# microsoft/XPretrain

Measured on AMD Instinct MI355X. Metric: video-text pairs/sec, higher is better.
Workload: dtype bf16; 1 GPU; CLIP-ViP ViT-B/16 video-text contrastive train step (fwd+loss+bwd+grad-sync+clip+AdamW), 12 frames 224^2, 32 text tokens, local batch 8, BASELINE configs[1]; global_batch=8, parallelism=dp1, gemm_cu_budget=256, grad_wire=fp32, forced_one_rank_collectives=False, video_forward_chains=2, optimizer_overlaps_next_forward_from_layer=3, launch=eager

## Files before the change

include/xpretrain_hip.h:

```cpp
#ifndef XPRETRAIN_HIP_H
#define XPRETRAIN_HIP_H

#include <stddef.h>
#include <stdint.h>

#ifdef __cplusplus
extern "C" {
#endif

#define XP_ABI_VERSION 1

enum { XP_BF16 = 0, XP_F32 = 1 };
enum { XP_OK = 0, XP_ERR_ARG = -1, XP_ERR_LAUNCH = -2, XP_ERR_UNSUPPORTED = -3 };

int xp_abi_version(void);
const char* xp_last_error(void);

enum {
  XP_EPI_NONE = 0,
  XP_EPI_BIAS = 1,
  XP_EPI_BIAS_QSCALE = 2,
  XP_EPI_BIAS_GELU = 3,
  XP_EPI_BIAS_RESID = 4,
  XP_EPI_GELU_BWD = 5,
  XP_EPI_PATCH = 6,
  XP_EPI_SCALE = 7,
  XP_EPI_BIAS_GELU_ERF = 8,
  XP_EPI_GELU_ERF_BWD = 9
};

typedef struct XpGemmDesc {
  const void* A; const void* B; void* C;
  int64_t M, N, K;
  int64_t lda, ldb, ldc;
  int32_t a_kstrided, b_kstrided;
  int32_t in_dtype, out_dtype;
  int32_t epilogue;
  int32_t split_k;
  int64_t a_grp, a_grp_stride, a_off;
  int64_t c_grp, c_grp_stride, c_off;
  const float* bias;
  float scale; int64_t scale_cols;
  const void* resid; int64_t ldr;
  void* aux; int64_t ldaux;
  const float* tab1; const float* tab2; int64_t tab_L;
  float* colsum_partials;
  int32_t reserved0;
  int32_t side_M;
  const float* resid_side; float* out_side; int64_t side_S;
  const void* a_frames; int32_t a_frames_u8; int32_t fr_H, fr_W, fr_P; float fr_mean[3], fr_std[3];
} XpGemmDesc;

int xp_gemm(const XpGemmDesc* desc, void* stream);

int32_t xp_gemm_auto_split(const XpGemmDesc* desc);
int32_t xp_gemm_auto_split_slack(const XpGemmDesc* desc);
int xp_set_cu_budget(int32_t cus);
int32_t xp_get_cu_budget(void);
int64_t xp_gemm_colsum_rows(const XpGemmDesc* desc);
int32_t xp_gemm_tile_rows(const XpGemmDesc* desc);

int xp_splitk_reduce(const float* slabs, float* out, int64_t n, int32_t splits, int32_t accumulate, void* stream);

size_t xp_colsum_workspace_bytes(int64_t rows, int64_t cols);
int xp_colsum(const void* X, int64_t rows, int64_t cols, int64_t ldx, int32_t dtype, float* out,
              int32_t accumulate, void* workspace, size_t workspace_bytes, void* stream);

int64_t xp_colsum_partial_rows(int64_t rows, int64_t cols);
int xp_colsum_partials(const void* X, int64_t rows, int64_t cols, int64_t ldx, int32_t dtype, float* partials,
                       size_t partials_bytes, void* stream);

#define XP_REDUCE_MAX_SEGS 16
typedef struct {
  const float* in; float* out;
  int64_t stride;
  int32_t nrows, width;
  int32_t accumulate, reserved;
} XpReduceSeg;
size_t xp_reduce_rows_batch_workspace_bytes(const XpReduceSeg* segs_host, int32_t n);
int xp_reduce_rows_batch(const XpReduceSeg* segs_host, int32_t n, void* workspace, size_t workspace_bytes, void* stream);

int xp_layernorm_fwd(const void* x, int64_t ldx, const float* gamma, const float* beta, void* y, int64_t ldy,
                     float* mean, float* rstd, int64_t rows, int64_t cols, float eps, int32_t dtype, void* stream);
int xp_layernorm_fwd_side(const void* x, int64_t ldx, const float* gamma, const float* beta, void* y, int64_t ldy,
                          float* mean, float* rstd, int64_t rows, int64_t cols, float eps, int32_t dtype,
                          const float* x_side, float* y_side, int64_t side_S, int32_t side_M, int32_t side_stride, void* stream);
size_t xp_layernorm_bwd_workspace_bytes(int64_t rows, int64_t cols);
int64_t xp_layernorm_bwd_partial_rows(int64_t rows);
int xp_layernorm_bwd_partials(const void* dy, int64_t lddy, const void* x, int64_t ldx, const float* gamma,
                              const float* mean, const float* rstd, const void* dres, int64_t lddres,
                              void* dx, int64_t lddx, int32_t with_dx_colsum, int64_t rows, int64_t cols,
                              int32_t dtype, void* workspace, size_t workspace_bytes, void* stream);
int xp_layernorm_bwd(const void* dy, int64_t lddy, const void* x, int64_t ldx, const float* gamma,
                     const float* mean, const float* rstd, const void* dres, int64_t lddres,
                     void* dx, int64_t lddx, float* dgamma, float* dbeta, int32_t accumulate,
                     int64_t rows, int64_t cols, int32_t dtype,
                     void* workspace, size_t workspace_bytes, void* stream);
int xp_layernorm_bwd_partials_side(const void* dy, int64_t lddy, const void* x, int64_t ldx, const float* gamma,
                                   const float* mean, const float* rstd, const void* dres, int64_t lddres,
                                   void* dx, int64_t lddx, int32_t with_dx_colsum, int64_t rows, int64_t cols,
                                   int32_t dtype, const float* x_side, int64_t side_S, int32_t side_M, int32_t side_stride,
                                   void* workspace, size_t workspace_bytes, void* stream);
int xp_layernorm_bwd_side(const void* dy, int64_t lddy, const void* x, int64_t ldx, const float* gamma,
                          const float* mean, const float* rstd, const void* dres, int64_t lddres,
                          void* dx, int64_t lddx, float* dgamma, float* dbeta, int32_t accumulate,
                          int64_t rows, int64_t cols, int32_t dtype,
                          const float* x_side, int64_t side_S, int32_t side_M, int32_t side_stride,
                          void* workspace, size_t workspace_bytes, void* stream);

enum { XP_ATTN_PROXY = 0, XP_ATTN_CAUSAL = 1 };
size_t xp_attn_workspace_bytes(int32_t mode, int64_t B, int64_t H, int64_t M, int64_t N, int64_t L);
int xp_attn_fwd(const void* qkv, int64_t ldqkv, void* out, int64_t ldo, float* stats,
                const int64_t* pad_mask, int32_t mode, int64_t B, int64_t H, int64_t S,
                int64_t M, int64_t N, int64_t L, int32_t dtype,
                void* workspace, size_t workspace_bytes, void* stream);
int xp_attn_bwd(const void* qkv, int64_t ldqkv, const void* out, const void* dout, int64_t ldo,
                const float* stats, const int64_t* pad_mask, void* dqkv, float q_scale,
                int32_t mode, int64_t B, int64_t H, int64_t S, int64_t M, int64_t N, int64_t L, int32_t dtype,
                void* workspace, size_t workspace_bytes, void* stream);
int xp_set_attn_bwd_wide(int32_t on);
int32_t xp_get_attn_bwd_wide(void);
int64_t xp_attn_bwd_colsum_rows(int32_t mode, int64_t B, int64_t H, int64_t S, int64_t M, int64_t N, int64_t L, int32_t dtype);
int xp_attn_bwd2(const void* qkv, int64_t ldqkv, const void* out, const void* dout, int64_t ldo,
                 const float* stats, const int64_t* pad_mask, void* dqkv, float q_scale,
                 int32_t mode, int64_t B, int64_t H, int64_t S, int64_t M, int64_t N, int64_t L, int32_t dtype,
                 void* workspace, size_t workspace_bytes, float* dqkv_colsum_partials, void* stream);

int xp_attn_probs(const void* qkv, int64_t ldqkv, const float* stats, const int64_t* pad_mask,
                  float* probs, float* probs_proxy, int32_t mode, int64_t B, int64_t H, int64_t S,
                  int64_t M, int64_t N, int64_t L, int32_t dtype, void* stream);

size_t xp_attn_pooled_workspace_bytes(int64_t B, int64_t H, int64_t S, int32_t dtype);
int xp_attn_pooled_fwd(const void* q, const void* kv, int64_t ldkv, void* out, float* stats, int64_t B, int64_t H, int64_t S,
                       int32_t dtype, void* workspace, size_t workspace_bytes, void* stream);
int64_t xp_attn_pooled_colsum_rows(int64_t B, int64_t H, int64_t S, int32_t dtype);
int64_t xp_attn_pooled_colsum_rows_max(int64_t B, int64_t S);
int xp_attn_pooled_bwd(const void* q, const void* kv, int64_t ldkv, const void* out, const void* dout, const float* stats,
                       void* dq, int64_t lddq, void* dkv, int64_t lddkv, float q_scale, int64_t B, int64_t H, int64_t S,
                       int32_t dtype, void* workspace, size_t workspace_bytes, float* dkv_colsum_partials, void* stream);

int xp_im2col(const float* video, void* patches, int64_t BT, int64_t H, int64_t W, int64_t P, int32_t dtype, void* stream);
int xp_im2col_u8(const uint8_t* frames, const float* mean3_host, const float* std3_host, void* patches, int64_t BT,
                 int64_t H, int64_t W, int64_t P, int32_t dtype, void* stream);
#define XP_FRAMES_MAX_VIDEOS 32
#define XP_FRAMES_MAX_SIZE 16384
typedef struct {
  const uint8_t* src; int64_t src_bytes;
  int64_t stride_t, stride_y, stride_x, stride_c;
  int32_t T, H, W;
  int32_t box_y, box_x, box_h, box_w;
  int32_t rh, rw;
  int32_t top, left;
  int32_t flip;
} XpFrameSrc;
int xp_frames_resize_norm(const XpFrameSrc* videos_host, int32_t n_videos, const float* mean3_host,
                          const float* std3_host, float* out, int32_t oh, int32_t ow, void* stream);
#define XP_FRAMES_TRANSFORM_MAX_VIDEOS 24
enum { XP_FRAMES_FILTER_BICUBIC = 0, XP_FRAMES_FILTER_BILINEAR2 = 1 };
enum { XP_FRAMES_COLOR_BRIGHTNESS = 0, XP_FRAMES_COLOR_SATURATION = 2, XP_FRAMES_COLOR_HUE = 3 };
typedef struct {
  XpFrameSrc src;
  int32_t filter;
  int32_t mid_h, mid_w;
  int32_t crop_y, crop_x, crop_h, crop_w;
  int32_t n_color;
  int32_t color_op[3];
  float color_factor[3];
} XpFrameTransform;
int xp_frames_transform(const XpFrameTransform* videos_host, int32_t n_videos, const float* mean3_host,
                        const float* std3_host, float* out, int32_t oh, int32_t ow, void* stream);
#define XP_FRAMES_AA_MAX_TAPS 128
size_t xp_frames_transform_aa_workspace_bytes(const XpFrameTransform* videos_host, int32_t n_videos, int32_t oh, int32_t ow);
int xp_frames_transform_aa(const XpFrameTransform* videos_host, int32_t n_videos, const float* mean3_host,
                           const float* std3_host, float* out, int32_t oh, int32_t ow, void* workspace, size_t workspace_bytes,
                           void* stream);
int xp_vip_proxy_rows(const float* class_emb, const float* added_cls, const float* pos, void* x,
                      int64_t B, int64_t S, int64_t M, int64_t D, int32_t dtype, void* stream);
size_t xp_vip_embed_bwd_workspace_bytes(int64_t B, int64_t T, int64_t L, int64_t D);
int xp_vip_embed_bwd(const void* dx, float* d_class, float* d_added, float* d_pos, float* d_time,
                     int64_t B, int64_t M, int64_t T, int64_t L, int64_t D, int32_t dtype, int32_t accumulate,
                     void* workspace, size_t workspace_bytes, void* stream);
int xp_pos_resample_fwd(const float* pos, float* out, int32_t g0, int32_t gh, int32_t gw, int32_t D, void* stream);
int xp_pos_resample_bwd(const float* d_out, float* d_pos, int32_t g0, int32_t gh, int32_t gw, int32_t D, void* stream);
int xp_text_embed_fwd(const int64_t* ids, const float* tok, const float* pos, void* x,
                      int64_t B, int64_t Lt, int64_t D, int64_t vocab, int32_t dtype, void* stream);
int xp_text_embed_bwd(const int64_t* ids, const void* dx, float* d_tok, float* d_pos,
                      int64_t B, int64_t Lt, int64_t D, int64_t vocab, int32_t dtype, int32_t accumulate, void* stream);
int xp_argmax_rows(const int64_t* ids, int64_t* idx, int64_t B, int64_t Lt, void* stream);
int xp_gather_rows(const void* x, const int64_t* idx, void* out, int64_t B, int64_t S, int64_t D, int32_t dtype, void* stream);
int xp_scatter_rows(const void* dout, const int64_t* idx, void* dx, int64_t B, int64_t S, int64_t D, int32_t dtype, void* stream);
int xp_l2norm_fwd(const void* x, float* y, float* inv_norm, int64_t rows, int64_t cols, int32_t dtype, void* stream);
int xp_l2norm_bwd(const float* dy, const float* y, const float* inv_norm, void* dx, int64_t rows, int64_t cols,
                  int32_t dtype, void* stream);
int xp_cast(const float* src, void* dst, int64_t n, int32_t dtype, void* stream);
int xp_cast_back(const void* src, float* dst, int64_t n, int32_t dtype, int32_t accumulate, void* stream);

#define XP_OPT_CHUNK 65536
#define XP_OPT_MAX_TENSORS 256
#define XP_OPT_MAX_GROUPS 16
typedef struct {
  void* p; void* m; void* v;
  void* shadow;
  int64_t numel;
  int32_t shadow_dtype;
  int32_t reserved;
} XpAdamTensor;
typedef struct {
  float lr, beta1, beta2, eps, weight_decay;
  float step_size;
} XpAdamGroup;
int xp_grad_sqnorm_partials(const XpAdamTensor* table, const int32_t* chunk_map, int32_t n_chunks,
                            const void* const* grads_host, int32_t n_tensors, float* partials, void* stream);
int xp_adamw_step(const XpAdamTensor* table, const int32_t* chunk_map, int32_t n_chunks,
                  const void* const* grads_host, const uint8_t* group_of_host, int32_t n_tensors,
                  const XpAdamGroup* groups_host, int32_t n_groups, const float* norm_partials,
                  int32_t n_norm_partials, float max_norm, float* grad_norm_out, void* stream);

enum XpOptKind { XP_OPT_ADAM, XP_OPT_ADAMAX };
typedef struct {
  float lr, beta1, beta2, eps, weight_decay;
  float step_size;
  float bias2_sqrt;
  float one_minus_beta1;
} XpOptGroup;
int xp_optim_step(int32_t kind, const XpAdamTensor* table, const int32_t* chunk_map, int32_t n_chunks,
                  const void* const* grads_host, const uint8_t* group_of_host, int32_t n_tensors,
                  const XpOptGroup* groups_host, int32_t n_groups, const float* norm_partials,
                  int32_t n_norm_partials, float max_norm, float* grad_norm_out, void* stream);

typedef struct {
  float norm;
  int32_t finite;
  int32_t first_bad_chunk;
  int32_t reserved;
  int64_t applied, skipped;
} XpStepVerdict;
int xp_step_verdict(const float* partials, int32_t n_partials, XpStepVerdict* verdict, void* stream);
int xp_adamw_step_guarded(const XpAdamTensor* table, const int32_t* chunk_map, int32_t n_chunks,
                          const void* const* grads_host, const uint8_t* group_of_host, int32_t n_tensors,
                          const XpAdamGroup* groups_host, int32_t n_groups, const float* norm_partials,
                          int32_t n_norm_partials, float max_norm, float* grad_norm_out,
                          const XpStepVerdict* verdict, void* stream);
int xp_optim_step_guarded(int32_t kind, const XpAdamTensor* table, const int32_t* chunk_map, int32_t n_chunks,
                          const void* const* grads_host, const uint8_t* group_of_host, int32_t n_tensors,
                          const XpOptGroup* groups_host, int32_t n_groups, const float* norm_partials,
                          int32_t n_norm_partials, float max_norm, float* grad_norm_out,
                          const XpStepVerdict* verdict, void* stream);

size_t xp_nce_loss_workspace_bytes(int64_t n, int64_t d);
int xp_nce_loss(const float* vis, const float* txt, const float* log_scale, float* loss,
                float* d_vis, float* d_txt, float* d_log_scale, int64_t n, int64_t d,
                void* workspace, size_t workspace_bytes, void* stream);

size_t xp_vsc_fc_loss_workspace_bytes(int64_t n, int64_t d);
int xp_vsc_fc_loss(const float* vis, const float* txt, const float* img, const float* cap, const float* log_scale,
                   float* loss, float* d_vis, float* d_txt, float* d_img, float* d_cap, float* d_log_scale,
                   int64_t n, int64_t d, void* workspace, size_t workspace_bytes, void* stream);

enum XpLossKind { XP_LOSS_NCE, XP_LOSS_VSC_FC, XP_LOSS_DSL, XP_LOSS_VS_VC, XP_LOSS_VS_VC_FC,
                  XP_LOSS_VSC, XP_LOSS_VIDIMG, XP_LOSS_VIDIMG_DIVIDE };
size_t xp_contrastive_loss_workspace_bytes(int32_t kind, int64_t n, int64_t m, int64_t d);
int xp_contrastive_loss(int32_t kind, const float* vis, const float* txt, const float* img, const float* cap,
                        const float* log_scale, float* loss, float* d_vis, float* d_txt, float* d_img, float* d_cap,
                        float* d_log_scale, int64_t n, int64_t m, int64_t d,
                        void* workspace, size_t workspace_bytes, void* stream);

enum XpPairLossKind { XP_PAIR_NCE, XP_PAIR_TRIPLET, XP_PAIR_HARDNEG, XP_PAIR_MILNCE };
typedef struct {
  float temp, margin;
  int32_t max_violation, order_measure, hard_negative_num, bag;
} XpPairLossParams;
size_t xp_pair_loss_workspace_bytes(int32_t kind, const XpPairLossParams* params, int64_t n, int64_t d);
int xp_pair_loss(int32_t kind, const XpPairLossParams* params, const float* vis, const float* txt, float* loss,
                 float* d_vis, float* d_txt, int64_t n, int64_t d, void* workspace, size_t workspace_bytes, void* stream);

int xp_sim_matrix(const float* a, const float* b, float* sim, int64_t na, int64_t nb, int64_t d, void* stream);
int xp_dsl_rerank(float* sim, int64_t n, int64_t m, float theta, int32_t multiply, void* stream);
int xp_retrieval_ranks(const float* sim, const int64_t* labels, int64_t n, int64_t m, int32_t transpose,
                       int32_t* greater, int32_t* equal, void* stream);

#define XP_RETRIEVAL_TILE 128
#define XP_RETRIEVAL_MAX_K 128
int xp_retrieval_stream_plan(int64_t nq, int64_t ng, int32_t k, int32_t* stat_tiles_per_split, int32_t* topk_tiles_per_split);
size_t xp_retrieval_ranks_streamed_workspace_bytes(int64_t nq, int64_t ng, int64_t d, int32_t dsl);
int xp_retrieval_ranks_streamed(const float* q, const float* g, const int64_t* labels_q, const int64_t* labels_g, int64_t nq,
                                int64_t ng, int64_t d, int32_t dsl, float theta, int32_t* greater_q, int32_t* equal_q,
                                int32_t* greater_g, int32_t* equal_g, void* workspace, size_t workspace_bytes, void* stream);
size_t xp_retrieval_topk_workspace_bytes(int64_t nq, int64_t ng, int64_t d, int32_t k);
int xp_retrieval_topk(const float* q, const float* g, int64_t nq, int64_t ng, int64_t d, int32_t k, int64_t index_base,
                      int32_t accumulate, float* vals, int64_t* idx, void* workspace, size_t workspace_bytes, void* stream);

typedef struct XpLayerDims {
  int64_t rows, D, Dff, B, S, heads;
  int64_t M, N, L;
  int32_t attn_mode, dtype;
  float q_scale, ln_eps;
  int32_t act;
} XpLayerDims;
enum { XP_ACT_QUICK_GELU = 0, XP_ACT_GELU = 1 };

typedef struct XpLayerFwd {
  XpLayerDims dims;
  const void* x; const void* Wqkv; const void* Wo; const void* W1; const void* W2;
  const float* ln1_w; const float* ln1_b; const float* bqkv; const float* bo;
  const float* ln2_w; const float* ln2_b; const float* b1; const float* b2;
  const int64_t* pad_mask;
  void* h1; void* qkv; void* attn_o; void* x2; void* h2; void* pre; void* act; void* x3;
  float* mean1; float* rstd1; float* mean2; float* rstd2; float* stats;
  void* workspace; size_t workspace_bytes;
  const float* side_in; float* side_out; int64_t side_S; int32_t side_M; int32_t reserved;
  float* side_x2;
} XpLayerFwd;
size_t xp_encoder_layer_fwd_workspace_bytes(const XpLayerDims* dims);
int xp_encoder_layer_fwd(const XpLayerFwd* args, void* stream);

typedef struct XpLayerBwd {
  XpLayerDims dims;
  const void* x; const void* h1; const void* qkv; const void* attn_o; const void* x2; const void* h2; const void* pre;
  const void* act; const void* Wqkv; const void* Wo; const void* W1; const void* W2;
  const float* ln1_w; const float* ln2_w; const float* mean1; const float* rstd1; const float* mean2; const float* rstd2;
  const float* stats; const int64_t* pad_mask;
  const void* dx3;
  void* dx;
  float* dln1_w; float* dln1_b; float* dwqkv; float* dbqkv; float* dwo; float* dbo;
  float* dln2_w; float* dln2_b; float* dw1; float* db1; float* dw2; float* db2;
  void* workspace; size_t workspace_bytes;
  const float* side_in; const float* side_x2; int64_t side_S; int32_t side_M; int32_t reserved;
} XpLayerBwd;
size_t xp_encoder_layer_bwd_workspace_bytes(const XpLayerDims* dims);
int xp_encoder_layer_bwd(const XpLayerBwd* args, void* stream);
typedef struct XpLayerPooledFwd {
  XpLayerDims dims;
  const void* x; const void* Wqkv; const void* Wo; const void* W1; const void* W2;
  const float* ln1_w; const float* ln1_b; const float* bqkv; const float* bo;
  const float* ln2_w; const float* ln2_b; const float* b1; const float* b2;
  void* h1; void* kv; float* mean1; float* rstd1;
  void* h1p; void* q; void* attn_o; void* x2; void* h2; void* pre; void* act; void* x3;
  float* mean1p; float* rstd1p; float* mean2; float* rstd2; float* stats;
  void* workspace; size_t workspace_bytes;
  const float* side_in; float* side_out; float* side_x2;
} XpLayerPooledFwd;
size_t xp_encoder_layer_pooled_fwd_workspace_bytes(const XpLayerDims* dims);
int xp_encoder_layer_pooled_fwd(const XpLayerPooledFwd* args, void* stream);

typedef struct XpLayerPooledBwd {
  XpLayerDims dims;
  const void* x; const void* h1; const void* kv; const void* h1p; const void* q; const void* attn_o; const void* x2;
  const void* h2; const void* pre; const void* act; const void* Wqkv; const void* Wo; const void* W1; const void* W2;
  const float* ln1_w; const float* ln2_w; const float* mean1; const float* rstd1; const float* mean1p; const float* rstd1p;
  const float* mean2; const float* rstd2; const float* stats;
  const void* dx3;
  void* dx;
  float* dln1_w; float* dln1_b; float* dwqkv; float* dbqkv; float* dwo; float* dbo;
  float* dln2_w; float* dln2_b; float* dw1; float* db1; float* dw2; float* db2;
  void* workspace; size_t workspace_bytes;
  const float* side_in; const float* side_x2;
} XpLayerPooledBwd;
size_t xp_encoder_layer_pooled_bwd_workspace_bytes(const XpLayerDims* dims);
int xp_encoder_layer_pooled_bwd(const XpLayerPooledBwd* args, void* stream);
void* xp_side_stream(void);

int xp_debug_set_gemm_trace(void* device_buffer);
int xp_debug_gemm_timer_arm(int64_t M, int64_t N, int64_t K, int32_t epilogue, int32_t a_kstrided, int32_t b_kstrided, int32_t split_k,
                            int32_t max_launches);
int32_t xp_debug_gemm_timer_read(float* ms, int32_t cap);
int xp_debug_set_attn_trace(void* device_buffer);
int xp_debug_gemm_occupancy(int lds_bytes);
enum { XP_GEMM_FAMILY_256 = 0,
       XP_GEMM_FAMILY_DIRECT = 1,
       XP_GEMM_FAMILY_STAGED = 2,
       XP_GEMM_FAMILY_FRAMES = 3 };
enum { XP_GEMM_EPI_FAST = 0,
       XP_GEMM_EPI_ROW8 = 1,
       XP_GEMM_EPI_ROW4 = 2 };
typedef struct XpGemmPlanInfo {
  int32_t family, tile_rows;
  int32_t split, flat_split;
  int64_t k_per_split;
  int32_t tiles_m, tiles_n, group_n;
  int32_t epi_impl;
  int32_t grid[3];
  int32_t reserved;
  int64_t colsum_rows;
} XpGemmPlanInfo;
int xp_debug_gemm_plan(const XpGemmDesc* desc, XpGemmPlanInfo* out);
enum { XP_ATTN_KERNEL_FWD = 0,
       XP_ATTN_KERNEL_FWD3 = 1,
       XP_ATTN_KERNEL_FWD4 = 2,
       XP_ATTN_KERNEL_BWD_PAIR = 3,
       XP_ATTN_KERNEL_BWD5 = 4,
       XP_ATTN_KERNEL_F32 = 5 };
enum { XP_ATTN_OPTIN_BWD6 = 6 };
typedef struct XpAttnPlanInfo {
  int32_t kernel;
  int32_t grid, lds_bytes;
  int32_t reduce_grid;
  int32_t uses_counter;
  int32_t reserved;
  int64_t part[2], delta[2], dq[2], dkv[2], counter[2];
  int64_t workspace_bytes;
  int64_t colsum_rows;
} XpAttnPlanInfo;
int xp_debug_attn_plan(int32_t mode, int64_t B, int64_t H, int64_t S, int64_t M, int64_t N, int64_t L, int32_t dtype,
                       int32_t has_pad_mask, int32_t backward, int32_t cus, XpAttnPlanInfo* out);
typedef struct XpAttnPooledPlanInfo {
  int32_t chunks, chunk_keys;
  int32_t grid, combine_grid;
  int64_t part_ml[2], part_acc[2];
  int64_t part_dq[2];
  int64_t workspace_bytes;
  int64_t colsum_rows;
} XpAttnPooledPlanInfo;
int xp_debug_attn_pooled_plan(int64_t B, int64_t H, int64_t S, int32_t dtype, int32_t backward, int32_t cus,
                              XpAttnPooledPlanInfo* out);
int xp_probe_mfma_bf16(const void* a, const void* b, float* c, void* stream);
int xp_probe_mfma_f32(const float* a, const float* b, float* c, void* stream);
int xp_probe_pk_f32(void* err , int32_t iters, int32_t blocks, uint32_t seed, void* stream);
int xp_probe_stream_copy(void* dst, const void* src, int64_t nbytes, int32_t blocks, int32_t iters, void* stream);
int xp_probe_stream_copy_fat(void* dst, const void* src, int64_t nbytes, int32_t blocks, int32_t iters, void* stream);
int xp_probe_tr16(const void* in , const int32_t* lane_byte_off , void* out , void* stream);

#ifdef __cplusplus
}
#endif
#endif
```

xpretrain_amd/csrc/gemm.hip:

```cpp
#include "common.h"
#include "gemm_common.h"
#include <stdlib.h>
#include <mutex>
#include <vector>

namespace {

using namespace xpgemm;
constexpr int BM = 128, BN = 128, BKB = 128;
constexpr int NT = 256;
constexpr int TILE_BYTES = 128 * 128;

template <typename T>
__device__ __forceinline__ void gload_kc(u32x4 (&r)[4], const T* base, int64_t ld, int64_t row0, int64_t rows,
                                         int64_t k0, int64_t kend, const Remap& map, int tid) {
  constexpr int EPC = 16 / sizeof(T);
  const int c = tid & 7, rr = tid >> 3;
  const int64_t k = k0 + c * EPC;
#pragma unroll
  for (int j = 0; j < 4; ++j) {
    const int64_t row = row0 + rr + 32 * j;
    if (row < rows && k < kend)
      r[j] = *reinterpret_cast<const u32x4*>(base + map(row) * ld + k);
    else
// ... 386 lines not shown
      return;
    }
  }
  if (f == Family::DIRECT) launch2<T, true>(d, kp, grid, st);
  else                     launch2<T, false>(d, kp, grid, st);
}

}

extern "C" int xp_debug_gemm_occupancy(int lds_bytes) {
  int nb = -1;
  hipError_t e = hipOccupancyMaxActiveBlocksPerMultiprocessor(&nb, gemm_kernel<bf16_t, false, false, true>, 2 * NT, (size_t)lds_bytes);
  if (e != hipSuccess) return -(int)e;
  return nb;
}

static unsigned long long* g_gemm_trace = nullptr;
extern "C" int xp_debug_set_gemm_trace(void* device_buffer) { g_gemm_trace = (unsigned long long*)device_buffer; return XP_OK; }

namespace {
struct GemmTimer {
  std::mutex mu;
  bool armed = false;
  int64_t M = 0, N = 0, K = 0; int epi = 0, aks = 0, bks = 0, split = 1;
  std::vector<hipEvent_t> ev;
  size_t used = 0;
} g_timer;
static volatile bool g_timer_on = false;
}

extern "C" int xp_debug_gemm_timer_arm(int64_t M, int64_t N, int64_t K, int32_t epilogue, int32_t a_kstrided, int32_t b_kstrided,
                                       int32_t split_k, int32_t max_launches) {
  XP_REQUIRE(max_launches > 0 && max_launches <= 4096, "xp_debug_gemm_timer_arm: max_launches must be 1..4096");
  std::lock_guard<std::mutex> lock(g_timer.mu);
  while (g_timer.ev.size() < (size_t)max_launches * 2) {
    hipEvent_t e;
    if (hipEventCreate(&e) != hipSuccess) { xp_set_error("xp_debug_gemm_timer_arm: hipEventCreate failed"); return XP_ERR_LAUNCH; }
    g_timer.ev.push_back(e);
  }
  g_timer.M = M; g_timer.N = N; g_timer.K = K; g_timer.epi = epilogue; g_timer.aks = a_kstrided; g_timer.bks = b_kstrided;
  g_timer.split = split_k > 1 ? split_k : 1;
  g_timer.used = 0; g_timer.armed = true; g_timer_on = true;
  return XP_OK;
}

extern "C" int32_t xp_debug_gemm_timer_read(float* ms, int32_t cap) {
  std::lock_guard<std::mutex> lock(g_timer.mu);
  g_timer_on = false; g_timer.armed = false;
  const int n = (int)(g_timer.used / 2);
  for (int i = 0; i < n && i < cap; ++i) {
    if (hipEventSynchronize(g_timer.ev[2 * i + 1]) != hipSuccess || hipEventElapsedTime(&ms[i], g_timer.ev[2 * i], g_timer.ev[2 * i + 1]) != hipSuccess) {
      xp_set_error("xp_debug_gemm_timer_read: event query failed");
      return -1;
    }
  }
  g_timer.used = 0;
  return n;
}

static int gemm_timer_slot(const XpGemmDesc* d, int split) {
  if (!g_timer_on) return -1;
  std::lock_guard<std::mutex> lock(g_timer.mu);
  if (!g_timer.armed || d->M != g_timer.M || d->N != g_timer.N || d->K != g_timer.K || d->epilogue != g_timer.epi ||
      (d->a_kstrided != 0) != (g_timer.aks != 0) || (d->b_kstrided != 0) != (g_timer.bks != 0) || split != g_timer.split ||
      g_timer.used + 2 > g_timer.ev.size())
    return -1;
  const int slot = (int)g_timer.used;
  g_timer.used += 2;
  return slot;
}

struct GemmPlan {
  Family family;
  int tile_rows;
  int split; int64_t k_per_split;
  int tiles_m, tiles_n, group_n, xcd_remap, flat_split;
  int wide, fast_epi;
  int epi_impl;
  int64_t colsum_rows;
  dim3 grid;
};

static GemmPlan plan_gemm(const XpGemmDesc* d, int split) {
  GemmPlan p{};
  p.split = split = split > 1 ? split : 1;
  const int esz = d->in_dtype == XP_BF16 ? 2 : 4, ke = BKB / esz;
  p.k_per_split = cdiv(cdiv(d->K, split), ke) * ke;
  p.xcd_remap = 1;
  p.wide = d->N % 8 == 0 && d->ldc % 8 == 0 && (!d->resid || d->ldr % 8 == 0) && (!d->aux || d->ldaux % 8 == 0);
  const int64_t osz = d->out_dtype == XP_F32 ? 4 : esz, lim = (int64_t)EPI_OOB - 64, rows = d->M + 256;
  p.fast_epi = p.wide && !xp_debug_flag("gemm_slow_epi") && d->c_grp == 0 && rows * d->ldc * osz < lim &&
               (!d->resid || rows * d->ldr * esz < lim) && (!d->aux || rows * d->ldaux * osz < lim);
  const int ep = epi_base(d->epilogue);
  const bool f32 = d->out_dtype == XP_F32, cs_epi = ep == XP_EPI_NONE || ep == XP_EPI_GELU_BWD;
  p.epi_impl = epi_impl(p.fast_epi, p.wide, ep, f32, d->colsum_partials != nullptr);
  const bool epi256 = p.epi_impl == XP_GEMM_EPI_FAST;
  const char* env = getenv("XPRETRAIN_GEMM256");
  const int mode = env ? atoi(env) : 1;
  const int64_t k_last = d->K - (int64_t)(split - 1) * p.k_per_split;
  if (mode != 0 && xp_gemm256_legal(d) && epi256 && (mode != 1 || cdiv(d->M, 256) * cdiv(d->N, 256) * split >= 96) &&
      cdiv(k_last, 64) >= 2 && (split == 1 || cdiv(d->K, p.k_per_split) == split)) {
    p.family = Family::G256; p.tile_rows = 256;
    p.tiles_m = (int)cdiv(d->M, 256); p.tiles_n = (int)cdiv(d->N, 256);
    p.group_n = split > 1 ? p.tiles_n : xp_gemm256_group_n(d, p.tiles_n);
    const bool chunk_major = split > 1 && !xp_debug_flag("dw_tile_major");
    p.flat_split = chunk_major ? split : 0;
    p.colsum_rows = split == 1 && !f32 && cs_epi ? 2 * cdiv(d->M, 256) : 0;
    p.grid = dim3(p.tiles_m * p.tiles_n * (chunk_major ? split : 1), 1, chunk_major ? 1 : split);
    return p;
  }
  p.family = d->in_dtype == XP_BF16 && d->a_frames ? Family::FRAMES : glds_ok(d, esz) ? Family::DIRECT : Family::STAGED;
  p.tile_rows = BM;
  p.tiles_m = (int)cdiv(d->M, BM); p.tiles_n = (int)cdiv(d->N, BN);
  const int gmax = 4;
  p.group_n = (int)cdiv(p.tiles_n, cdiv(p.tiles_n, gmax));
  p.grid = dim3(p.tiles_m * p.tiles_n, 1, split);
  return p;
}

extern "C" int xp_gemm(const XpGemmDesc* d, void* stream) {
  XP_REQUIRE(d && (d->A || d->a_frames) && d->B && d->C, "xp_gemm: null operand");
  XP_REQUIRE(d->M > 0 && d->N > 0 && d->K > 0, "xp_gemm: empty problem M=%lld N=%lld K=%lld",
             (long long)d->M, (long long)d->N, (long long)d->K);
  XP_REQUIRE(d->in_dtype == XP_BF16 || d->in_dtype == XP_F32, "xp_gemm: bad in_dtype %d", d->in_dtype);
  XP_REQUIRE(d->out_dtype == d->in_dtype || d->out_dtype == XP_F32, "xp_gemm: bad out_dtype %d", d->out_dtype);
  const int esz = d->in_dtype == XP_BF16 ? 2 : 4;
  const int epc = 16 / esz;
  const int64_t a_contig = d->a_kstrided ? d->M : d->K, b_contig = d->b_kstrided ? d->N : d->K;
  XP_REQUIRE(a_contig % epc == 0 && b_contig % epc == 0 && d->lda % epc == 0 && d->ldb % epc == 0,
             "xp_gemm: contiguous extents / leading dims must be multiples of %d elements", epc);
  XP_REQUIRE(d->N % 4 == 0 && d->ldc % 4 == 0, "xp_gemm: N and ldc must be multiples of 4");
  XP_REQUIRE(((uintptr_t)d->A | (uintptr_t)d->B | (uintptr_t)d->C) % 16 == 0, "xp_gemm: operands must be 16-byte aligned");
  if (d->a_frames) {
    const int64_t P = d->fr_P, gh = P > 0 ? d->fr_H / P : 0, gw = P > 0 ? d->fr_W / P : 0;
    XP_REQUIRE(d->in_dtype == XP_BF16 && !d->a_kstrided && !d->b_kstrided && d->a_grp == 0 && (d->split_k <= 1),
               "xp_gemm: a_frames needs bf16 compute, k-contiguous operands, no row remap of A, no split-K");
    XP_REQUIRE(P > 0 && P % 8 == 0 && d->fr_H % P == 0 && d->fr_W % P == 0 && d->K == 3 * P * P && gh * gw > 0 && d->M % (gh * gw) == 0,
               "xp_gemm: a_frames needs P %% 8 == 0, H and W multiples of P, K == 3*P*P and M a multiple of the patches per frame");
    XP_REQUIRE(((uintptr_t)d->a_frames & (d->a_frames_u8 ? 7 : 15)) == 0 && (d->a_frames_u8 ? d->fr_W % 8 == 0 : d->fr_W % 4 == 0),
               "xp_gemm: a_frames must be 16-byte (fp32) / 8-byte (uint8) aligned with a row pitch that keeps 8-pixel strips aligned");
    if (d->a_frames_u8) for (int c = 0; c < 3; ++c) XP_REQUIRE(d->fr_std[c] > 0.f, "xp_gemm: fr_std[%d] must be positive", c);
  }
  XP_REQUIRE(d->epilogue >= XP_EPI_NONE && d->epilogue <= XP_EPI_GELU_ERF_BWD, "xp_gemm: bad epilogue %d", d->epilogue);
  const int ep = epi_base(d->epilogue);
  if (ep == XP_EPI_BIAS || ep == XP_EPI_BIAS_QSCALE || ep == XP_EPI_BIAS_GELU || ep == XP_EPI_BIAS_RESID)
    XP_REQUIRE(d->bias, "xp_gemm: epilogue %d needs bias", ep);
  if (ep == XP_EPI_BIAS_RESID || ep == XP_EPI_GELU_BWD) XP_REQUIRE(d->resid && d->ldr % 4 == 0, "xp_gemm: epilogue %d needs resid", ep);
  if (ep == XP_EPI_BIAS_GELU) XP_REQUIRE(!d->aux || d->ldaux % 4 == 0, "xp_gemm: epilogue BIAS_GELU: bad ldaux");
  if (ep == XP_EPI_PATCH) XP_REQUIRE(d->tab1 && d->tab2 && d->tab_L > 0, "xp_gemm: epilogue PATCH needs tab1/tab2/tab_L");
  const int split = d->split_k > 1 ? d->split_k : 1;
  if (split > 1) XP_REQUIRE(ep == XP_EPI_NONE && d->out_dtype == XP_F32 && d->c_grp == 0 && d->ldc == d->N,
                            "xp_gemm: split_k needs EPI_NONE, f32 output, dense C");

  const GemmPlan plan = plan_gemm(d, split);
  KParams kp;
  kp.A = d->A; kp.B = d->B; kp.C = d->C;
  kp.M = d->M; kp.N = d->N; kp.K = d->K; kp.lda = d->lda; kp.ldb = d->ldb; kp.ldc = d->ldc;
  kp.amap = Remap{d->a_grp, d->a_grp_stride, d->a_off};
  kp.cmap = Remap{d->c_grp, d->c_grp_stride, d->c_off};
  kp.epilogue = ep; kp.out_f32 = d->out_dtype == XP_F32;
  kp.k_per_split = plan.k_per_split;
  kp.bias = d->bias; kp.scale = d->scale; kp.scale_cols = d->scale_cols;
  kp.resid = d->resid; kp.ldr = d->ldr; kp.aux = d->aux; kp.ldaux = d->ldaux;
  kp.tab1 = d->tab1; kp.tab2 = d->tab2; kp.tab_L = d->tab_L;
  kp.dbg = g_gemm_trace;
  kp.im_src = d->a_frames; kp.im_u8 = d->a_frames_u8; kp.im_H = d->fr_H; kp.im_W = d->fr_W; kp.im_P = d->fr_P;
  kp.im_gw = d->fr_P > 0 ? d->fr_W / d->fr_P : 1; kp.im_L = d->fr_P > 0 ? (d->fr_H / d->fr_P) * kp.im_gw : 1;
  for (int c = 0; c < 3; ++c) { kp.im_mean[c] = d->fr_mean[c]; kp.im_std[c] = d->fr_std[c]; }
  kp.tiles_m = plan.tiles_m; kp.tiles_n = plan.tiles_n; kp.group_n = plan.group_n; kp.xcd_remap = plan.xcd_remap;
  kp.flat_split = plan.flat_split; kp.wide = plan.wide; kp.fast_epi = plan.fast_epi;
  kp.colsum = d->colsum_partials;
  kp.rside = d->resid_side; kp.oside = d->out_side; kp.side_S = (unsigned)d->side_S; kp.side_M = (unsigned)d->side_M;
  if (d->resid_side || d->out_side)
    XP_REQUIRE(d->resid_side && d->out_side && ep == XP_EPI_BIAS_RESID && d->out_dtype == d->in_dtype && d->c_grp == 0 &&
               d->side_S > 0 && d->side_M > 0 && d->side_M <= d->side_S && d->M + 512 < ((int64_t)1 << 24) && d->N % 8 == 0,
               "xp_gemm: resid_side / out_side need both pointers, EPI_BIAS_RESID, an unmapped output, 0 < side_M <= side_S, M < 2^24");
  if (d->colsum_partials)
    XP_REQUIRE(plan.colsum_rows > 0, "xp_gemm: fused column sums are not available for this problem "
               "(xp_gemm_colsum_rows() == 0): use xp_colsum / xp_colsum_partials");
  const int zsplits = (int)cdiv(d->K, plan.k_per_split);
  XP_REQUIRE(split == 1 || zsplits == split, "xp_gemm: split_k=%d leaves empty slabs for K=%lld (use <= %d)",
             split, (long long)d->K, zsplits);
  hipStream_t st = (hipStream_t)stream;
  const int tslot = gemm_timer_slot(d, split);
  if (tslot >= 0) (void)hipEventRecord(g_timer.ev[tslot], st);
  struct Stop { int slot; hipStream_t st; ~Stop() { if (slot >= 0) (void)hipEventRecord(g_timer.ev[slot + 1], st); } } stop{tslot, st};
  if (plan.family == Family::G256) {
    if (!xp_gemm256_launch(d, kp, plan.grid, st)) {
      xp_set_error("xp_gemm: the 256x256 family cannot launch: no current device, or its 128 KiB dynamic-LDS opt-in was refused");
      return XP_ERR_LAUNCH;
    }
    XP_CHECK_LAUNCH("xp_gemm(256)");
    return XP_OK;
  }
  if (d->in_dtype == XP_BF16) launch<bf16_t>(plan.family, d, kp, plan.grid, st);
  else                        launch<float>(plan.family, d, kp, plan.grid, st);
  XP_CHECK_LAUNCH("xp_gemm");
  return XP_OK;
}

extern "C" int64_t xp_gemm_colsum_rows(const XpGemmDesc* d) { return d ? plan_gemm(d, d->split_k).colsum_rows : 0; }

extern "C" int xp_debug_gemm_plan(const XpGemmDesc* d, XpGemmPlanInfo* out) {
  XP_REQUIRE(d && out, "xp_debug_gemm_plan: null argument");
  const GemmPlan p = plan_gemm(d, d->split_k);
  static_assert((int)Family::G256 == XP_GEMM_FAMILY_256 && (int)Family::DIRECT == XP_GEMM_FAMILY_DIRECT &&
                (int)Family::STAGED == XP_GEMM_FAMILY_STAGED && (int)Family::FRAMES == XP_GEMM_FAMILY_FRAMES, "XP_GEMM_FAMILY_*");
  *out = XpGemmPlanInfo{};
  out->family = (int)p.family; out->tile_rows = p.tile_rows;
  out->split = p.split; out->flat_split = p.flat_split; out->k_per_split = p.k_per_split;
  out->tiles_m = p.tiles_m; out->tiles_n = p.tiles_n; out->group_n = p.group_n;
  out->epi_impl = p.epi_impl;
  out->grid[0] = (int)p.grid.x; out->grid[1] = (int)p.grid.y; out->grid[2] = (int)p.grid.z;
  out->colsum_rows = p.colsum_rows;
  return XP_OK;
}

extern "C" int32_t xp_gemm_tile_rows(const XpGemmDesc* d) {
  if (!d || d->M <= 0 || d->N <= 0 || d->K <= 0) return 0;
  return plan_gemm(d, d->split_k).tile_rows;
}

static int valid_split(int64_t K, int64_t s0, int64_t ke) {
  if (s0 <= 1) return 1;
  const int64_t kps = cdiv(cdiv(K, s0), ke) * ke;
  return (int)cdiv(K, kps);
}

static int g_cu_budget = [] {
  const char* e = getenv("XPRETRAIN_CU_BUDGET");
  const int v = e ? atoi(e) : 256;
  return v >= 64 && v <= 256 ? v : 256;
}();
extern "C" int xp_set_cu_budget(int32_t cus) {
  XP_REQUIRE(cus >= 64 && cus <= 256, "xp_set_cu_budget: %d not in 64..256", cus);
  g_cu_budget = cus;
  return XP_OK;
}
extern "C" int32_t xp_get_cu_budget(void) { return g_cu_budget; }

constexpr int64_t XP_SPLITK_FILL = 144, XP_SPLITK_FILL_SLACK = 112;
static int64_t g_fill[2] = {XP_SPLITK_FILL, XP_SPLITK_FILL_SLACK};
static const bool g_fill_env = [] {
  const char* e = getenv("XPRETRAIN_SPLITK_FILL");
  if (!e) return false;
  int a = 0, b = 0;
  const int n = sscanf(e, "%d%*[,x]%d", &a, &b);
  if (n >= 1 && a >= 9 && a <= 256) g_fill[0] = a;
  if (n >= 2 && b >= 9 && b <= 256) g_fill[1] = b;
  return true;
}();
static int32_t auto_split_fill(const XpGemmDesc* d, int64_t fill);
extern "C" int32_t xp_gemm_auto_split(const XpGemmDesc* d) { return auto_split_fill(d, g_fill[0]); }
extern "C" int32_t xp_gemm_auto_split_slack(const XpGemmDesc* d) {
  const int32_t s = auto_split_fill(d, g_fill[1]), g = auto_split_fill(d, g_fill[0]);
  return s < g ? s : g;
}

static int32_t auto_split_fill(const XpGemmDesc* d, int64_t fill) {
  if (!d || d->M <= 0 || d->N <= 0 || d->K <= 0) return 1;
  const int esz = d->in_dtype == XP_BF16 ? 2 : 4;
  const int64_t ke = BKB / esz;
  const int64_t t256 = cdiv(d->M, 256) * cdiv(d->N, 256);
  const int64_t cus = g_cu_budget < fill ? g_cu_budget : fill;
  int64_t s0 = cus / t256 < d->K / 512 ? cus / t256 : d->K / 512;
  const int s256 = valid_split(d->K, s0, 64);
  if (plan_gemm(d, s256).family == Family::G256) return s256;
  const int64_t t128 = cdiv(d->M, BM) * cdiv(d->N, BN);
  if (t128 >= 256) return 1;
  s0 = 512 / t128 < d->K / 512 ? 512 / t128 : d->K / 512;
  return valid_split(d->K, s0, ke);
}
```

xpretrain_amd/csrc/gemm256.hip:

```cpp
#include "common.h"
#include "gemm_common.h"

namespace {

using namespace xpgemm;

typedef bf16_t T;
constexpr int TM = 256, TN = 256, SKB = 128, KE = 64;
constexpr int NTH = 512, NWAVES = 8;
constexpr int WAVES_N = 4, MT = 8, NT = 4;
constexpr int HALF_ROWS = 128, HALF_BYTES = HALF_ROWS * SKB, NSLOT = 8, LDS_BYTES = NSLOT * HALF_BYTES;

typedef __attribute__((address_space(3))) char lds_char;

template <bool KS, int SUB>
struct HalfStager {
  __amdgpu_buffer_rsrc_t rsrc;
  unsigned voff[2][2];
  unsigned step;
  unsigned lds_off[2];

  static __device__ __forceinline__ int tile_row(int r, int h) { return (r / SUB) * (2 * SUB) + h * SUB + (r % SUB); }

  __device__ __forceinline__ void init(const T* base, int64_t ld, int64_t row0, int64_t rows, int64_t kend, int64_t kbeg,
                                       int lane, int wave) {
    const int64_t bytes = (KS ? kend : rows) * ld * 2;
    rsrc = __builtin_amdgcn_make_buffer_rsrc(const_cast<T*>(base), 0, (unsigned)bytes, 0x00020000);
#pragma unroll
    for (int j = 0; j < 2; ++j) {
      const int pass = j * NWAVES + wave;
      lds_off[j] = pass * 1024;
#pragma unroll
      for (int h = 0; h < 2; ++h) {
        int64_t off;
        if constexpr (!KS) {
          const int row = pass * 8 + (lane >> 3);
          const int c = (lane & 7) ^ swz128(row);
          off = ((row0 + tile_row(row, h)) * ld + kbeg) * 2 + c * 16;
        } else {
          const int kr = pass * 4 + (lane >> 4), c16 = lane & 15;
          const int src = (((c16 >> 1) ^ ks_f(kr)) << 1) | (c16 & 1);
          off = ((kbeg + kr) * ld + row0 + tile_row(src * 8, h)) * 2;
        }
        voff[h][j] = off >= bytes ? 0xFFFFFFF0u : (unsigned)off;
      }
    }
    step = (unsigned)((KS ? (int64_t)KE * ld : (int64_t)KE) * 2);
  }
  __device__ __forceinline__ void issue(char* slot, int h, int kt) const {
    lds_char* t3 = (lds_char*)slot;
    const unsigned adv = (unsigned)kt * step;
#pragma unroll
    for (int j = 0; j < 2; ++j) {
      unsigned o = voff[h][j] + adv;
      if (o < voff[h][j]) o = 0xFFFFFFF0u;
      __builtin_amdgcn_raw_ptr_buffer_load_lds(rsrc, t3 + lds_off[j], 16, o, 0, 0, 0);
    }
  }
};

template <bool KS>
__device__ __forceinline__ bf16x8 frag(const char* tile, int ot, int ks, int lane) {
  constexpr int RB = HALF_ROWS * 2;
  const int i = lane & 15, g = lane >> 4;
  if constexpr (!KS) {
    return *reinterpret_cast<const bf16x8*>(tile + tile128_off(ot * 16 + i, ks * 4 + g));
  } else {
    const int f = (i >> 2) | ((g & 1) << 2);
    const int kr = ks * 32 + g * 8 + (i >> 2);
    const char* p = tile + kr * RB + ((ot ^ f) << 5) + ((i & 3) << 3);
    i16x4 lo = lds_read_tr16_async<0>(p);
    i16x4 hi = lds_read_tr16_async<4 * RB>(p);
    typedef __attribute__((ext_vector_type(8))) short i16x8;
    i16x8 v = {lo[0], lo[1], lo[2], lo[3], hi[0], hi[1], hi[2], hi[3]};
    return __builtin_bit_cast(bf16x8, v);
  }
}

template <int N> __device__ __forceinline__ void wait_vmcnt() { asm volatile("s_waitcnt vmcnt(%0)" ::"n"(N) : "memory"); }

template <bool AKS, bool BKS, typename... Act>
__global__ __launch_bounds__(NTH, 2) void gemm256_kernel(KParams p) {
  constexpr int ACT = ActOf<Act...>::value;
  extern __shared__ __attribute__((aligned(16))) char smem[];
  const int tid = threadIdx.x, lane = tid & 63;
  const int wave = __builtin_amdgcn_readfirstlane(tid >> 6);
  const int wm = wave / WAVES_N, wn = wave % WAVES_N;

  const int nwg = p.tiles_m * p.tiles_n;
  int bid, zs, nsplit;
  if (p.flat_split > 0) {
    const int l = xcd_remap(blockIdx.x, nwg * p.flat_split, 1);
    zs = l / nwg; bid = l - zs * nwg; nsplit = p.flat_split;
  } else {
    bid = xcd_remap(blockIdx.x, nwg, p.xcd_remap); zs = blockIdx.z; nsplit = gridDim.z;
  }
  int tm, tn;
  tile_of(bid, p.tiles_m, p.tiles_n, p.group_n, tm, tn);
  const int64_t m0 = (int64_t)tm * TM, n0 = (int64_t)tn * TN;

  const int64_t kbeg = (int64_t)zs * p.k_per_split;
  const int64_t kend = (kbeg + p.k_per_split < p.K) ? kbeg + p.k_per_split : p.K;
  const int nk = (int)((kend - kbeg + KE - 1) / KE);

  HalfStager<AKS, 64> ga;
  HalfStager<BKS, 32> gb;
  ga.init(reinterpret_cast<const T*>(p.A), p.lda, m0, p.M, kend, kbeg, lane, wave);
  gb.init(reinterpret_cast<const T*>(p.B), p.ldb, n0, p.N, kend, kbeg, lane, wave);

  f32x4 acc[NT][MT];
#pragma unroll
  for (int a = 0; a < NT; ++a)
#pragma unroll
    for (int b = 0; b < MT; ++b) acc[a][b] = f32x4{0.f, 0.f, 0.f, 0.f};

  const bool trace = p.dbg != nullptr && bid == nwg / 2 && zs == 0 && wave == 0;
  unsigned long long* tr = p.dbg;
  if (trace && lane == 0) { tr[0] = __builtin_amdgcn_s_memtime(); tr[1] = nk; }
  const bool tline = p.dbg != nullptr && wave == 0 && lane == 0 && zs == 0 && tr[4] == 0x7aceull;
  if (tline) { tr[64 + bid * 4 + 0] = __builtin_amdgcn_s_memrealtime(); tr[64 + bid * 4 + 3] = __builtin_amdgcn_s_getreg(4 | (0 << 6) | (31 << 11)); }

  auto slot = [&](int kt, int w) -> char* { return smem + (((kt & 1) << 2) + w) * HALF_BYTES; };

  gb.issue(slot(1, 3), 0, 0);
  ga.issue(slot(0, 0), 0, 0); gb.issue(slot(0, 1), 1, 0); ga.issue(slot(0, 2), 1, 0); gb.issue(slot(0, 3), 0, 1);
  wait_vmcnt<4>();
  __builtin_amdgcn_s_barrier();
  if (wm == 1) __builtin_amdgcn_s_barrier();

  bf16x8 fa[2][4], fb[2][2][2], fbn[2][2];

#define XP_PHASE_MMA(HA)                                                                              \
  do {                                                                                                \
    __builtin_amdgcn_s_barrier();                                                                     \
    asm volatile("s_waitcnt lgkmcnt(0)" ::: "memory");                                                \
    __builtin_amdgcn_sched_barrier(0);                                                                \
    __builtin_amdgcn_s_setprio(1);                                                                    \
    _Pragma("unroll") for (int hb = 0; hb < 2; ++hb)                                                  \
      _Pragma("unroll") for (int ks = 0; ks < 2; ++ks)                                                \
        _Pragma("unroll") for (int mt = 0; mt < 4; ++mt)                                              \
          _Pragma("unroll") for (int nt = 0; nt < 2; ++nt)                                            \
            acc[hb * 2 + nt][(HA) * 4 + mt] = mma16(fb[hb][ks][nt], fa[ks][mt], acc[hb * 2 + nt][(HA) * 4 + mt]); \
    __builtin_amdgcn_s_setprio(0);                                                                    \
    __builtin_amdgcn_sched_barrier(0);                                                                \
    __builtin_amdgcn_s_barrier();                                                                     \
  } while (0)
#define XP_READ_A(TILE)                                                                               \
  _Pragma("unroll") for (int ks = 0; ks < 2; ++ks)                                                    \
    _Pragma("unroll") for (int mt = 0; mt < 4; ++mt) fa[ks][mt] = frag<AKS>(TILE, wm * 4 + mt, ks, lane)
#define XP_READ_B(DST, TILE)                                                                          \
  _Pragma("unroll") for (int ks = 0; ks < 2; ++ks)                                                    \
    _Pragma("unroll") for (int nt = 0; nt < 2; ++nt) DST[ks][nt] = frag<BKS>(TILE, wn * 2 + nt, ks, lane)

  XP_READ_B(fbn, slot(1, 3));

  auto ktile = [&](int t, auto tail_c) {
    constexpr int TAIL = decltype(tail_c)::value;
#pragma unroll
    for (int ks = 0; ks < 2; ++ks)
#pragma unroll
      for (int nt = 0; nt < 2; ++nt) fb[0][ks][nt] = fbn[ks][nt];
    XP_READ_B(fb[1], slot(t, 1));
    __builtin_amdgcn_sched_barrier(0);
    XP_READ_A(slot(t, 0));
    __builtin_amdgcn_sched_barrier(0);
    if constexpr (TAIL <= 1) { ga.issue(slot(t + 1, 0), 0, t + 1); gb.issue(slot(t + 1, 1), 1, t + 1); }
    wait_vmcnt<(TAIL <= 1 ? 4 : 0)>();
    XP_PHASE_MMA(0);
    if constexpr (TAIL <= 1) { XP_READ_B(fbn, slot(t, 3)); }
    __builtin_amdgcn_sched_barrier(0);
    XP_READ_A(slot(t, 2));
    __builtin_amdgcn_sched_barrier(0);
    if constexpr (TAIL <= 1) ga.issue(slot(t + 1, 2), 1, t + 1);
    if constexpr (TAIL == 0) gb.issue(slot(t + 1, 3), 0, t + 2);
    wait_vmcnt<(TAIL == 0 ? 4 : (TAIL == 1 ? 2 : 0))>();
    XP_PHASE_MMA(1);
  };
  for (int t = 0; t < nk - 2; ++t) ktile(t, std::integral_constant<int, 0>{});
  ktile(nk - 2, std::integral_constant<int, 1>{});
  ktile(nk - 1, std::integral_constant<int, 2>{});
#undef XP_PHASE_MMA
#undef XP_READ_A
#undef XP_READ_B
  if (wm == 0) __builtin_amdgcn_s_barrier();
  __builtin_amdgcn_s_barrier();
  if (trace && lane == 0) tr[2] = __builtin_amdgcn_s_memtime();
  if (tline) tr[64 + bid * 4 + 1] = __builtin_amdgcn_s_memrealtime();

  constexpr int CW = NT * 16;
  char* stg = smem + wave * (32 * CW * 4);
  const int i16 = lane & 15, g = lane >> 4;
  float* Cf = reinterpret_cast<float*>(p.C);
  T* Ct = reinterpret_cast<T*>(p.C);
  if (nsplit > 1) Cf += (int64_t)zs * p.M * p.N;
  auto stage_round = [&](int q) {
#pragma unroll
    for (int h = 0; h < 2; ++h) {
      const int row = h * 16 + i16;
#pragma unroll
      for (int nt = 0; nt < NT; ++nt)
        *reinterpret_cast<f32x4*>(stg + row * (CW * 4) + (((nt * 4 + g) ^ (row & 7)) << 4)) = acc[nt][q * 2 + h];
    }
    asm volatile("s_waitcnt lgkmcnt(0)" ::: "memory");
  };
  const bool fast = fast_epi_dispatch<ACT>(p, [&](auto epi_c, auto f32_c, auto cs_c) {
    constexpr int EPI = decltype(epi_c)::value;
    constexpr bool F32 = decltype(f32_c)::value;
    constexpr bool COLSUM = decltype(cs_c)::value;
    f32x8 cs = {f32x4{0.f, 0.f, 0.f, 0.f}, f32x4{0.f, 0.f, 0.f, 0.f}};
    const int c = lane & 7, r8 = lane >> 3;
    const FastEpi<T, EPI, F32, ACT> fe(p, F32 ? (void*)Cf : (void*)Ct, n0 + wn * CW + c * 8);
    const unsigned mrow = (unsigned)(m0 + wm * (MT * 16)) + r8;
    Raw8<T> pre[2][4];
    if constexpr (EpiTraits<EPI>::pre) {
#pragma unroll
      for (int pass = 0; pass < 4; ++pass) pre[0][pass] = fe.load_pre(mrow + pass * 8);
    }
#pragma unroll
    for (int q = 0; q < MT / 2; ++q) {
      if constexpr (EpiTraits<EPI>::pre) {
        if (q + 1 < MT / 2) {
#pragma unroll
          for (int pass = 0; pass < 4; ++pass) pre[(q + 1) & 1][pass] = fe.load_pre(mrow + (q + 1) * 32 + pass * 8);
        }
      }
      stage_round(q);
      f32x8 v[4];
#pragma unroll
      for (int pass = 0; pass < 4; ++pass) {
        const int row = pass * 8 + r8;
        v[pass].lo = *reinterpret_cast<const f32x4*>(stg + row * (CW * 4) + (((2 * c) ^ (row & 7)) << 4));
        v[pass].hi = *reinterpret_cast<const f32x4*>(stg + row * (CW * 4) + (((2 * c + 1) ^ (row & 7)) << 4));
      }
#pragma unroll
      for (int pass = 0; pass < 4; ++pass) {
        const f32x8 o = fe.finish(v[pass], pre[q & 1][pass], mrow + q * 32 + pass * 8);
        if constexpr (COLSUM) {
          if (mrow + q * 32 + pass * 8 < (unsigned)p.M) { cs.lo += o.lo; cs.hi += o.hi; }
        }
      }
      asm volatile("s_waitcnt lgkmcnt(0)" ::: "memory");
    }
    if constexpr (COLSUM) {
#pragma unroll
      for (int o = 8; o < 64; o <<= 1)
#pragma unroll
        for (int e = 0; e < 4; ++e) { cs.lo[e] += __shfl_xor(cs.lo[e], o, 64); cs.hi[e] += __shfl_xor(cs.hi[e], o, 64); }
      const int64_t n = n0 + wn * CW + c * 8;
      if (r8 == 0 && n < p.N) {
        float* dst = p.colsum + ((int64_t)tm * 2 + wm) * p.N + n;
        store4(dst, cs.lo); store4(dst + 4, cs.hi);
      }
    }
  });
  (void)fast;
  if (trace && lane == 0) tr[3] = __builtin_amdgcn_s_memtime();
  if (tline) { asm volatile("s_waitcnt vmcnt(0)" ::: "memory"); tr[64 + bid * 4 + 2] = __builtin_amdgcn_s_memrealtime(); }
}

template <bool AKS, bool BKS>
bool launch_one(int act, const KParams& kp, dim3 grid, hipStream_t st) {
  auto kern = act == XP_ACT_GELU ? gemm256_kernel<AKS, BKS, GeluErfTag> : gemm256_kernel<AKS, BKS>;
  if (!xp_device_cus(reinterpret_cast<const void*>(kern), LDS_BYTES)) return false;
  kern<<<grid, NTH, LDS_BYTES, st>>>(kp);
  return true;
}

template __global__ void gemm256_kernel<false, false>(KParams);
template __global__ void gemm256_kernel<false, true>(KParams);
template __global__ void gemm256_kernel<true, true>(KParams);
template __global__ void gemm256_kernel<true, false>(KParams);
template __global__ void gemm256_kernel<false, false, GeluErfTag>(KParams);
template __global__ void gemm256_kernel<false, true, GeluErfTag>(KParams);
template __global__ void gemm256_kernel<true, true, GeluErfTag>(KParams);
template __global__ void gemm256_kernel<true, false, GeluErfTag>(KParams);

}

bool xp_gemm256_legal(const XpGemmDesc* d) {
  if (d->in_dtype != XP_BF16 || d->a_grp != 0 || d->a_frames) return false;
  const int64_t a_rows = d->a_kstrided ? d->K : d->M, b_rows = d->b_kstrided ? d->K : d->N;
  if (!d->a_kstrided && (d->K % KE != 0 || d->lda != d->K)) return false;
  if (!d->b_kstrided && (d->K % KE != 0 || d->ldb != d->K)) return false;
  if (d->a_kstrided && (d->M % TM != 0 || d->lda != d->M)) return false;
  if (d->b_kstrided && (d->N % TN != 0 || d->ldb != d->N)) return false;
  const int64_t lim = (int64_t)0xFFFFFFF0u - 512 * 1024 * 1024;
  return (a_rows + TM) * d->lda * 2 < lim && (b_rows + TN) * d->ldb * 2 < lim;
}

int xp_gemm256_group_n(const XpGemmDesc* d, int tiles_n) {
  int groups = 1;
  const int64_t wbytes = (int64_t)tiles_n * TN * d->K * (d->in_dtype == XP_BF16 ? 2 : 4);
  while (groups < 4 && wbytes / groups > (int64_t)3600 * 1024 && tiles_n / (groups * 2) >= 4) groups *= 2;
  return (int)cdiv(tiles_n, groups);
}

bool xp_gemm256_launch(const XpGemmDesc* d, const xpgemm::KParams& kp, dim3 grid, hipStream_t st) {
  const int act = xpgemm::epi_act(d->epilogue);
  if (!d->a_kstrided && !d->b_kstrided)      return launch_one<false, false>(act, kp, grid, st);
  else if (!d->a_kstrided && d->b_kstrided)  return launch_one<false, true>(act, kp, grid, st);
  else if (d->a_kstrided && d->b_kstrided)   return launch_one<true, true>(act, kp, grid, st);
  return launch_one<true, false>(act, kp, grid, st);
}
```

xpretrain_amd/csrc/gemm_common.h:

```cpp
#pragma once
#include "common.h"
#include <type_traits>

namespace xpgemm {

struct Remap {
  int64_t grp, stride, off;
  __device__ __forceinline__ int64_t operator()(int64_t r) const {
    return grp == 0 ? r : (r / grp) * stride + off + (r % grp);
  }
};

__host__ __device__ constexpr int epi_base(int epilogue) {
  return epilogue == XP_EPI_BIAS_GELU_ERF ? XP_EPI_BIAS_GELU : epilogue == XP_EPI_GELU_ERF_BWD ? XP_EPI_GELU_BWD : epilogue;
}
__host__ __device__ constexpr int epi_act(int epilogue) {
  return epilogue == XP_EPI_BIAS_GELU_ERF || epilogue == XP_EPI_GELU_ERF_BWD ? XP_ACT_GELU : XP_ACT_QUICK_GELU;
}

struct GeluErfTag {};
template <typename... Tag> struct ActOf { static constexpr int value = XP_ACT_QUICK_GELU; };
template <> struct ActOf<GeluErfTag> { static constexpr int value = XP_ACT_GELU; };

struct KParams {
  const void* A; const void* B; void* C;
  int64_t M, N, K, lda, ldb, ldc;
  Remap amap, cmap;
  int epilogue, out_f32;
  int64_t k_per_split;
  const float* bias; float scale; int64_t scale_cols;
  const void* resid; int64_t ldr;
  void* aux; int64_t ldaux;
  const float* tab1; const float* tab2; int64_t tab_L;
  int tiles_m, tiles_n;
  int group_n;
  int xcd_remap;
  int wide;
  int fast_epi;
  float* colsum;
  const float* rside; float* oside; unsigned side_S, side_M;
  unsigned long long* dbg;
  int flat_split;
  const void* im_src; int im_u8, im_H, im_W, im_P, im_gw, im_L; float im_mean[3], im_std[3];
};


struct SideRows {
  const float* rin; float* out; unsigned S, M; int64_t N, rows; float inv_S;
  __device__ __forceinline__ SideRows(const KParams& p)
      : rin(p.rside), out(p.oside), S(p.side_S), M(p.side_M), N(p.N), rows(p.M), inv_S(1.0f / (float)p.side_S) {}
  __device__ __forceinline__ bool on() const { return rin != nullptr; }
  __device__ __forceinline__ bool hit(unsigned m, int64_t& base) const {
    unsigned q = (unsigned)((float)m * inv_S);
    int rem = (int)m - (int)(q * S);
    if (rem < 0) { --q; rem += (int)S; } else if (rem >= (int)S) { ++q; rem -= (int)S; }
    base = ((int64_t)q * M + rem) * N;
    return (unsigned)rem < M && (int64_t)m < rows;
  }
};

__device__ __forceinline__ f32x4 qscale4(float scale, int64_t scale_cols, int64_t n) {
  return f32x4{n < scale_cols ? scale : 1.f, n + 1 < scale_cols ? scale : 1.f, n + 2 < scale_cols ? scale : 1.f,
               n + 3 < scale_cols ? scale : 1.f};
}

struct EpiLane {
  f32x4 bias, colscale;
  __device__ __forceinline__ EpiLane(const KParams& p, int64_t n) {
    const int ep = p.epilogue;
    const bool has_bias = ep == XP_EPI_BIAS || ep == XP_EPI_BIAS_QSCALE || ep == XP_EPI_BIAS_GELU || ep == XP_EPI_BIAS_RESID;
    bias = has_bias ? load4(p.bias + n) : f32x4{0.f, 0.f, 0.f, 0.f};
    colscale = ep == XP_EPI_SCALE ? f32x4{p.scale, p.scale, p.scale, p.scale}
             : ep == XP_EPI_BIAS_QSCALE ? qscale4(p.scale, p.scale_cols, n) : f32x4{1.f, 1.f, 1.f, 1.f};
  }
};

template <typename T, int ACT = XP_ACT_QUICK_GELU>
__device__ __forceinline__ void epi_row(const KParams& p, const EpiLane& el, f32x4 v, int64_t m, int64_t n, float* Cf, T* Ct) {
  const int ep = p.epilogue;
  v = (v + el.bias) * el.colscale;
  const int64_t crow = p.cmap(m);
  if (ep == XP_EPI_BIAS_GELU) {
    if (!p.aux) {}
    else if (p.out_f32) store4(reinterpret_cast<float*>(p.aux) + crow * p.ldaux + n, v);
    else                store4(reinterpret_cast<T*>(p.aux) + crow * p.ldaux + n, v);
#pragma unroll
    for (int e = 0; e < 4; ++e) v[e] = act_f<ACT>(v[e]);
  } else if (ep == XP_EPI_BIAS_RESID) {
    const SideRows sr(p);
    int64_t sb;
    if (sr.on() && sr.hit((unsigned)m, sb)) { v += load4(sr.rin + sb + n); store4(sr.out + sb + n, v); }
    else v += load4(reinterpret_cast<const T*>(p.resid) + crow * p.ldr + n);
  } else if (ep == XP_EPI_GELU_BWD) {
    const f32x4 pre = load4(reinterpret_cast<const T*>(p.resid) + crow * p.ldr + n);
#pragma unroll
    for (int e = 0; e < 4; ++e) v[e] *= act_grad_f<ACT>(pre[e]);
  } else if (ep == XP_EPI_PATCH) {
    const int64_t w = p.cmap.grp ? (m % p.cmap.grp) : m;
    v += load4(p.tab1 + (w / p.tab_L) * p.N + n);
    v += load4(p.tab2 + (w % p.tab_L) * p.N + n);
  }
  if (p.out_f32) store4(Cf + crow * p.ldc + n, v);
  else           store4(Ct + crow * p.ldc + n, v);
}

struct EpiLane8 {
  f32x8 bias, cs;
  __device__ __forceinline__ EpiLane8(const KParams& p, int64_t n) {
    const EpiLane a(p, n), b(p, n + 4);
    bias = f32x8{a.bias, b.bias}; cs = f32x8{a.colscale, b.colscale};
  }
};
template <typename T, int ACT = XP_ACT_QUICK_GELU>
__device__ __forceinline__ void epi_row8(const KParams& p, const EpiLane8& el, f32x8 v, int64_t m, int64_t n, float* Cf, T* Ct) {
  const int ep = p.epilogue;
  v.lo = (v.lo + el.bias.lo) * el.cs.lo; v.hi = (v.hi + el.bias.hi) * el.cs.hi;
  const int64_t crow = p.cmap(m);
  if (ep == XP_EPI_BIAS_GELU) {
    if (!p.aux) {}
    else if (p.out_f32) store8(reinterpret_cast<float*>(p.aux) + crow * p.ldaux + n, v);
    else                store8(reinterpret_cast<T*>(p.aux) + crow * p.ldaux + n, v);
#pragma unroll
    for (int e = 0; e < 4; ++e) { v.lo[e] = act_f<ACT>(v.lo[e]); v.hi[e] = act_f<ACT>(v.hi[e]); }
  } else if (ep == XP_EPI_BIAS_RESID) {
    const SideRows sr(p);
    int64_t sb;
    if (sr.on() && sr.hit((unsigned)m, sb)) {
      const f32x8 r = load8(sr.rin + sb + n);
      v.lo += r.lo; v.hi += r.hi;
      store8(sr.out + sb + n, v);
    } else {
      const f32x8 r = load8(reinterpret_cast<const T*>(p.resid) + crow * p.ldr + n);
      v.lo += r.lo; v.hi += r.hi;
    }
  } else if (ep == XP_EPI_GELU_BWD) {
    const f32x8 pre = load8(reinterpret_cast<const T*>(p.resid) + crow * p.ldr + n);
#pragma unroll
    for (int e = 0; e < 4; ++e) { v.lo[e] *= act_grad_f<ACT>(pre.lo[e]); v.hi[e] *= act_grad_f<ACT>(pre.hi[e]); }
  } else if (ep == XP_EPI_PATCH) {
    const int64_t w = p.cmap.grp ? (m % p.cmap.grp) : m;
    const f32x8 a = load8(p.tab1 + (w / p.tab_L) * p.N + n), b = load8(p.tab2 + (w % p.tab_L) * p.N + n);
    v.lo += a.lo + b.lo; v.hi += a.hi + b.hi;
  }
  if (p.out_f32) store8(Cf + crow * p.ldc + n, v);
  else           store8(Ct + crow * p.ldc + n, v);
}

typedef __attribute__((ext_vector_type(4))) unsigned u32x4;
constexpr unsigned EPI_OOB = 0xFFFFFF00u;

template <int EPI> struct EpiTraits {
  static_assert(EPI >= XP_EPI_NONE && EPI <= XP_EPI_SCALE, "EpiTraits takes the base kind (epi_base)");
  static constexpr bool bias = EPI == XP_EPI_BIAS || EPI == XP_EPI_BIAS_QSCALE || EPI == XP_EPI_BIAS_GELU || EPI == XP_EPI_BIAS_RESID;
  static constexpr bool scale = EPI == XP_EPI_BIAS_QSCALE || EPI == XP_EPI_SCALE;
  static constexpr bool pre = EPI == XP_EPI_BIAS_RESID || EPI == XP_EPI_GELU_BWD;
};

template <typename T, bool F32>
__device__ __forceinline__ void bstore8(__amdgpu_buffer_rsrc_t r, unsigned off, const f32x8& v) {
  if constexpr (F32 || sizeof(T) == 4) {
    __builtin_amdgcn_raw_buffer_store_b128(__builtin_bit_cast(u32x4, v.lo), r, off, 0, 0);
    __builtin_amdgcn_raw_buffer_store_b128(__builtin_bit_cast(u32x4, v.hi), r, off + 16, 0, 0);
  } else {
    bf16x8 o = {(bf16_t)v.lo[0], (bf16_t)v.lo[1], (bf16_t)v.lo[2], (bf16_t)v.lo[3],
                (bf16_t)v.hi[0], (bf16_t)v.hi[1], (bf16_t)v.hi[2], (bf16_t)v.hi[3]};
    __builtin_amdgcn_raw_buffer_store_b128(__builtin_bit_cast(u32x4, o), r, off, 0, 0);
  }
}
template <typename T> struct Raw8 { u32x4 a, b; };
template <typename T>
__device__ __forceinline__ Raw8<T> bload8(__amdgpu_buffer_rsrc_t r, unsigned off) {
  Raw8<T> x;
  x.a = __builtin_amdgcn_raw_buffer_load_b128(r, off, 0, 0);
  if constexpr (sizeof(T) == 4) x.b = __builtin_amdgcn_raw_buffer_load_b128(r, off + 16, 0, 0);
  return x;
}
template <typename T>
__device__ __forceinline__ f32x8 raw8_f32(const Raw8<T>& x) {
  if constexpr (sizeof(T) == 4) return f32x8{__builtin_bit_cast(f32x4, x.a), __builtin_bit_cast(f32x4, x.b)};
  else {
    const bf16x8 v = __builtin_bit_cast(bf16x8, x.a);
    return f32x8{f32x4{(float)v[0], (float)v[1], (float)v[2], (float)v[3]}, f32x4{(float)v[4], (float)v[5], (float)v[6], (float)v[7]}};
  }
}

template <typename T, int EPI, bool F32, int ACT = XP_ACT_QUICK_GELU>
struct FastEpi {
  using Tr = EpiTraits<EPI>;
  static constexpr unsigned OSZ = F32 ? 4 : sizeof(T);
  __amdgpu_buffer_rsrc_t rc, rx;
  f32x8 bias, cs;
  unsigned ld_c, ld_x;
  unsigned col_c, col_x;
  bool ok, keep_aux;
  SideRows side; int64_t ncol;
  __device__ __forceinline__ FastEpi(const KParams& p, void* Cbase, int64_t n) : side(p) {
// ... 109 lines not shown
```

xpretrain_amd/csrc/layer.hip:

```cpp
#include "common.h"
#include <string.h>
#include <stdlib.h>
#include <initializer_list>
#include <mutex>

namespace {

inline size_t align256(size_t n) { return (n + 255) & ~(size_t)255; }

struct Carver {
  char* base; size_t cap, off = 0;
  bool fits = true;
  template <class T = void>
  T* take(size_t n, size_t* aligned = nullptr) {
    T* p = base ? reinterpret_cast<T*>(base + off) : nullptr;
    n = align256(n);
    off += n;
    if (aligned) *aligned = n;
    if (base && off + 256 > cap) fits = false;
    return p;
  }
  size_t bytes() const { return off + 256; }
};
#define XP_REQUIRE_WORKSPACE(name, a, w)                                                                    \
  XP_REQUIRE((a)->workspace && (w).ws.fits, "%s: workspace too small (%zu < %zu)", name, (a)->workspace_bytes, (w).ws.bytes())

XpGemmDesc gemm_desc(const void* A, const void* B, void* C, int64_t M, int64_t N, int64_t K, int dtype) {
  XpGemmDesc d;
  memset(&d, 0, sizeof(d));
  d.A = A; d.B = B; d.C = C; d.M = M; d.N = N; d.K = K;
  d.lda = K; d.ldb = K; d.ldc = N; d.ldr = N; d.ldaux = N;
  d.in_dtype = dtype; d.out_dtype = dtype; d.split_k = 1; d.scale = 1.0f;
  return d;
}

XpGemmDesc wgrad_desc(const void* dy, int64_t lddy, const void* x, int64_t ldx, float* dw, int64_t k, int64_t n_out, int64_t n_in,
                      int dtype) {
  XpGemmDesc d = gemm_desc(dy, x, dw, n_out, n_in, k, dtype);
  d.a_kstrided = d.b_kstrided = 1; d.lda = lddy; d.ldb = ldx; d.out_dtype = XP_F32;
  return d;
}
int run_wgrad(XpGemmDesc d, float* slabs, size_t slab_bytes, void* st, bool slack) {
  const int split = slack ? xp_gemm_auto_split_slack(&d) : xp_gemm_auto_split(&d);
  if (split <= 1) return xp_gemm(&d, st);
  XP_REQUIRE(slab_bytes >= (size_t)split * d.M * d.N * sizeof(float), "encoder layer backward: split-K slab space too small");
  float* dw = (float*)d.C;
  d.C = slabs; d.split_k = split;
  int rc = xp_gemm(&d, st);
  if (rc) return rc;
  return xp_splitk_reduce(slabs, dw, d.M * d.N, split, 0, st);
}
XpGemmDesc wgrad_desc(const void* dy, const void* x, float* dw, int64_t k, int64_t n_out, int64_t n_in, int dtype) {
  return wgrad_desc(dy, n_out, x, n_in, dw, k, n_out, n_in, dtype);
}
size_t max_slab_bytes(size_t s, std::initializer_list<XpGemmDesc> ds) {
  for (XpGemmDesc d : ds) {
    const int a = xp_gemm_auto_split(&d), b = xp_gemm_auto_split_slack(&d), split = a > b ? a : b;
    const size_t t = split <= 1 ? 0 : (size_t)split * d.M * d.N * sizeof(float);
    if (t > s) s = t;
  }
  return s;
}

struct Defer {
  XpReduceSeg segs[XP_REDUCE_MAX_SEGS]; int n = 0;
  void add(const float* in, float* out, int64_t stride, int nrows, int width) {
    if (!out) return;
    XpReduceSeg& s = segs[n++];
    s.in = in; s.out = out; s.stride = stride; s.nrows = nrows; s.width = width; s.accumulate = 0; s.reserved = 0;
  }
};

struct WgradSide {
  hipStream_t side = nullptr;
  hipEvent_t ev[4] = {nullptr, nullptr, nullptr, nullptr};
  hipEvent_t done = nullptr;
  bool ok = false;
};
WgradSide* wgrad_side() {
  static const bool on = !getenv("XPRETRAIN_WGRAD_STREAM") || atoi(getenv("XPRETRAIN_WGRAD_STREAM")) != 0;
  if (!on) return nullptr;
  static std::mutex mu;
  static WgradSide per_dev[16];
  int dev = 0;
  if (hipGetDevice(&dev) != hipSuccess || dev < 0 || dev >= 16) return nullptr;
  std::lock_guard<std::mutex> lock(mu);
  WgradSide& w = per_dev[dev];
  if (!w.side) {
    bool good = hipStreamCreateWithPriority(&w.side, hipStreamNonBlocking, 0) == hipSuccess;
    for (int i = 0; i < 4 && good; ++i) good = hipEventCreateWithFlags(&w.ev[i], hipEventDisableTiming) == hipSuccess;
    good = good && hipEventCreateWithFlags(&w.done, hipEventDisableTiming) == hipSuccess;
    w.ok = good;
  }
  return w.ok ? &w : nullptr;
}

struct WgradOrder {
  WgradSide* side; hipStream_t main; const char* name;
  void* stream() const { return side ? (void*)side->side : (void*)main; }
  int mark(int i) const {
    if (!side) return XP_OK;
    if (hipEventRecord(side->ev[i], main) != hipSuccess || hipStreamWaitEvent(side->side, side->ev[i], 0) != hipSuccess) {
      xp_set_error("%s: event hand-off to the weight-gradient stream failed", name);
      return XP_ERR_LAUNCH;
    }
    return XP_OK;
  }
  int join() const {
    if (!side) return XP_OK;
    if (hipEventRecord(side->done, side->side) != hipSuccess || hipStreamWaitEvent(main, side->done, 0) != hipSuccess) {
      xp_set_error("%s: joining the weight-gradient stream failed", name);
      return XP_ERR_LAUNCH;
    }
    return XP_OK;
  }
};


inline int epi_act_fwd(const XpLayerDims& d) { return d.act == XP_ACT_GELU ? XP_EPI_BIAS_GELU_ERF : XP_EPI_BIAS_GELU; }
inline int epi_act_bwd(const XpLayerDims& d) { return d.act == XP_ACT_GELU ? XP_EPI_GELU_ERF_BWD : XP_EPI_GELU_BWD; }

template <class Args>
int out_proj_mlp_fwd(const Args& a, int64_t n, int64_t ldr, const float* side_x, float* side_x2, float* side_out, int64_t sS,
                     int32_t sM, void* st) {
  const XpLayerDims& d = a.dims;
  const int64_t D = d.D, Dff = d.Dff;
  const int dt = d.dtype;
  int rc;
  XpGemmDesc g = gemm_desc(a.attn_o, a.Wo, a.x2, n, D, D, dt);
  g.epilogue = XP_EPI_BIAS_RESID; g.bias = a.bo; g.resid = a.x; g.ldr = ldr;
  if (side_x) { g.resid_side = side_x; g.out_side = side_x2; g.side_S = sS; g.side_M = sM; }
  if ((rc = xp_gemm(&g, st))) return rc;
  if ((rc = xp_layernorm_fwd_side(a.x2, D, a.ln2_w, a.ln2_b, a.h2, D, a.mean2, a.rstd2, n, D, d.ln_eps, dt,
                                  side_x2, nullptr, sS, sM, sM, st))) return rc;
  g = gemm_desc(a.h2, a.W1, a.act, n, Dff, D, dt);
  g.epilogue = epi_act_fwd(d); g.bias = a.b1; g.aux = a.pre;
  if ((rc = xp_gemm(&g, st))) return rc;
  g = gemm_desc(a.act, a.W2, a.x3, n, D, Dff, dt);
  g.epilogue = XP_EPI_BIAS_RESID; g.bias = a.b2; g.resid = a.x2;
  if (side_x) { g.resid_side = side_x2; g.out_side = side_out; g.side_S = sS; g.side_M = sM; }
  return xp_gemm(&g, st);
}

struct TailBwd {
  void *dpre, *dh2, *dx2, *dattn, *red; float *cs_pre, *ln2_part;
  size_t esz, cs_pre_bytes, ln2_bytes, red_bytes, slabs;
  int64_t db1_fused_rows, cs_pre_rows, ln_rows;
};
TailBwd carve_tail_bwd(Carver& ws, int64_t n, int64_t D, int64_t Dff, int dt, int64_t db1_fused_rows) {
  TailBwd t;
  t.esz = dt == XP_BF16 ? 2 : 4;
  t.dpre = ws.take(n * Dff * t.esz); t.dh2 = ws.take(n * D * t.esz); t.dx2 = ws.take(n * D * t.esz); t.dattn = ws.take(n * D * t.esz);
  t.db1_fused_rows = db1_fused_rows;
  t.cs_pre_rows = db1_fused_rows > 0 ? db1_fused_rows : xp_colsum_partial_rows(n, Dff);
  t.cs_pre = ws.take<float>(t.cs_pre_rows * Dff * sizeof(float), &t.cs_pre_bytes);
  t.ln_rows = xp_layernorm_bwd_partial_rows(n);
  t.ln2_part = ws.take<float>(xp_layernorm_bwd_workspace_bytes(n, D), &t.ln2_bytes);
  t.red = ws.take((size_t)XP_REDUCE_MAX_SEGS * 32 * (size_t)(3 * D > Dff ? 3 * D : Dff) * sizeof(float) + 16, &t.red_bytes);
  t.slabs = max_slab_bytes(0, {wgrad_desc(nullptr, nullptr, nullptr, n, D, Dff, dt), wgrad_desc(nullptr, nullptr, nullptr, n, Dff, D, dt),
                               wgrad_desc(nullptr, nullptr, nullptr, n, D, D, dt)});
  return t;
}

template <class Args>
int mlp_out_proj_bwd(const Args& a, int64_t n, const TailBwd& t, float* slabs, size_t slab_bytes, int64_t sS,
                     int32_t sM, Defer& df, const WgradOrder& wg, void* st) {
  const int64_t D = a.dims.D, Dff = a.dims.Dff;
  const int dt = a.dims.dtype;
  int rc;
  XpGemmDesc g = gemm_desc(a.dx3, a.W2, t.dpre, n, Dff, D, dt);
  g.b_kstrided = 1; g.ldb = Dff; g.epilogue = epi_act_bwd(a.dims); g.resid = a.pre; g.ldr = Dff;
  if (a.db1 && t.db1_fused_rows > 0) g.colsum_partials = t.cs_pre;
  if ((rc = xp_gemm(&g, st))) return rc;
  if (a.db1) {
    if (t.db1_fused_rows == 0 && (rc = xp_colsum_partials(t.dpre, n, Dff, Dff, dt, t.cs_pre, t.cs_pre_bytes, st))) return rc;
    df.add(t.cs_pre, a.db1, Dff, (int)t.cs_pre_rows, (int)Dff);
  }
  if (a.dw2 && (rc = run_wgrad(wgrad_desc(a.dx3, a.act, a.dw2, n, D, Dff, dt), slabs, slab_bytes, wg.stream(), true))) return rc;
  if ((rc = wg.mark(1))) return rc;
  g = gemm_desc(t.dpre, a.W1, t.dh2, n, D, Dff, dt);
  g.b_kstrided = 1; g.ldb = D;
  if ((rc = xp_gemm(&g, st))) return rc;
  if (a.dw1 && (rc = run_wgrad(wgrad_desc(t.dpre, a.h2, a.dw1, n, Dff, D, dt), slabs, slab_bytes, wg.stream(), true))) return rc;
  if ((rc = xp_layernorm_bwd_partials_side(t.dh2, D, a.x2, D, a.ln2_w, a.mean2, a.rstd2, a.dx3, D, t.dx2, D, 2, n, D, dt,
                                           a.side_x2, sS, sM, sM, t.ln2_part, t.ln2_bytes, st))) return rc;
  df.add(t.ln2_part, a.dln2_w, 4 * D, (int)t.ln_rows, (int)D);
  df.add(t.ln2_part + D, a.dln2_b, 4 * D, (int)t.ln_rows, (int)D);
  df.add(t.ln2_part + 2 * D, a.dbo, 4 * D, (int)t.ln_rows, (int)D);
  df.add(t.ln2_part + 3 * D, a.db2, 4 * D, (int)t.ln_rows, (int)D);
  if ((rc = wg.mark(2))) return rc;
  g = gemm_desc(t.dx2, a.Wo, t.dattn, n, D, D, dt);
  g.b_kstrided = 1; g.ldb = D;
  if ((rc = xp_gemm(&g, st))) return rc;
  if (a.dwo && (rc = run_wgrad(wgrad_desc(t.dx2, a.attn_o, a.dwo, n, D, D, dt), slabs, slab_bytes, wg.stream(), true))) return rc;
  return XP_OK;
}

int finish_bwd(const Defer& df, void* red_ws, size_t red_bytes, const WgradOrder& wg, void* st) {
  if (df.n) {
    XP_REQUIRE(xp_reduce_rows_batch_workspace_bytes(df.segs, df.n) <= red_bytes, "%s: reduce scratch too small", wg.name);
    int rc = xp_reduce_rows_batch(df.segs, df.n, red_ws, red_bytes, st);
    if (rc) return rc;
  }
  return wg.join();
}

int check_dims(const char* name, const XpLayerDims& d) {
  XP_REQUIRE(d.rows > 0 && d.D > 0 && d.Dff > 0 && d.B > 0 && d.S > 0 && d.heads > 0, "%s: empty dimension", name);
  XP_REQUIRE(d.rows == d.B * d.S && d.D == d.heads * 64, "%s: rows != B*S or D != heads*64", name);
  XP_REQUIRE(d.dtype == XP_BF16 || d.dtype == XP_F32, "%s: bad dtype %d", name, d.dtype);
  XP_REQUIRE(d.act == XP_ACT_QUICK_GELU || d.act == XP_ACT_GELU, "%s: bad XpLayerDims::act %d (XP_ACT_QUICK_GELU = 0, XP_ACT_GELU = 1)",
             name, d.act);
  return XP_OK;
}

}

extern "C" void* xp_side_stream(void) {
  WgradSide* w = wgrad_side();
  return w ? (void*)w->side : nullptr;
}

namespace {
struct FwdWs { Carver ws; void* attn; float* side_x2; size_t attn_bytes; };
FwdWs carve_fwd(const XpLayerDims& d, int64_t side_rows, void* base, size_t cap) {
  FwdWs w;
  Carver& ws = w.ws = Carver{(char*)base, cap};
  w.attn = ws.take(xp_attn_workspace_bytes(d.attn_mode, d.B, d.heads, d.M, d.N, d.L), &w.attn_bytes);
  w.side_x2 = ws.take<float>((size_t)side_rows * d.D * sizeof(float));
  return w;
}
}

extern "C" size_t xp_encoder_layer_fwd_workspace_bytes(const XpLayerDims* d) {
  if (!d) return 0;
  return carve_fwd(*d, d->attn_mode == XP_ATTN_PROXY ? d->B * d->M : d->rows, nullptr, 0).ws.bytes();
}

extern "C" int xp_encoder_layer_fwd(const XpLayerFwd* a, void* st) {
  XP_REQUIRE(a, "xp_encoder_layer_fwd: null argument");
  const XpLayerDims& d = a->dims;
  int rc = check_dims("xp_encoder_layer_fwd", d);
  if (rc) return rc;
  XP_REQUIRE(a->x && a->Wqkv && a->Wo && a->W1 && a->W2 && a->ln1_w && a->ln1_b && a->bqkv && a->bo && a->ln2_w && a->ln2_b &&
             a->b1 && a->b2 && a->h1 && a->qkv && a->attn_o && a->x2 && a->h2 && a->act && a->x3 && a->mean1 &&
             a->rstd1 && a->mean2 && a->rstd2 && a->stats, "xp_encoder_layer_fwd: null pointer");
  const int64_t rows = d.rows, D = d.D;
  const int dt = d.dtype;
  const bool sided = a->side_in != nullptr;
  XP_REQUIRE(!sided || (a->side_out && dt == XP_BF16 && a->side_S > 0 && a->side_M > 0 && a->side_M <= a->side_S),
             "xp_encoder_layer_fwd: side rows need side_in and side_out, bf16 and 0 < side_M <= side_S");
  const int64_t sS = a->side_S;
  const int32_t sM = a->side_M;
  const FwdWs w = carve_fwd(d, sided ? cdiv(rows, sS) * sM : 0, a->workspace, a->workspace_bytes);
  XP_REQUIRE_WORKSPACE("xp_encoder_layer_fwd", a, w);
  float* side_x2 = !sided ? nullptr : a->side_x2 ? a->side_x2 : w.side_x2;
  if ((rc = xp_layernorm_fwd_side(a->x, D, a->ln1_w, a->ln1_b, a->h1, D, a->mean1, a->rstd1, rows, D, d.ln_eps, dt,
                                  a->side_in, nullptr, sS, sM, sM, st))) return rc;
  XpGemmDesc g = gemm_desc(a->h1, a->Wqkv, a->qkv, rows, 3 * D, D, dt);
  g.epilogue = XP_EPI_BIAS_QSCALE; g.bias = a->bqkv; g.scale = d.q_scale; g.scale_cols = D;
  if ((rc = xp_gemm(&g, st))) return rc;
  if ((rc = xp_attn_fwd(a->qkv, 3 * D, a->attn_o, D, a->stats, a->pad_mask, d.attn_mode, d.B, d.heads, d.S, d.M, d.N, d.L, dt,
                        w.attn, w.attn_bytes, st))) return rc;
  return out_proj_mlp_fwd(*a, rows, D, a->side_in, side_x2, a->side_out, sS, sM, st);
}

namespace {
struct BwdWs {
  Carver ws; TailBwd t;
  void *dqkv, *dh1, *attn; float *slabs, *cs_qkv, *ln1_part;
  size_t slab_bytes, cs_qkv_bytes, ln1_bytes, attn_bytes;
  int64_t cs_qkv_rows;
  bool cs_qkv_fused;
};
BwdWs carve_bwd(const XpLayerDims& d, void* base, size_t cap) {
  BwdWs w;
  Carver& ws = w.ws = Carver{(char*)base, cap};
  const int64_t rows = d.rows, D = d.D, Dff = d.Dff;
  XpGemmDesc g = gemm_desc(nullptr, nullptr, nullptr, rows, Dff, D, d.dtype);
  g.b_kstrided = 1; g.ldb = Dff; g.epilogue = epi_act_bwd(d); g.ldr = Dff;
  g.resid = &g;
  w.t = carve_tail_bwd(ws, rows, D, Dff, d.dtype, xp_gemm_colsum_rows(&g));
  w.dqkv = ws.take(rows * 3 * D * w.t.esz); w.dh1 = ws.take(rows * D * w.t.esz);
  w.slabs = ws.take<float>(max_slab_bytes(w.t.slabs, {wgrad_desc(nullptr, nullptr, nullptr, rows, 3 * D, D, d.dtype)}), &w.slab_bytes);
  w.cs_qkv_rows = xp_attn_bwd_colsum_rows(d.attn_mode, d.B, d.heads, d.S, d.M, d.N, d.L, d.dtype);
  w.cs_qkv_fused = w.cs_qkv_rows > 0;
  if (!w.cs_qkv_fused) w.cs_qkv_rows = xp_colsum_partial_rows(rows, 3 * D);
  w.cs_qkv = ws.take<float>(w.cs_qkv_rows * 3 * D * sizeof(float), &w.cs_qkv_bytes);
  w.ln1_part = ws.take<float>(w.t.ln2_bytes, &w.ln1_bytes);
  w.attn = ws.take(xp_attn_workspace_bytes(d.attn_mode, d.B, d.heads, d.M, d.N, d.L), &w.attn_bytes);
  return w;
}
}

extern "C" size_t xp_encoder_layer_bwd_workspace_bytes(const XpLayerDims* d) {
  if (!d || d->rows <= 0) return 0;
  return carve_bwd(*d, nullptr, 0).ws.bytes();
}

extern "C" int xp_encoder_layer_bwd(const XpLayerBwd* a, void* st) {
  XP_REQUIRE(a, "xp_encoder_layer_bwd: null argument");
  const XpLayerDims& d = a->dims;
  int rc = check_dims("xp_encoder_layer_bwd", d);
  if (rc) return rc;
  XP_REQUIRE(a->x && a->h1 && a->qkv && a->attn_o && a->x2 && a->h2 && a->pre && a->act && a->Wqkv && a->Wo && a->W1 && a->W2 &&
             a->ln1_w && a->ln2_w && a->mean1 && a->rstd1 && a->mean2 && a->rstd2 && a->stats && a->dx3 && a->dx,
             "xp_encoder_layer_bwd: null pointer");
  XP_REQUIRE((!a->side_in && !a->side_x2) || (a->side_in && a->side_x2 && d.dtype == XP_BF16 && a->side_S > 0 && a->side_M > 0 &&
                                               a->side_M <= a->side_S),
             "xp_encoder_layer_bwd: side rows need side_in and side_x2, bf16 and 0 < side_M <= side_S");
  const BwdWs w = carve_bwd(d, a->workspace, a->workspace_bytes);
  XP_REQUIRE_WORKSPACE("xp_encoder_layer_bwd", a, w);
  const int64_t rows = d.rows, D = d.D;
  const int dt = d.dtype;
  Defer df;
  const WgradOrder wg{(d.attn_mode == XP_ATTN_PROXY && rows >= 4096) ? wgrad_side() : nullptr, (hipStream_t)st, "xp_encoder_layer_bwd"};
  if ((rc = wg.mark(0))) return rc;
  if ((rc = mlp_out_proj_bwd(*a, rows, w.t, w.slabs, w.slab_bytes, a->side_S, a->side_M, df, wg, st))) return rc;
  if ((rc = xp_attn_bwd2(a->qkv, 3 * D, a->attn_o, w.t.dattn, D, a->stats, a->pad_mask, w.dqkv, d.q_scale, d.attn_mode, d.B, d.heads,
                         d.S, d.M, d.N, d.L, dt, w.attn, w.attn_bytes, (a->dbqkv && w.cs_qkv_fused) ? w.cs_qkv : nullptr, st))) return rc;
  if ((rc = wg.mark(3))) return rc;
  XpGemmDesc g = gemm_desc(w.dqkv, a->Wqkv, w.dh1, rows, D, 3 * D, dt);
  g.b_kstrided = 1; g.ldb = D;
  if ((rc = xp_gemm(&g, st))) return rc;
  if (a->dwqkv && (rc = run_wgrad(wgrad_desc(w.dqkv, a->h1, a->dwqkv, rows, 3 * D, D, dt), w.slabs, w.slab_bytes, wg.stream(), false))) return rc;
  if (a->dbqkv) {
    if (!w.cs_qkv_fused && (rc = xp_colsum_partials(w.dqkv, rows, 3 * D, 3 * D, dt, w.cs_qkv, w.cs_qkv_bytes, st))) return rc;
    df.add(w.cs_qkv, a->dbqkv, 3 * D, (int)w.cs_qkv_rows, (int)(3 * D));
  }
  if ((rc = xp_layernorm_bwd_partials_side(w.dh1, D, a->x, D, a->ln1_w, a->mean1, a->rstd1, w.t.dx2, D, a->dx, D, 0, rows, D, dt,
                                           a->side_in, a->side_S, a->side_M, a->side_M, w.ln1_part, w.ln1_bytes, st))) return rc;
  df.add(w.ln1_part, a->dln1_w, 2 * D, (int)w.t.ln_rows, (int)D);
  df.add(w.ln1_part + D, a->dln1_b, 2 * D, (int)w.t.ln_rows, (int)D);
  return finish_bwd(df, w.t.red, w.t.red_bytes, wg, st);
}

namespace {

int check_pooled_dims(const char* name, const XpLayerDims& d) {
  int rc = check_dims(name, d);
  if (rc) return rc;
  XP_REQUIRE(d.attn_mode == XP_ATTN_PROXY && d.M >= 1 && d.N >= 1 && d.L >= 1 && d.S == d.M + d.N * d.L,
             "%s: the pooled layer is the video tower's (XP_ATTN_PROXY, M >= 1, S == M + N*L)", name);
  return XP_OK;
}

struct PooledFwdWs { Carver ws; void* attn; float *side0, *side_x2; size_t attn_bytes; };
PooledFwdWs carve_pooled_fwd(const XpLayerDims& d, void* base, size_t cap) {
  PooledFwdWs w;
  Carver& ws = w.ws = Carver{(char*)base, cap};
  w.attn = ws.take(xp_attn_pooled_workspace_bytes(d.B, d.heads, d.S, d.dtype), &w.attn_bytes);
  w.side0 = ws.take<float>((size_t)d.B * d.D * sizeof(float)); w.side_x2 = ws.take<float>((size_t)d.B * d.D * sizeof(float));
  return w;
}

struct PooledBwdWs {
  Carver ws; TailBwd t;
  char* dqkv; void *dh1, *attn; float *slabs, *cs_q, *cs_kv, *ln1_part, *ln1p_part;
  size_t slab_bytes, cs_q_bytes, ln1_bytes, ln1p_bytes, attn_bytes;
  int64_t cs_q_rows, ln_rows;
};
PooledBwdWs carve_pooled_bwd(const XpLayerDims& d, void* base, size_t cap) {
  PooledBwdWs w;
  Carver& ws = w.ws = Carver{(char*)base, cap};
  const int64_t rows = d.rows, D = d.D, B = d.B, S = d.S;
  const int dt = d.dtype;
  w.t = carve_tail_bwd(ws, B, D, d.Dff, dt, 0);
  w.dqkv = ws.take<char>(rows * 3 * D * w.t.esz); w.dh1 = ws.take(rows * D * w.t.esz);
  XpGemmDesc gq = wgrad_desc(nullptr, 3 * D, nullptr, D, nullptr, B, D, D, dt);
  gq.a_grp = 1; gq.a_grp_stride = S;
  w.slabs = ws.take<float>(max_slab_bytes(w.t.slabs, {gq, wgrad_desc(nullptr, 3 * D, nullptr, D, nullptr, rows, 2 * D, D, dt)}), &w.slab_bytes);
  w.cs_q_rows = xp_colsum_partial_rows(B, D);
  w.cs_q = ws.take<float>(w.cs_q_rows * D * sizeof(float), &w.cs_q_bytes);
  w.cs_kv = ws.take<float>(xp_attn_pooled_colsum_rows_max(B, S) * 2 * D * sizeof(float));
  w.ln_rows = xp_layernorm_bwd_partial_rows(rows);
  w.ln1_part = ws.take<float>(xp_layernorm_bwd_workspace_bytes(rows, D), &w.ln1_bytes);
  w.ln1p_part = ws.take<float>(w.t.ln2_bytes, &w.ln1p_bytes);
  w.attn = ws.take(xp_attn_pooled_workspace_bytes(B, d.heads, S, dt), &w.attn_bytes);
  return w;
}

}

extern "C" size_t xp_encoder_layer_pooled_fwd_workspace_bytes(const XpLayerDims* d) {
  if (!d || d->B <= 0 || d->D <= 0 || d->S <= 0 || d->heads <= 0) return 0;
  return carve_pooled_fwd(*d, nullptr, 0).ws.bytes();
}

extern "C" int xp_encoder_layer_pooled_fwd(const XpLayerPooledFwd* a, void* st) {
  XP_REQUIRE(a, "xp_encoder_layer_pooled_fwd: null argument");
  const XpLayerDims& d = a->dims;
  int rc = check_pooled_dims("xp_encoder_layer_pooled_fwd", d);
  if (rc) return rc;
  XP_REQUIRE(a->x && a->Wqkv && a->Wo && a->W1 && a->W2 && a->ln1_w && a->ln1_b && a->bqkv && a->bo && a->ln2_w && a->ln2_b &&
             a->b1 && a->b2 && a->h1 && a->kv && a->mean1 && a->rstd1 && a->h1p && a->q && a->attn_o && a->x2 && a->h2 && a->act &&
             a->x3 && a->mean1p && a->rstd1p && a->mean2 && a->rstd2 && a->stats, "xp_encoder_layer_pooled_fwd: null pointer");
  const int64_t rows = d.rows, D = d.D, B = d.B, S = d.S;
  const int dt = d.dtype;
  const bool sided = a->side_in != nullptr;
  XP_REQUIRE(!sided || (a->side_out && dt == XP_BF16), "xp_encoder_layer_pooled_fwd: side rows need side_in and side_out, and bf16");
  const PooledFwdWs w = carve_pooled_fwd(d, a->workspace, a->workspace_bytes);
  XP_REQUIRE_WORKSPACE("xp_encoder_layer_pooled_fwd", a, w);
  float* side0 = sided ? w.side0 : nullptr;
  float* side_x2 = !sided ? nullptr : a->side_x2 ? a->side_x2 : w.side_x2;
  const int64_t sS = sided ? S : 0;
  const int32_t sM = sided ? (int32_t)d.M : 0, s1 = sided ? 1 : 0;
  const size_t esz = dt == XP_BF16 ? 2 : 4;
  if ((rc = xp_layernorm_fwd_side(a->x, D, a->ln1_w, a->ln1_b, a->h1, D, a->mean1, a->rstd1, rows, D, d.ln_eps, dt,
                                  a->side_in, nullptr, sS, sM, sM, st))) return rc;
  if (sided && (rc = xp_gather_rows(a->side_in, nullptr, side0, B, d.M, D, XP_F32, st))) return rc;
  if ((rc = xp_layernorm_fwd_side(a->x, S * D, a->ln1_w, a->ln1_b, a->h1p, D, a->mean1p, a->rstd1p, B, D, d.ln_eps, dt,
                                  side0, nullptr, s1, s1, s1, st))) return rc;
  XpGemmDesc g = gemm_desc(a->h1, static_cast<const char*>(a->Wqkv) + (size_t)D * D * esz, a->kv, rows, 2 * D, D, dt);
  g.epilogue = XP_EPI_BIAS; g.bias = a->bqkv + D;
  if ((rc = xp_gemm(&g, st))) return rc;
  g = gemm_desc(a->h1p, a->Wqkv, a->q, B, D, D, dt);
  g.epilogue = XP_EPI_BIAS_QSCALE; g.bias = a->bqkv; g.scale = d.q_scale; g.scale_cols = D;
  if ((rc = xp_gemm(&g, st))) return rc;
  if ((rc = xp_attn_pooled_fwd(a->q, a->kv, 2 * D, a->attn_o, a->stats, B, d.heads, S, dt, w.attn, w.attn_bytes, st))) return rc;
  return out_proj_mlp_fwd(*a, B, S * D, side0, side_x2, a->side_out, s1, s1, st);
}

extern "C" size_t xp_encoder_layer_pooled_bwd_workspace_bytes(const XpLayerDims* d) {
  if (!d || d->rows <= 0 || d->B <= 0 || d->D <= 0 || d->Dff <= 0 || d->S <= 0 || d->heads <= 0) return 0;
  return carve_pooled_bwd(*d, nullptr, 0).ws.bytes();
}

extern "C" int xp_encoder_layer_pooled_bwd(const XpLayerPooledBwd* a, void* st) {
  XP_REQUIRE(a, "xp_encoder_layer_pooled_bwd: null argument");
  const XpLayerDims& d = a->dims;
  int rc = check_pooled_dims("xp_encoder_layer_pooled_bwd", d);
  if (rc) return rc;
  XP_REQUIRE(a->x && a->h1 && a->kv && a->h1p && a->q && a->attn_o && a->x2 && a->h2 && a->pre && a->act && a->Wqkv && a->Wo &&
             a->W1 && a->W2 && a->ln1_w && a->ln2_w && a->mean1 && a->rstd1 && a->mean1p && a->rstd1p && a->mean2 && a->rstd2 &&
             a->stats && a->dx3 && a->dx, "xp_encoder_layer_pooled_bwd: null pointer");
  XP_REQUIRE((!a->side_in && !a->side_x2) || (a->side_in && a->side_x2 && d.dtype == XP_BF16),
             "xp_encoder_layer_pooled_bwd: side rows need side_in and side_x2, and bf16");
  const PooledBwdWs w = carve_pooled_bwd(d, a->workspace, a->workspace_bytes);
  XP_REQUIRE_WORKSPACE("xp_encoder_layer_pooled_bwd", a, w);
  char* const dqkv = w.dqkv;
  const int64_t rows = d.rows, D = d.D, B = d.B, S = d.S;
  const int dt = d.dtype;
  const bool sided = a->side_in != nullptr;
  const int64_t sS = sided ? S : 0;
  const int32_t sM = sided ? (int32_t)d.M : 0, s1 = sided ? 1 : 0;
  void* dkv = dqkv + (size_t)D * w.t.esz;
  Defer df;
  const WgradOrder wg{rows >= 4096 ? wgrad_side() : nullptr, (hipStream_t)st, "xp_encoder_layer_pooled_bwd"};
  if ((rc = wg.mark(0))) return rc;
  if ((rc = mlp_out_proj_bwd(*a, B, w.t, w.slabs, w.slab_bytes, s1, s1, df, wg, st))) return rc;
  if ((rc = xp_attn_pooled_bwd(a->q, a->kv, 2 * D, a->attn_o, w.t.dattn, a->stats, dqkv, S * 3 * D, dkv, 3 * D, d.q_scale, B, d.heads,
                               S, dt, w.attn, w.attn_bytes, a->dbqkv ? w.cs_kv : nullptr, st))) return rc;
  if ((rc = wg.mark(3))) return rc;
  XpGemmDesc g = gemm_desc(dkv, static_cast<const char*>(a->Wqkv) + (size_t)D * D * w.t.esz, w.dh1, rows, D, 2 * D, dt);
  g.lda = 3 * D; g.b_kstrided = 1; g.ldb = D;
  if ((rc = xp_gemm(&g, st))) return rc;
  g = gemm_desc(dqkv, a->Wqkv, w.dh1, B, D, 3 * D, dt);
  g.a_grp = 1; g.a_grp_stride = S; g.b_kstrided = 1; g.ldb = D; g.c_grp = 1; g.c_grp_stride = S;
  if ((rc = xp_gemm(&g, st))) return rc;
  if (a->dwqkv) {
    g = wgrad_desc(dqkv, 3 * D, a->h1p, D, a->dwqkv, B, D, D, dt);
    g.a_grp = 1; g.a_grp_stride = S;
    if ((rc = run_wgrad(g, w.slabs, w.slab_bytes, wg.stream(), true))) return rc;
    if ((rc = run_wgrad(wgrad_desc(dkv, 3 * D, a->h1, D, a->dwqkv + D * D, rows, 2 * D, D, dt), w.slabs, w.slab_bytes, wg.stream(), false))) return rc;
  }
  if (a->dbqkv) {
    const int64_t kv_rows = xp_attn_pooled_colsum_rows(B, d.heads, S, dt);
    XP_REQUIRE(kv_rows > 0, "xp_encoder_layer_pooled_bwd: no current device");
    if ((rc = xp_colsum_partials(dqkv, B, D, S * 3 * D, dt, w.cs_q, w.cs_q_bytes, st))) return rc;
    df.add(w.cs_q, a->dbqkv, D, (int)w.cs_q_rows, (int)D);
    df.add(w.cs_kv, a->dbqkv + D, 2 * D, (int)kv_rows, (int)(2 * D));
// ... 10 lines not shown
```

xpretrain_amd/functional.py:

```python
from __future__ import annotations

import contextlib
import ctypes as C
import os
import weakref
from typing import Optional, Tuple

import torch

from . import _lib as L
from . import hip_ops as H


class _Entry:
    __slots__ = ("ver", "buf", "refs")

    def __init__(self, ver, buf, refs):
        self.ver, self.buf, self.refs = ver, buf, refs


class WeightCache:

    def __init__(self):
        self._c = {}
        self.generation = 0
        self.structure_version = 0
        self.casts = 0
        self._hooked = False

    def _ensure_hook(self):
        if not self._hooked:
            from torch.optim.optimizer import register_optimizer_step_post_hook

            def hook(opt, args, kwargs):
                after = getattr(opt, "_xp_after_step", None)
                if after is not None:
                    after(self)
                else:
                    self.invalidate()
            register_optimizer_step_post_hook(hook)
            self._hooked = True

    def _ver(self, ws):
        return tuple((w._version, w.data_ptr(), self.generation) for w in ws)

    def invalidate(self, keep=None):
        self.generation += 1
        for key, ent in keep or ():
            if self._c.get(key) is ent:
                ws = [r() for r in ent.refs]
                if all(w is not None for w in ws):
                    ent.ver = self._ver(ws)
                torch.autograd.graph.increment_version(ent.buf)

    @staticmethod
    def _alive(ent, ws) -> bool:
        return ent is not None and all(r() is w for r, w in zip(ent.refs, ws))

    def get(self, w: torch.Tensor, dtype) -> torch.Tensor:
        if dtype == torch.float32:
            return w.detach()
        return self.fused((w,), dtype, _single=True)

    def fused(self, ws, dtype, _single=False) -> torch.Tensor:
        self._ensure_hook()
        key = (tuple(id(w) for w in ws), dtype)
        ver = self._ver(ws)
        ent = self._c.get(key)
        if not self._alive(ent, ws) or ent.ver != ver:
            rows = sum(w.shape[0] for w in ws) if not _single else ws[0].shape[0]
            shape = tuple(ws[0].shape) if _single else (rows,) + tuple(ws[0].shape[1:])
            reuse = ent is not None and tuple(ent.buf.shape) == shape and ent.buf.device == ws[0].device
            if not reuse:
                self.structure_version += 1
            buf = ent.buf if reuse else torch.empty(shape, dtype=dtype, device=ws[0].device)
            if reuse:
                torch.autograd.graph.increment_version(buf)
            self.casts += 1
            if _single:
                H.cast(ws[0].detach(), dtype, out=buf)
            else:
                r = 0
                for w in ws:
                    H.cast(w.detach(), dtype, out=buf[r:r + w.shape[0]])
                    r += w.shape[0]
            ent = _Entry(ver, buf, tuple(weakref.ref(w) for w in ws))
            self._c[key] = ent
        return ent.buf

    def shadow_bindings(self, params):
        ids = {id(p) for p in params}
        shadows, entries = {}, []
        for key, ent in self._c.items():
            ws = [r() for r in ent.refs]
            if any(w is None or id(w) not in ids or id(w) in shadows for w in ws) or not ent.buf.is_contiguous():
                continue
            code = {torch.bfloat16: 0, torch.float32: 1}.get(ent.buf.dtype)
            if code is None:
                continue
            off = 0
            for w in ws:
                shadows[id(w)] = (ent.buf.data_ptr() + off * ent.buf.element_size(), code)
                off += w.numel()
            entries.append((key, ent))
        return shadows, entries

    def clear(self):
        self._c.clear()
        self.structure_version += 1


WEIGHTS = WeightCache()


_SPLITS = {}


def _split_for(n_out: int, n_in: int, rows: int, dtype: torch.dtype, a_remap, slack: bool = False, lddy: Optional[int] = None,
               ldx: Optional[int] = None) -> int:
    lddy, ldx = lddy or n_out, ldx or n_in
    key = (n_out, n_in, rows, dtype, a_remap, slack, lddy, ldx)
    s = _SPLITS.get(key)
    if s is None:
        s = _SPLITS[key] = H.gemm_auto_split(n_out, n_in, rows, dtype, lda=lddy, ldb=ldx, a_remap=a_remap, slack=slack)
    return s


def _wgrad(dy: torch.Tensor, x: torch.Tensor, rows: int, n_out: int, n_in: int, a_remap=(0, 0, 0), slack: bool = False, *,
           lddy: Optional[int] = None, ldx: Optional[int] = None, out: Optional[torch.Tensor] = None) -> torch.Tensor:
    lddy, ldx = lddy or n_out, ldx or n_in
    split = _split_for(n_out, n_in, rows, dy.dtype, tuple(a_remap), slack, lddy, ldx)
    dw = torch.empty((n_out, n_in), dtype=torch.float32, device=dy.device) if out is None else out.view(n_out, n_in)
    if split <= 1:
        H.gemm(dy, x, n_out, n_in, rows, a_kstrided=True, b_kstrided=True, lda=lddy, ldb=ldx, out=dw,
               out_dtype=torch.float32, a_remap=a_remap)
    else:
        ws = H.workspace(split * n_out * n_in * 4, dy.device, "splitk")
        H.gemm(dy, x, n_out, n_in, rows, a_kstrided=True, b_kstrided=True, lda=lddy, ldb=ldx, out=ws,
               split_k=split, a_remap=a_remap)
        H.splitk_reduce(ws, dw, splits=split)
    return dw


LAYER_CALLS = "op_by_op" not in L.DEBUG
_DT_CODE = {torch.bfloat16: L.XP_BF16, torch.float32: L.XP_F32}
_NULLCTX = contextlib.nullcontext()
_ES = {torch.bfloat16: 2, torch.float32: 4}
_PLANS = {}


def set_cu_budget(cus: int) -> None:
    L.check(L.lib().xp_set_cu_budget(int(cus)), "xp_set_cu_budget")
    _SPLITS.clear()
    _PLANS.clear()


def _arena_layout(pieces):
    fill, o = [], 0
    for name, n, bpr in pieces:
        fill.append((name, o, bpr))
        o += (n * bpr + 255) & ~255
    return tuple(fill), o


def _piece_views(plan, arena):
    views = {}
    for (name, n, bpr), (_, o, _) in zip(plan.pieces, plan.fill):
        raw = arena[o:o + n * bpr]
        views[name] = raw.view(torch.float32) if name[:4] in ("mean", "rstd", "stat") else raw.view(plan.dtype).view(n, -1)
    return views


def _finish_plan(plan, dims, dtype, pieces, queries):
    plan.dims, plan.pieces, plan.dtype, plan.side_row = dims, pieces, dtype, dims.D * 4
    plan.rD, plan.size = dims.D * _ES[dtype], (dims.M, dims.N, dims.L) if dims.attn_mode == L.ATTN_PROXY else None
    plan.side_S, plan.side_M = (dims.S, dims.M) if dims.attn_mode == L.ATTN_PROXY else (1, 1)
    plan.fill, plan.arena_bytes = _arena_layout(pieces)
    plan.fwd_ws, plan.bwd_ws = (int(getattr(L.lib(), q)(C.byref(dims))) for q in queries)
    D, Dff = dims.D, dims.Dff
    plan.gsizes = [D, D, 3 * D * D, 3 * D, D * D, D, D, D, Dff * D, Dff, D * Dff, D]
    plan.gnames = ["dln1_w", "dln1_b", "dwqkv", "dbqkv", "dwo", "dbo", "dln2_w", "dln2_b", "dw1", "db1", "dw2", "db2"]
    plan.gtotal = sum(plan.gsizes)


class _LayerPlan:

    def __init__(self, rows, D, Dff, B, S, heads, size, dtype, act=L.ACT_QUICK_GELU):
        d = L.XpLayerDims()
        d.rows, d.D, d.Dff, d.B, d.S, d.heads = rows, D, Dff, B, S, heads
        d.M, d.N, d.L = size if size is not None else (0, 1, S)
        d.attn_mode = L.ATTN_PROXY if size is not None else L.ATTN_CAUSAL
        d.dtype, d.q_scale, d.ln_eps = _DT_CODE[dtype], (D // heads) ** -0.5, 1e-5
        d.act = act
        rD, rF = D * _ES[dtype], Dff * _ES[dtype]
        _finish_plan(self, d, dtype, (("h1", rows, rD), ("qkv", rows, 3 * rD), ("attn_o", rows, rD), ("x2", rows, rD), ("h2", rows, rD),
                                   ("pre", rows, rF), ("act", rows, rF), ("mean1", rows, 4), ("rstd1", rows, 4), ("mean2", rows, 4),
                                   ("rstd2", rows, 4), ("stats", rows, heads * 2 * 4)),
                     ("xp_encoder_layer_fwd_workspace_bytes", "xp_encoder_layer_bwd_workspace_bytes"))


def _layer_plan(rows, D, Dff, B, S, heads, size, dtype, act=L.ACT_QUICK_GELU) -> _LayerPlan:
    key = (rows, D, Dff, B, S, heads, size, dtype, act)
    p = _PLANS.get(key)
    if p is None:
        p = _PLANS[key] = _LayerPlan(*key)
    return p


def _native_ok(x, params, pad_mask) -> bool:
    dev = x.device
    if not x.is_cuda or not x.is_contiguous():
        return False
    for n, t in zip(_FWD_PARAMS, params):
        if t.dtype != (x.dtype if n[0] == "W" else torch.float32) or t.device != dev or not t.is_contiguous():
            return False
    if pad_mask is not None and (pad_mask.dtype != torch.int64 or pad_mask.device != dev or not pad_mask.is_contiguous()):
        return False
    return True


_LATE_UPDATES = weakref.WeakSet()


class LateUpdate:

    def __init__(self, first_layer, owner=None):
        self.first_layer = int(first_layer)
        self.streams = {}
        self.event = None
        self.owner = weakref.ref(owner) if owner is not None else None
        self.encoders = weakref.WeakSet()
        _LATE_UPDATES.add(self)

    @contextlib.contextmanager
    def launch(self, main_stream):
        side = self.streams.get(main_stream.device)
        if side is None:
            side = self.streams[main_stream.device] = torch.cuda.Stream(device=main_stream.device)
        side.wait_stream(main_stream)
        with torch.cuda.stream(side):
            yield side
            ev = torch.cuda.Event()
            ev.record(side)
        self.event = ev

    def _ordered(self) -> bool:
        return self.event is None or torch.cuda.is_current_stream_capturing()

    def wait(self, layer_index, *streams):
        if layer_index != self.first_layer or self._ordered():
            return
        for st in (streams or (torch.cuda.current_stream(),)):
            st.wait_event(self.event)

    def join(self):
        if self._ordered():
            return
        if self.event.query():
            self.event = None
        else:
            torch.cuda.current_stream().wait_event(self.event)

    def attach(self, encoders):
        mine = self.owner() if self.owner is not None else None
        for enc in encoders:
            other = enc.late_update
            if other is not None and other.owner is not None and other.owner() not in (None, mine):
                raise ValueError("overlap_next_forward: this encoder already waits for another optimizer's late update")
        for enc in encoders:
            if enc.late_update is not None:
                enc.late_update.join()
            enc.late_update = self
            self.encoders.add(enc)

    def detach(self):
        self.join()
        for enc in list(self.encoders):
            if enc.late_update is self:
                enc.late_update = None
        self.encoders.clear()

    def __deepcopy__(self, memo):
        return None


def join_late_weights():
    for lu in list(_LATE_UPDATES):
        lu.join()


FWD_SPLIT = os.environ.get("XPRETRAIN_FWD_SPLIT", "1") != "0"
FWD_SPLIT_MIN_ROWS = 8192
FWD_SPLIT_HOLD_BYTES = 48 << 30
FWD_SPLIT_STREAM = "side"
_SPLIT_STREAMS = {}


def second_chain_stream_mode() -> str:
    return "own" if FWD_SPLIT_STREAM == "own" else "side"


def _second_chain_stream(device):
    st = _SPLIT_STREAMS.get(device.index)
    if st is None:
        if second_chain_stream_mode() == "side":
            with torch.cuda.device(device):
                ptr = L.lib().xp_side_stream()
            if ptr:
                st = torch.cuda.ExternalStream(ptr, device=device)
        if st is None:
            st = torch.cuda.Stream(device=device)
        _SPLIT_STREAMS[device.index] = st
    return st


class ForwardSplit:

    def __init__(self, device):
        self.stream = _second_chain_stream(device)
        self.main = torch.cuda.current_stream(device)
        self.stream.wait_stream(self.main)
        self.held = []

    def hold(self, *tensors):
        self.held.extend(t for t in tensors if t is not None)

    def join(self):
        self.main.wait_stream(self.stream)
        self.held.clear()


_FWD_PARAMS = ("ln1_w", "ln1_b", "Wqkv", "bqkv", "Wo", "bo", "ln2_w", "ln2_b", "W1", "b1", "W2", "b2")
_BWD_PARAMS = ("ln1_w", "ln2_w", "Wqkv", "Wo", "W1", "W2")


def _layer_args(struct, plan, dims, names, params, arena, r0=0, keep_pre=True, **tensors):
    a = struct()
    a.dims = dims
    for n, t in zip(names, params):
        setattr(a, n, t.data_ptr())
    base = arena.data_ptr()
    for n, o, bpr in plan.fill:
        setattr(a, n, base + o + r0 * bpr)
    if not keep_pre:
        a.pre = 0
    first = r0 * plan.rD
    for n, t in tensors.items():
        if t is not None:
            setattr(a, n, t.data_ptr() + first)
    return a


def _side_args(a, plan, r0, **sides):
    a.side_S, a.side_M = plan.side_S, plan.side_M
    first = r0 // plan.side_S * plan.side_M * plan.side_row
    for n, t in sides.items():
        if t is not None:
            setattr(a, n, t.data_ptr() + first)


def _call_native(entry, a, ws_bytes, device, ws_tag):
    ws = H.workspace(ws_bytes, device, ws_tag)
    a.workspace, a.workspace_bytes = ws.data_ptr(), ws.numel()
    L.check(getattr(L.lib(), entry)(C.byref(a), H._stream()), entry)


def _layer_fwd_args(plan, dims, x, params, pad_mask, arena, x3, keep_pre, side, side_out, side_x2, r0=0):
    a = _layer_args(L.XpLayerFwd, plan, dims, _FWD_PARAMS, params, arena, r0, keep_pre, x=x, x3=x3)
    a.pad_mask = 0 if pad_mask is None else pad_mask.data_ptr()
    if side is not None:
        _side_args(a, plan, r0, side_in=side, side_out=side_out, side_x2=side_x2)
    return a


def _layer_fwd_native(plan, x, params, pad_mask, arena, x3, keep_pre, side, side_out, side_x2, split):
    dev, d = x.device, plan.dims
    if split is None:
        parts = [(plan, 0, None)]
    else:
        hp = _layer_plan(d.rows // 2, d.D, d.Dff, d.B // 2, d.S, d.heads, (d.M, d.N, d.L), x.dtype, d.act)
        if (d.rows // 2) % 4:
            raise RuntimeError(f"ForwardSplit: (B/2)*S = {d.rows // 2} rows per chain must be a multiple of 4")
        parts = [(hp, 0, None), (hp, d.rows // 2, split.stream)]
    for pl, r0, stream in parts:
        with (torch.cuda.stream(stream) if stream is not None else _NULLCTX):
            a = _layer_fwd_args(plan, pl.dims, x, params, pad_mask, arena, x3, keep_pre, side, side_out, side_x2, r0)
            _call_native("xp_encoder_layer_fwd", a, pl.fwd_ws, dev, "layer_fwd")


GRAD_SINKS = {}
_SINK_CLAIMS = {}


def grad_sink_key(params16):
    return tuple(p.data_ptr() for p in params16)


def _claim_sink(key, sink, numel, device, params):
    if sink is None or sink.numel() != numel or sink.device != device or not all(p.grad is None for p in params):
        return None
    task = torch._C._current_graph_task_id()
    if task < 0 or _SINK_CLAIMS.get(key) == task:
        return None
    _SINK_CLAIMS[key] = task
    return sink


def release_grad_sinks():
    _SINK_CLAIMS.clear()


def layer_grad_groups(model):
    groups = []
    for m in model.modules():
        if all(hasattr(m, a) for a in ("self_attn", "mlp", "layer_norm1", "layer_norm2")):
            a, f = m.self_attn, m.mlp
            groups.append([m.layer_norm1.weight, m.layer_norm1.bias, a.q_proj.weight, a.k_proj.weight, a.v_proj.weight,
                           a.q_proj.bias, a.k_proj.bias, a.v_proj.bias, a.out_proj.weight, a.out_proj.bias,
                           m.layer_norm2.weight, m.layer_norm2.bias, f.fc1.weight, f.fc1.bias, f.fc2.weight, f.fc2.bias])
    return groups


def _record_sink(ctx, ln1_w, ln1_b, wq, bq, wk, bk, wv, bv, wo, bo, ln2_w, ln2_b, w1, b1, w2, b2):
    if GRAD_SINKS:
        ctx.sink_params = (ln1_w, ln1_b, wq, wk, wv, bq, bk, bv, wo, bo, ln2_w, ln2_b, w1, b1, w2, b2)
        ctx.sink_key = grad_sink_key(ctx.sink_params)
    else:
        ctx.sink_params, ctx.sink_key = (), None


def _qkv_grads(dwqkv, dbqkv, need, D):
    pick = lambda t, i, ok: t[i * D:(i + 1) * D] if (t is not None and ok) else None
    return (pick(dwqkv, 0, need[3]), pick(dbqkv, 0, need[4]), pick(dwqkv, 1, need[5]), pick(dbqkv, 1, need[6]),
            pick(dwqkv, 2, need[7]), pick(dbqkv, 2, need[8]))


def _layer_backward(ctx, build, entry, ws_tag, ops, x, *rest):
    plan, dev, need = ctx.plan, x.device, ctx.needs_input_grad
    flat = None
    if GRAD_SINKS and ctx.sink_key is not None and all(need[1:17]):
        flat = _claim_sink(ctx.sink_key, GRAD_SINKS.get(ctx.sink_key), plan.gtotal, dev, ctx.sink_params)
    if flat is None:
        flat = torch.empty(plan.gtotal, dtype=torch.float32, device=dev)
    want = dict(dln1_w=need[1], dln1_b=need[2], dwqkv=need[3] or need[5] or need[7], dbqkv=need[4] or need[6] or need[8],
                dwo=need[9], dbo=need[10], dln2_w=need[11], dln2_b=need[12], dw1=need[13], db1=need[14], dw2=need[15], db2=need[16])
    g = {name: t for name, t in zip(plan.gnames, flat.split_with_sizes(plan.gsizes)) if want[name]}
    dx = torch.empty_like(x)
    if ctx.native:
        _call_native(entry, build(plan, x, *rest, dx, g), plan.bwd_ws, dev, ws_tag)
    else:
        ops(plan, x, *rest, dx, g)
    D, Dff = plan.dims.D, plan.dims.Dff
    gw = lambda n, shape: g[n].view(shape) if n in g else None
    return (dx, g.get("dln1_w"), g.get("dln1_b"), *_qkv_grads(gw("dwqkv", (3 * D, D)), g.get("dbqkv"), need, D),
            gw("dwo", (D, D)), g.get("dbo"), g.get("dln2_w"), g.get("dln2_b"),
            gw("dw1", (Dff, D)), g.get("db1"), gw("dw2", (D, Dff)), g.get("db2"))


def _layer_bwd_args(plan, x, params, arena, dx3, pad_mask, side, side_x2, dx, grads):
    a = _layer_args(L.XpLayerBwd, plan, plan.dims, _BWD_PARAMS, params, arena, x=x, dx3=dx3, dx=dx, **grads)
    a.pad_mask = 0 if pad_mask is None else pad_mask.data_ptr()
    if side is not None and side_x2 is not None:
        _side_args(a, plan, 0, side_in=side, side_x2=side_x2)
    return a


def _attn_front_ops(v, x, ln1_w, ln1_b, Wqkv, bqkv, B, S, heads, size, pad_mask, side, lns):
    rows, D = x.shape
    h1, _, _ = H.layernorm_fwd(x, ln1_w, ln1_b, rows, D, x_side=side, side=lns, y=v.get("h1"), mean=v.get("mean1"), rstd=v.get("rstd1"))
    qkv = H.gemm(h1, Wqkv, rows, 3 * D, D, epilogue=L.EPI_BIAS_QSCALE, bias=bqkv, scale=64 ** -0.5, scale_cols=D, out=v.get("qkv"))
    _, stats = H.attn_fwd(qkv, B, S, heads, size=size, pad_mask=pad_mask, out=v.get("attn_o"), stats=v.get("stats"))
    return qkv, stats


def _mlp_fwd_ops(v, p, x, ldr, n, training, side_x, side_x2, side_out, sd, x3, act):
    D, Dff = p["Wo"].shape[0], p["W1"].shape[0]
    lns = None if sd is None else (sd[0], sd[1], sd[1])
    x2 = H.gemm(v["attn_o"], p["Wo"], n, D, D, epilogue=L.EPI_BIAS_RESID, bias=p["bo"].detach(), resid=x, ldr=ldr, out=v["x2"],
                resid_side=side_x, out_side=side_x2, side=sd)
    h2, _, _ = H.layernorm_fwd(x2, p["ln2_w"], p["ln2_b"], n, D, x_side=side_x2, side=lns, y=v["h2"], mean=v["mean2"], rstd=v["rstd2"])
    a = H.gemm(h2, p["W1"], n, Dff, D, epilogue=L.EPI_ACT_FWD[act], bias=p["b1"].detach(), aux=v["pre"] if training else None,
               out=v["act"])
    H.gemm(a, p["W2"], n, D, Dff, epilogue=L.EPI_BIAS_RESID, bias=p["b2"].detach(), resid=x2, out=x3,
           resid_side=side_x2, out_side=side_out, side=sd)


def _mlp_bwd_ops(v, p, g, dx3, n, defer, db1_fused, side_x2, lns, act):
    D, Dff = p["Wo"].shape[0], p["W1"].shape[0]
    epi = L.EPI_ACT_BWD[act]
    if "db1" in g and db1_fused:
        dpre, _ = H.gemm(dx3, p["W2"], n, Dff, D, b_kstrided=True, epilogue=epi, resid=v["pre"], colsum_defer=defer,
                         colsum_name="db1", colsum_out=g["db1"])
    else:
        dpre = H.gemm(dx3, p["W2"], n, Dff, D, b_kstrided=True, epilogue=epi, resid=v["pre"])
        if "db1" in g:
            H.colsum_deferred(dpre, n, Dff, defer, name="db1", out=g["db1"])
    if "dw2" in g:
        _wgrad(dx3, v["act"], n, D, Dff, slack=True, out=g["dw2"])
    dh2 = H.gemm(dpre, p["W1"], n, D, Dff, b_kstrided=True)
    if "dw1" in g:
        _wgrad(dpre, v["h2"], n, Dff, D, slack=True, out=g["dw1"])
    dx2 = H.layernorm_bwd(dh2, v["x2"], p["ln2_w"], v["mean2"], v["rstd2"], n, D, dres=dx3, defer=defer, dx_colsum=True,
                          dres_colsum=True, name="ln2", x_side=side_x2, side=lns, dgamma=g.get("dln2_w"), dbeta=g.get("dln2_b"),
                          dx_colsum_out=g.get("dbo"), dres_colsum_out=g.get("db2"))[0]
    dattn = H.gemm(dx2, p["Wo"], n, D, D, b_kstrided=True)
    if "dwo" in g:
        _wgrad(dx2, v["attn_o"], n, D, D, slack=True, out=g["dwo"])
    return dx2, dattn


def _layer_fwd_ops(plan, x, params, pad_mask, arena, x3, training, side, side_out, side_x2):
    d = plan.dims
    v, p = _piece_views(plan, arena), dict(zip(_FWD_PARAMS, params))
    sd, lns = (None, None) if side is None else ((plan.side_S, plan.side_M), (plan.side_S, plan.side_M, plan.side_M))
    if side is not None and side_x2 is None:
        side_x2 = torch.empty_like(side)
    _attn_front_ops(v, x, p["ln1_w"], p["ln1_b"], p["Wqkv"], p["bqkv"], d.B, d.S, d.heads, plan.size, pad_mask, side, lns)
    _mlp_fwd_ops(v, p, x, None, d.rows, training, side, side_x2, side_out, sd, x3, d.act)


def _layer_bwd_ops(plan, x, params, arena, dx3, pad_mask, side, side_x2, dx, g):
    d = plan.dims
    rows, D = d.rows, d.D
    v, p = _piece_views(plan, arena), dict(zip(_BWD_PARAMS, params))
    lns = None if side is None else (plan.side_S, plan.side_M, plan.side_M)
    defer = H.DeferredReduce(x.device)
    dx2, dattn = _mlp_bwd_ops(v, p, g, dx3, rows, defer, True, side_x2, lns, d.act)
    dbqkv = g.get("dbqkv")
    dqkv = H.attn_bwd(v["qkv"], v["attn_o"], dattn, v["stats"], d.B, d.S, d.heads, size=plan.size, pad_mask=pad_mask,
                      q_scale=64 ** -0.5, colsum_defer=None if dbqkv is None else defer, colsum_name="dbqkv", colsum_out=dbqkv)
    dqkv = dqkv if dbqkv is None else dqkv[0]
    dh1 = H.gemm(dqkv, p["Wqkv"], rows, D, 3 * D, b_kstrided=True)
    if "dwqkv" in g:
        _wgrad(dqkv, v["h1"], rows, 3 * D, D, out=g["dwqkv"])
    H.layernorm_bwd(dh1, x, p["ln1_w"], v["mean1"], v["rstd1"], rows, D, dres=dx2, dx=dx, defer=defer, name="ln1", x_side=side,
                    side=lns, dgamma=g.get("dln1_w"), dbeta=g.get("dln1_b"))
    defer.flush()


def _check_layer_args(name, x, heads, act, side, side_rows, side_what):
    if act not in (L.ACT_QUICK_GELU, L.ACT_GELU):
        raise ValueError(f"{name}: act={act!r} is not one of {L.ACTS}")
    if side is not None and (x.dtype != torch.bfloat16 or side.dtype != torch.float32 or not side.is_contiguous() or side.device != x.device
                             or tuple(side.shape) != (side_rows, x.shape[1])):
        raise TypeError(f"{name}: side rows must be a contiguous fp32 {side_what} tensor beside a bf16 stream")
    if x.shape[1] // heads != 64:
        raise RuntimeError(f"xpretrain_amd attention kernels are built for head_dim 64, got {x.shape[1] // heads}")


def _compute_weights(dt, wq, bq, wk, bk, wv, bv, wo, w1, w2):
    get = WEIGHTS.get
    return WEIGHTS.fused((wq, wk, wv), dt), WEIGHTS.fused((bq, bk, bv), torch.float32), get(wo, dt), get(w1, dt), get(w2, dt)


def _layer_outputs(ctx, x3, side_out):
    if side_out is None:
        return x3
    ctx.mark_non_differentiable(side_out)
    ctx.set_materialize_grads(False)
    return x3, side_out


def _check_dx3(name, dx3, x, shape):
    if dx3.dtype != x.dtype or dx3.device != x.device or tuple(dx3.shape) != tuple(shape):
        raise TypeError(f"{name}.backward: incoming gradient is {dx3.dtype} {tuple(dx3.shape)} on {dx3.device}, "
                        f"expected {x.dtype} {tuple(shape)} on {x.device}")
    return dx3.contiguous()


class EncoderLayerFn(torch.autograd.Function):

    @staticmethod
    def forward(ctx, x, ln1_w, ln1_b, wq, bq, wk, bk, wv, bv, wo, bo, ln2_w, ln2_b, w1, b1, w2, b2,
                B: int, S: int, heads: int, size: Optional[Tuple[int, int, int]], pad_mask: Optional[torch.Tensor],
                training: bool = True, side: Optional[torch.Tensor] = None, split: Optional["ForwardSplit"] = None,
                act: int = L.ACT_QUICK_GELU):
        dt = x.dtype
        _check_layer_args("EncoderLayerFn", x, heads, act, side, B * size[0] if size is not None else B * S,
                          "[B*M, D] (video) / [B*S, D] (text)")
        rows, D = x.shape
        Dff = w1.shape[0]
        casts0 = WEIGHTS.casts
        Wqkv, bqkv, Wo, W1, W2 = _compute_weights(dt, wq, bq, wk, bk, wv, bv, wo, w1, w2)
        params = (ln1_w, ln1_b, Wqkv, bqkv, Wo, bo, ln2_w, ln2_b, W1, b1, W2, b2)
        plan = _layer_plan(rows, D, Dff, B, S, heads, size, dt, act)
        arena = torch.empty(plan.arena_bytes, dtype=torch.uint8, device=x.device)
        x3 = torch.empty_like(x)
        side_out = None if side is None else torch.empty_like(side)
        side_x2 = torch.empty_like(side) if side is not None and training else None
        ctx.plan, ctx.native = plan, LAYER_CALLS and _native_ok(x, params, pad_mask)
        if ctx.native:
            if split is not None and (size is None or B % 2 or pad_mask is not None):
                split = None
            if split is not None and WEIGHTS.casts != casts0:
                split.stream.wait_stream(torch.cuda.current_stream())
            _layer_fwd_native(plan, x, params, pad_mask, arena, x3, training, side, side_out, side_x2, split)
            if split is not None:
                split.hold(x, arena, x3, side, side_out, side_x2)
        else:
            _layer_fwd_ops(plan, x, params, pad_mask, arena, x3, training, side, side_out, side_x2)
        ctx.save_for_backward(x, arena, ln1_w, ln2_w, Wqkv, Wo, W1, W2, pad_mask, side, side_x2)
        _record_sink(ctx, ln1_w, ln1_b, wq, bq, wk, bk, wv, bv, wo, bo, ln2_w, ln2_b, w1, b1, w2, b2)
        return _layer_outputs(ctx, x3, side_out)

    @staticmethod
    def backward(ctx, dx3, _dside=None):
        if dx3 is None:
            return (None,) * 26
        x, arena, *params, pad_mask, side, side_x2 = ctx.saved_tensors
        dx3 = _check_dx3("EncoderLayerFn", dx3, x, x.shape)
        return _layer_backward(ctx, _layer_bwd_args, "xp_encoder_layer_bwd", "layer_bwd", _layer_bwd_ops, x, params, arena, dx3,
                               pad_mask, side, side_x2) + (None,) * 9


class _PooledLayerPlan:

    def __init__(self, rows, D, Dff, B, S, heads, size, dtype, act=L.ACT_QUICK_GELU):
        rD, rF = D * _ES[dtype], Dff * _ES[dtype]
        _finish_plan(self, _layer_plan(rows, D, Dff, B, S, heads, size, dtype, act).dims, dtype,
                     (("h1", rows, rD), ("kv", rows, 2 * rD), ("mean1", rows, 4), ("rstd1", rows, 4), ("h1p", B, rD), ("q", B, rD),
                      ("attn_o", B, rD), ("x2", B, rD), ("h2", B, rD), ("pre", B, rF), ("act", B, rF), ("mean1p", B, 4),
                      ("rstd1p", B, 4), ("mean2", B, 4), ("rstd2", B, 4), ("stats", B, heads * 2 * 4)),
                     ("xp_encoder_layer_pooled_fwd_workspace_bytes", "xp_encoder_layer_pooled_bwd_workspace_bytes"))


def _pooled_plan(rows, D, Dff, B, S, heads, size, dtype, act=L.ACT_QUICK_GELU) -> _PooledLayerPlan:
    key = ("pooled", rows, D, Dff, B, S, heads, size, dtype, act)
    p = _PLANS.get(key)
    if p is None:
        p = _PLANS[key] = _PooledLayerPlan(rows, D, Dff, B, S, heads, size, dtype, act)
    return p


def _pooled_fwd_args(plan, x, params, arena, x3, keep_pre, side, side_out, side_x2):
    return _layer_args(L.XpLayerPooledFwd, plan, plan.dims, _FWD_PARAMS, params, arena, keep_pre=keep_pre, x=x, x3=x3,
                       side_in=side, side_out=side_out, side_x2=side_x2)


def _pooled_bwd_args(plan, x, params, arena, dx3, side, side_x2, dx, grads):
    return _layer_args(L.XpLayerPooledBwd, plan, plan.dims, _BWD_PARAMS, params, arena, x=x, dx3=dx3, dx=dx, side_in=side,
                       side_x2=side_x2, **grads)


def _pooled_fwd_ops(plan, x, params, arena, x3, training, side, side_out, side_x2):
    d = plan.dims
    rows, D, B, S, M = d.rows, d.D, d.B, d.S, d.M
    v, p = _piece_views(plan, arena), dict(zip(_FWD_PARAMS, params))
    Wqkv, bqkv = p["Wqkv"], p["bqkv"]
    lns, p1, sd = (None, None, None) if side is None else ((S, M, M), (1, 1, 1), (1, 1))
    h1, _, _ = H.layernorm_fwd(x, p["ln1_w"], p["ln1_b"], rows, D, x_side=side, side=lns, y=v["h1"], mean=v["mean1"], rstd=v["rstd1"])
    side0 = None if side is None else H.gather_rows(side, None, B, M, D)
    h1p, _, _ = H.layernorm_fwd(x, p["ln1_w"], p["ln1_b"], B, D, ldx=S * D, x_side=side0, side=p1, y=v["h1p"], mean=v["mean1p"],
                                rstd=v["rstd1p"])
    kv = H.gemm(h1, Wqkv[D:], rows, 2 * D, D, epilogue=L.EPI_BIAS, bias=bqkv[D:], out=v["kv"])
    q = H.gemm(h1p, Wqkv, B, D, D, epilogue=L.EPI_BIAS_QSCALE, bias=bqkv, scale=64 ** -0.5, scale_cols=D, out=v["q"])
    H.attn_pooled_fwd(q, kv, B, S, d.heads, out=v["attn_o"], stats=v["stats"])
    _mlp_fwd_ops(v, p, x, S * D, B, training, side0, side_x2, side_out, sd, x3, d.act)


def _pooled_bwd_ops(plan, x, params, arena, dx3, side, side_x2, dx, g):
    d = plan.dims
    rows, D, B, S, M = d.rows, d.D, d.B, d.S, d.M
    v, p = _piece_views(plan, arena), dict(zip(_BWD_PARAMS, params))
    Wqkv, dbqkv = p["Wqkv"], g.get("dbqkv")
    lns, p1 = (None, None) if side is None else ((S, M, M), (1, 1, 1))
    defer = H.DeferredReduce(x.device)
    dx2, dattn = _mlp_bwd_ops(v, p, g, dx3, B, defer, False, side_x2, p1, d.act)
    dqkv = torch.empty((rows, 3 * D), dtype=x.dtype, device=x.device)
    dq_view, dkv = dqkv.view(B, S * 3 * D)[:, :D], dqkv[:, D:]
    H.attn_pooled_bwd(v["q"], v["kv"], v["attn_o"], dattn, v["stats"], B, S, d.heads, q_scale=64 ** -0.5, dq=dq_view, dkv=dkv,
                      colsum_defer=None if dbqkv is None else defer, colsum_name="dbkv", colsum_out=None if dbqkv is None else dbqkv[D:])
    dh1 = H.gemm(dkv, Wqkv[D:], rows, D, 2 * D, lda=3 * D, b_kstrided=True, ldb=D)
    H.gemm(dqkv, Wqkv, B, D, 3 * D, b_kstrided=True, ldb=D, a_remap=(1, S, 0), c_remap=(1, S, 0), out=dh1)
    if "dwqkv" in g:
        dwqkv = g["dwqkv"].view(3 * D, D)
        _wgrad(dqkv, v["h1p"], B, D, D, a_remap=(1, S, 0), slack=True, lddy=3 * D, out=dwqkv[:D])
        _wgrad(dkv, v["h1"], rows, 2 * D, D, lddy=3 * D, out=dwqkv[D:])
    if dbqkv is not None:
        H.colsum_deferred(dqkv, B, D, defer, ldx=S * 3 * D, name="dbq", out=dbqkv)
    H.layernorm_bwd(dh1, x, p["ln1_w"], v["mean1"], v["rstd1"], rows, D, dx=dx, defer=defer, name="ln1", x_side=side, side=lns,
                    dgamma=g.get("dln1_w"), dbeta=g.get("dln1_b"))
    H.layernorm_bwd(dh1, x, p["ln1_w"], v["mean1p"], v["rstd1p"], B, D, ldx=S * D, lddy=S * D, dres=dx2, dx=dx, lddx=S * D, defer=defer,
                    param_grads=False, name="ln1_pooled", x_side=side, side=(1, 1, M))
    defer.flush()


class PooledEncoderLayerFn(torch.autograd.Function):

    @staticmethod
    def forward(ctx, x, ln1_w, ln1_b, wq, bq, wk, bk, wv, bv, wo, bo, ln2_w, ln2_b, w1, b1, w2, b2,
                B: int, S: int, heads: int, size: Tuple[int, int, int], training: bool = True, side: Optional[torch.Tensor] = None,
                act: int = L.ACT_QUICK_GELU):
        dt = x.dtype
        rows, D = x.shape
        M = size[0]
        _check_layer_args("PooledEncoderLayerFn", x, heads, act, side, B * M, "[B*M, D]")
        Dff = w1.shape[0]
        if M < 1 or S != M + size[1] * size[2] or rows != B * S:
            raise RuntimeError(f"PooledEncoderLayerFn: token 0 must be a proxy row of a [B*S, D] stream (size={size}, S={S}, rows={rows})")
        Wqkv, bqkv, Wo, W1, W2 = _compute_weights(dt, wq, bq, wk, bk, wv, bv, wo, w1, w2)
        dev = x.device
        x3 = torch.empty((B, D), dtype=dt, device=dev)
        side_out = side_x2 = None
        if side is not None:
            side_out = torch.empty((B, D), dtype=torch.float32, device=dev)
            side_x2 = torch.empty((B, D), dtype=torch.float32, device=dev)
        params = (ln1_w, ln1_b, Wqkv, bqkv, Wo, bo, ln2_w, ln2_b, W1, b1, W2, b2)
        plan = _pooled_plan(rows, D, Dff, B, S, heads, tuple(size), dt, act)
        arena = torch.empty(plan.arena_bytes, dtype=torch.uint8, device=dev)
        ctx.plan, ctx.native = plan, LAYER_CALLS and _native_ok(x, params, None)
        if ctx.native:
            a = _pooled_fwd_args(plan, x, params, arena, x3, training, side, side_out, side_x2)
            _call_native("xp_encoder_layer_pooled_fwd", a, plan.fwd_ws, dev, "layer_pooled_fwd")
        else:
            _pooled_fwd_ops(plan, x, params, arena, x3, training, side, side_out, side_x2)
        ctx.save_for_backward(x, arena, ln1_w, ln2_w, Wqkv, Wo, W1, W2, side, side_x2)
        _record_sink(ctx, ln1_w, ln1_b, wq, bq, wk, bk, wv, bv, wo, bo, ln2_w, ln2_b, w1, b1, w2, b2)
        return _layer_outputs(ctx, x3, side_out)

    @staticmethod
    def backward(ctx, dx3, _dside=None):
        if dx3 is None:
            return (None,) * 24
        x, arena, *params, side, side_x2 = ctx.saved_tensors
        dx3 = _check_dx3("PooledEncoderLayerFn", dx3, x, (ctx.plan.dims.B, x.shape[1]))
        return _layer_backward(ctx, _pooled_bwd_args, "xp_encoder_layer_pooled_bwd", "layer_pooled_bwd", _pooled_bwd_ops, x, params,
                               arena, dx3, side, side_x2) + (None,) * 7


def pooled_encoder_layer(x, layer, B, S, heads, size, side=None):
    return PooledEncoderLayerFn.apply(x, *_layer_params(layer), B, S, heads, tuple(size), torch.is_grad_enabled(), side, _layer_act(layer))


PROXY_SIDE = os.environ.get("XPRETRAIN_PROXY_FP32", "1") != "0"


def proxy_side_rows(class_emb, added_cls, pos_w, B: int, M: int) -> torch.Tensor:
    D = class_emb.shape[0]
    side = torch.empty((B * M, D), dtype=torch.float32, device=class_emb.device)
    return H.vip_proxy_rows(class_emb.detach(), added_cls.detach().contiguous(), pos_w.detach().contiguous(), side, B, M, M, D)


def with_side_rows(x: torch.Tensor, side: Optional[torch.Tensor], B: int, S: int) -> torch.Tensor:
    if side is None:
        return x
    D = x.shape[1]
    h = x.detach().float()
    h.view(B, S, D)[:, :side.shape[0] // B] = side.view(B, -1, D)
    return h


PATCH_GATHER = True


class VisionEmbedFn(torch.autograd.Function):

    @staticmethod
    def forward(ctx, video, patch_w, class_emb, added_cls, pos_w, time_table, dtype, want_wgrad=True):
        Bv, T, Cc, Hh, Ww = video.shape
        D, _, P, _ = patch_w.shape
        gh, gw = Hh // P, Ww // P
        Lp = gh * gw
        M = 1 + added_cls.shape[0]
        S = M + T * Lp
        if pos_w.shape[0] != 1 + Lp:
            raise ValueError(f"position_embedding has {pos_w.shape[0]} rows but the frame has {Lp} patches (+1)")
        K = 3 * P * P
        frames = video.reshape(Bv * T, Cc, Hh, Ww).contiguous()
        if frames.dtype != torch.uint8:
            frames = frames.float()
        Wp = WEIGHTS.get(patch_w, dtype).view(D, K)
        x = torch.empty((Bv * S, D), dtype=dtype, device=video.device)
        pos = pos_w.detach().contiguous()
        tt = time_table.detach().contiguous().float()
        need_patches = bool(want_wgrad) and ctx.needs_input_grad[1]
        on_the_fly = (not need_patches and PATCH_GATHER and dtype == torch.bfloat16 and P % 8 == 0 and Ww % 8 == 0)
        patches = None
        if on_the_fly:
            H.gemm(None, Wp, Bv * T * Lp, D, K, out=x, epilogue=L.EPI_PATCH, tab1=tt, tab2=pos[1:], tab_L=Lp, c_remap=(T * Lp, S, M),
                   frames=frames, frame_patch=P, frame_norm=(H.CLIP_MEAN, H.CLIP_STD) if frames.dtype == torch.uint8 else None)
        else:
            if frames.dtype == torch.uint8:
                patches = H.im2col_u8(frames, P, dtype)
            else:
                patches = H.im2col(frames, P, dtype)
            H.gemm(patches, Wp, Bv * T * Lp, D, K, out=x, epilogue=L.EPI_PATCH, tab1=tt, tab2=pos[1:], tab_L=Lp,
                   c_remap=(T * Lp, S, M))
        H.vip_proxy_rows(class_emb.detach(), added_cls.detach().contiguous(), pos, x, Bv, S, M, D)
        ctx.save_for_backward(patches)
        ctx.meta = (Bv, T, Lp, M, S, D, K, tuple(patch_w.shape), added_cls.shape[0])
        return x

    @staticmethod
    def backward(ctx, dx):
        (patches,) = ctx.saved_tensors
        Bv, T, Lp, M, S, D, K, wshape, nadd = ctx.meta
        dx = dx.contiguous()
        d_class, d_added, d_pos, d_time = H.vip_embed_bwd(dx, Bv, M, T, Lp, D)
        dwp = None if patches is None else _wgrad(dx, patches, Bv * T * Lp, D, K, a_remap=(T * Lp, S, M)).view(wshape)
        return None, dwp, d_class, d_added[:nadd], d_pos, d_time, None, None


class PosResampleFn(torch.autograd.Function):

    @staticmethod
    def forward(ctx, pos_w, gh, gw):
        ctx.meta = (H.pos_grid(pos_w.shape[0]), gh, gw)
        return H.pos_resample_fwd(pos_w.detach().contiguous(), gh, gw)

    @staticmethod
    def backward(ctx, d_out):
        return H.pos_resample_bwd(d_out.contiguous(), *ctx.meta), None, None


def pos_table(pos_w, gh: int, gw: int):
    if gh < 1 or gw < 1:
        raise ValueError(f"interpolate_pos_encoding: the frame is smaller than one patch (grid {gh} x {gw})")
    g0 = H.pos_grid(pos_w.shape[0])
    return pos_w if gh == gw == g0 else PosResampleFn.apply(pos_w, gh, gw)


class TextEmbedFn(torch.autograd.Function):

    @staticmethod
    def forward(ctx, ids, tok_w, pos_w, dtype):
        ids = ids.contiguous()
        x = H.text_embed_fwd(ids, tok_w.detach(), pos_w.detach(), dtype)
        ctx.save_for_backward(ids)
        ctx.meta = (tok_w.shape[0], pos_w.shape[0])
        return x

    @staticmethod
    def backward(ctx, dx):
        (ids,) = ctx.saved_tensors
        d_tok, d_pos = H.text_embed_bwd(ids, dx.contiguous(), *ctx.meta)
        return None, d_tok, d_pos, None


class LayerNormFn(torch.autograd.Function):

    @staticmethod
    def forward(ctx, x, gamma, beta, x_side=None, side=None, want_y_side=False):
        rows, D = x.shape
        y_side = torch.empty_like(x_side) if want_y_side else None
        y, mean, rstd = H.layernorm_fwd(x, gamma.detach(), beta.detach(), rows, D, x_side=x_side, y_side=y_side, side=side)
        ctx.save_for_backward(x, gamma, mean, rstd, x_side)
        ctx.side = side
        if want_y_side:
            ctx.mark_non_differentiable(y_side)
            ctx.set_materialize_grads(False)
            return y, y_side
        return y

    @staticmethod
    def backward(ctx, dy, _dys=None):
        if dy is None:
            return (None,) * 6
        x, gamma, mean, rstd, x_side = ctx.saved_tensors
        rows, D = x.shape
        dx, dg, db = H.layernorm_bwd(dy.contiguous(), x, gamma.detach(), mean, rstd, rows, D, x_side=x_side, side=ctx.side)
        return dx, dg, db, None, None, None


class GatherRowsFn(torch.autograd.Function):

    @staticmethod
    def forward(ctx, x, idx, B, S):
        D = x.shape[1]
        ctx.save_for_backward(idx)
        ctx.meta = (B, S, D)
        return H.gather_rows(x, idx, B, S, D)

    @staticmethod
    def backward(ctx, dout):
        (idx,) = ctx.saved_tensors
        B, S, D = ctx.meta
        return H.scatter_rows(dout.contiguous(), idx, B, S, D), None, None, None


class ProjectionFn(torch.autograd.Function):

    @staticmethod
    def forward(ctx, x, w):
        rows, K = x.shape
        N = w.shape[0]
        Wc = WEIGHTS.get(w, x.dtype)
        ctx.save_for_backward(x, Wc)
        return H.gemm(x, Wc, rows, N, K)

    @staticmethod
    def backward(ctx, dy):
        x, Wc = ctx.saved_tensors
        rows, K = x.shape
        N = Wc.shape[0]
        dy = dy.contiguous()
        dx = H.gemm(dy, Wc, rows, K, N, b_kstrided=True)
        dw = _wgrad(dy, x, rows, N, K)
        return dx, dw


class L2NormFn(torch.autograd.Function):

    @staticmethod
    def forward(ctx, x):
        rows, D = x.shape
        y, inv = H.l2norm_fwd(x, rows, D)
        ctx.save_for_backward(y, inv)
        ctx.dtype = x.dtype
        return y

    @staticmethod
    def backward(ctx, dy):
        y, inv = ctx.saved_tensors
        rows, D = y.shape
        return H.l2norm_bwd(dy.contiguous().float(), y, inv, rows, D, ctx.dtype)


def _sim(a: torch.Tensor, b: torch.Tensor) -> torch.Tensor:
    a, b = a.contiguous().float(), b.contiguous().float()
    out = torch.empty((a.shape[0], b.shape[0]), dtype=torch.float32, device=a.device)
    L.check(L.lib().xp_sim_matrix(H._p(a), H._p(b), H._p(out), a.shape[0], b.shape[0], a.shape[1], H._stream()), "xp_sim_matrix")
    return out


class SimLogitsFn(torch.autograd.Function):

    @staticmethod
    def forward(ctx, text, image, log_scale):
        scale = log_scale.detach().float().exp()
        logits = _sim(text, image) * scale
        ctx.save_for_backward(text, image, logits, scale)
        return logits

    @staticmethod
    def backward(ctx, g):
        text, image, logits, scale = ctx.saved_tensors
        g = g.contiguous().float()
        gs = g * scale
        dt = _sim(gs, image.float().t()).to(text.dtype) if ctx.needs_input_grad[0] else None
        di = _sim(gs.t(), text.float().t()).to(image.dtype) if ctx.needs_input_grad[1] else None
        dls = (g * logits).sum().reshape(()) if ctx.needs_input_grad[2] else None
        return dt, di, dls


class NCELossFn(torch.autograd.Function):

    @staticmethod
    def forward(ctx, vis, txt, log_scale):
        loss, dv, dt, dls = H.nce_loss(vis.contiguous().float(), txt.contiguous().float(),
                                       log_scale.detach().float().reshape(()))
        ctx.save_for_backward(dv, dt, dls)
        return loss

    @staticmethod
    def backward(ctx, g):
        dv, dt, dls = ctx.saved_tensors
        return dv * g, dt * g, dls * g


class VscFcLossFn(torch.autograd.Function):

    @staticmethod
    def forward(ctx, vis, txt, img, cap, log_scale):
        loss, *grads = H.vsc_fc_loss(vis.contiguous().float(), txt.contiguous().float(), img.contiguous().float(),
                                     cap.contiguous().float(), log_scale.detach().float().reshape(()))
        ctx.save_for_backward(*grads)
        return loss

    @staticmethod
    def backward(ctx, g):
        return tuple(t * g for t in ctx.saved_tensors)


class ContrastiveLossFn(torch.autograd.Function):

    @staticmethod
    def forward(ctx, kind, vis, txt, img, cap, log_scale):
        def f(t):
            return None if t is None else t.contiguous().float()
        loss, *grads = H.contrastive_loss(kind, f(vis), f(txt), f(img), f(cap), log_scale=log_scale.detach().float().reshape(()))
        ctx.has = [g is not None for g in grads]
        ctx.save_for_backward(*[g for g in grads if g is not None])
        return loss

    @staticmethod
    def backward(ctx, g):
        saved = iter(ctx.saved_tensors)
        return (None, *[next(saved) * g if h else None for h in ctx.has])


class PairLossFn(torch.autograd.Function):

    @staticmethod
    def forward(ctx, kind, vis, txt, params):
        loss, dv, dt = H.pair_loss(kind, vis.contiguous().float(), txt.contiguous().float(), **params)
        ctx.save_for_backward(dv, dt)
        return loss

    @staticmethod
    def backward(ctx, g):
        dv, dt = ctx.saved_tensors
        return None, dv * g, dt * g, None


def _layer_params(layer):
    cached = layer.__dict__.get("_xp_mods")
    if cached is not None:
        mods, tabs = cached
        lm = layer._modules
        a, m = lm["self_attn"]._modules, lm["mlp"]._modules
        live = (lm["layer_norm1"], a["q_proj"], a["k_proj"], a["v_proj"], a["out_proj"], lm["layer_norm2"], m["fc1"], m["fc2"])
        for x, y, t in zip(live, mods, tabs):
            if x is not y or x._parameters is not t:
                cached = None
                break
    if cached is None:
        a, m = layer.self_attn, layer.mlp
        mods = (layer.layer_norm1, a.q_proj, a.k_proj, a.v_proj, a.out_proj, layer.layer_norm2, m.fc1, m.fc2)
        tabs = tuple(x._parameters for x in mods)
        layer.__dict__["_xp_mods"] = (mods, tabs)
    return tuple(d[k] for d in tabs for k in ("weight", "bias"))


def _layer_act(layer) -> int:
    return layer._modules["mlp"].__dict__.get("act_kind", L.ACT_QUICK_GELU)


def layer_attentions(x, layer, B, S, size, pad_mask, side=None):
    ln1_w, ln1_b, wq, bq, wk, bk, wv, bv = _layer_params(layer)[:8]
    heads = layer.num_heads
# ... 13 lines not shown
```

xpretrain_amd/hip_ops.py:

```python
from __future__ import annotations

import ctypes as C
import math
from typing import NamedTuple, Optional

import torch

from . import _lib as L

_DT = {torch.bfloat16: L.XP_BF16, torch.float32: L.XP_F32}


def _stream():
    return C.c_void_p(torch.cuda.current_stream().cuda_stream)


def _p(t: Optional[torch.Tensor]):
    return C.c_void_p(0 if t is None else t.data_ptr())


def _dt(t: torch.Tensor) -> int:
    try:
        return _DT[t.dtype]
    except KeyError:
        raise TypeError(f"unsupported dtype {t.dtype}; xpretrain_amd computes in bfloat16 or float32")


def _chk(t: torch.Tensor, name: str, dtype=None):
    if not t.is_cuda:
        raise RuntimeError(f"{name}: expected a GPU tensor -- xpretrain_amd has no CPU path")
    if dtype is not None and t.dtype != dtype:
        raise TypeError(f"{name}: expected {dtype}, got {t.dtype}")
    return t


_ws_cache = {}


def workspace(nbytes: int, device, tag: str = "ws") -> torch.Tensor:
    key = (device.index if device.index is not None else torch.cuda.current_device(),
           torch.cuda.current_stream().cuda_stream, tag)
    buf = _ws_cache.get(key)
    if buf is None or buf.numel() < nbytes:
        buf = torch.empty(max(int(nbytes), 1 << 20), dtype=torch.uint8, device=device)
        _ws_cache[key] = buf
    return buf


def gemm(A: torch.Tensor, B: torch.Tensor, M: int, N: int, K: int, *, lda=None, ldb=None, out=None, ldc=None,
         a_kstrided=False, b_kstrided=False, out_dtype=None, epilogue=L.EPI_NONE, bias=None, scale=1.0,
         scale_cols=0, resid=None, ldr=None, aux=None, ldaux=None, tab1=None, tab2=None, tab_L=0,
         a_remap=(0, 0, 0), c_remap=(0, 0, 0), split_k=1, out_rows=None, colsum_defer=None, colsum_name="gemm_colsum",
         colsum_out=None, resid_side=None, out_side=None, side=None, frames=None, frame_patch=0, frame_norm=None, plan_only=False):
    if frames is not None:
        _chk(frames, "frames"); _chk(B, "B", torch.bfloat16)
        if A is not None or frames.dim() != 4 or frames.shape[1] != 3 or not frames.is_contiguous() or \
                frames.dtype not in (torch.float32, torch.uint8) or (frames.dtype == torch.uint8 and frame_norm is None):
            raise TypeError("gemm: frames must be a contiguous [BT,3,H,W] fp32 / uint8 (with frame_norm) tensor and A must be None")
        A = B
    else:
        _chk(A, "A"); _chk(B, "B", A.dtype)
    out_dtype = out_dtype or A.dtype
    if split_k > 1:
        out = torch.empty((split_k, M, N), dtype=torch.float32, device=A.device) if out is None else out
        out_dtype = torch.float32
    elif out is None:
        out = torch.empty((out_rows or M, N), dtype=out_dtype, device=A.device)
    d = L.XpGemmDesc()
    d.A, d.B, d.C = (0 if frames is not None else A.data_ptr()), B.data_ptr(), out.data_ptr()
    if frames is not None:
        d.a_frames, d.a_frames_u8 = frames.data_ptr(), int(frames.dtype == torch.uint8)
        d.fr_H, d.fr_W, d.fr_P = frames.shape[2], frames.shape[3], int(frame_patch)
        if frame_norm is not None:
            for c in range(3):
                d.fr_mean[c], d.fr_std[c] = float(frame_norm[0][c]), float(frame_norm[1][c])
    d.M, d.N, d.K = M, N, K
    d.lda = lda if lda is not None else (M if a_kstrided else K)
    d.ldb = ldb if ldb is not None else (N if b_kstrided else K)
    d.ldc = ldc if ldc is not None else N
    d.a_kstrided, d.b_kstrided = int(a_kstrided), int(b_kstrided)
    d.in_dtype, d.out_dtype = _dt(A), _DT[out_dtype]
    d.epilogue, d.split_k = epilogue, split_k
    d.a_grp, d.a_grp_stride, d.a_off = a_remap
    d.c_grp, d.c_grp_stride, d.c_off = c_remap
    d.bias = 0 if bias is None else _chk(bias, "bias", torch.float32).data_ptr()
    d.scale, d.scale_cols = float(scale), scale_cols
    d.resid = 0 if resid is None else _chk(resid, "resid", A.dtype).data_ptr()
    d.ldr = ldr if ldr is not None else N
    d.aux = 0 if aux is None else _chk(aux, "aux", out_dtype).data_ptr()
    d.ldaux = ldaux if ldaux is not None else N
    d.tab1 = 0 if tab1 is None else _chk(tab1, "tab1", torch.float32).data_ptr()
    d.tab2 = 0 if tab2 is None else _chk(tab2, "tab2", torch.float32).data_ptr()
    d.tab_L = tab_L
    if resid_side is not None or out_side is not None:
        _chk(resid_side, "resid_side", torch.float32); _chk(out_side, "out_side", torch.float32)
        S_, M_ = side
        need = ((M - 1) // S_ * M_ + min(M_, S_)) * N
        if not (resid_side.is_contiguous() and out_side.is_contiguous()) or resid_side.numel() < need or out_side.numel() < need:
            raise ValueError("gemm: resid_side / out_side are too small or not contiguous")
        d.resid_side, d.out_side, d.side_S, d.side_M = resid_side.data_ptr(), out_side.data_ptr(), S_, M_
    if plan_only:
        if colsum_defer is not None and L.lib().xp_gemm_colsum_rows(C.byref(d)) > 0:
            d.colsum_partials = 1
        return gemm_plan_of(d)
    nrows = L.lib().xp_gemm_colsum_rows(C.byref(d)) if colsum_defer is not None else 0
    if nrows:
        part = colsum_defer.slot(nrows * N * 4, colsum_name)
        d.colsum_partials = part.data_ptr()
    L.check(L.lib().xp_gemm(C.byref(d), _stream()), "xp_gemm")
    if colsum_defer is None:
        return out
    if not nrows:
        return out, colsum_deferred(out, M, N, colsum_defer, ldx=d.ldc, name=colsum_name, out=colsum_out)
    cs = torch.empty(N, dtype=torch.float32, device=A.device) if colsum_out is None else colsum_out
    colsum_defer.add(part, 0, cs, nrows, N, N)
    return out, cs


def gemm_plan_of(d: L.XpGemmDesc) -> dict:
    info = L.XpGemmPlanInfo()
    L.check(L.lib().xp_debug_gemm_plan(C.byref(d), C.byref(info)), "xp_debug_gemm_plan")
    return {f: (tuple(getattr(info, f)) if f == "grid" else getattr(info, f)) for f, _ in info._fields_ if f != "reserved"}


def gemm_auto_split(M: int, N: int, K: int, dtype: torch.dtype, *, a_kstrided=True, b_kstrided=True, lda=None,
                    ldb=None, a_remap=(0, 0, 0), slack=False) -> int:
    d = L.XpGemmDesc()
    d.M, d.N, d.K = M, N, K
    d.lda = lda if lda is not None else (M if a_kstrided else K)
    d.ldb = ldb if ldb is not None else (N if b_kstrided else K)
    d.ldc = N
    d.a_kstrided, d.b_kstrided = int(a_kstrided), int(b_kstrided)
    d.in_dtype, d.out_dtype = _DT[dtype], _DT[torch.float32]
    d.a_grp, d.a_grp_stride, d.a_off = a_remap
    return int((L.lib().xp_gemm_auto_split_slack if slack else L.lib().xp_gemm_auto_split)(C.byref(d)))


def splitk_reduce(slabs: torch.Tensor, out: torch.Tensor, accumulate=False, splits=None) -> torch.Tensor:
    n = out.numel()
    if splits is None:
        if slabs.dtype != torch.float32:
            raise TypeError("splitk_reduce: pass `splits` explicitly when the slab buffer is an untyped workspace")
        splits = slabs.numel() // n
    L.check(L.lib().xp_splitk_reduce(_p(slabs), _p(out), n, splits, int(accumulate), _stream()),
            "xp_splitk_reduce")
    return out


def colsum(X: torch.Tensor, rows: int, cols: int, ldx=None, out=None, accumulate=False) -> torch.Tensor:
    _chk(X, "X")
    out = torch.empty(cols, dtype=torch.float32, device=X.device) if out is None else out
    nb = L.lib().xp_colsum_workspace_bytes(rows, cols)
    ws = workspace(nb, X.device, "colsum")
    L.check(L.lib().xp_colsum(_p(X), rows, cols, ldx or cols, _dt(X), _p(out), int(accumulate), _p(ws), ws.numel(),
                              _stream()), "xp_colsum")
    return out


class DeferredReduce:

    def __init__(self, device):
        self.device = device
        self.segs = []
        self._keep = []
        self._names = set()

    def add(self, part: torch.Tensor, part_offset: int, out: torch.Tensor, nrows: int, width: int, stride: int,
            accumulate=False):
        sg = L.XpReduceSeg()
        sg.in_ = part.data_ptr() + 4 * part_offset
        sg.out = out.data_ptr()
        sg.stride, sg.nrows, sg.width, sg.accumulate = stride, nrows, width, int(accumulate)
        self.segs.append(sg)
        self._keep.append((part, out))

    def slot(self, nbytes: int, name: str) -> torch.Tensor:
        if name in self._names:
            raise RuntimeError(f"DeferredReduce: two producers named {name!r} before flush()")
        self._names.add(name)
        return workspace(nbytes, self.device, "defer:" + name)

    def flush(self):
        if not self.segs:
            return
        lib = L.lib()
        for i in range(0, len(self.segs), L.XP_REDUCE_MAX_SEGS):
            chunk = self.segs[i:i + L.XP_REDUCE_MAX_SEGS]
            arr = (L.XpReduceSeg * len(chunk))(*chunk)
            nb = lib.xp_reduce_rows_batch_workspace_bytes(arr, len(chunk))
            ws = workspace(nb, self.device, "reduce_batch")
            L.check(lib.xp_reduce_rows_batch(arr, len(chunk), _p(ws), ws.numel(), _stream()), "xp_reduce_rows_batch")
        self.segs, self._keep, self._names = [], [], set()


def colsum_deferred(X: torch.Tensor, rows: int, cols: int, defer: DeferredReduce, ldx=None, name="colsum", out=None,
                    accumulate=False) -> torch.Tensor:
    _chk(X, "X")
    out = torch.empty(cols, dtype=torch.float32, device=X.device) if out is None else out
    chunks = L.lib().xp_colsum_partial_rows(rows, cols)
    part = defer.slot(chunks * cols * 4, name)
    L.check(L.lib().xp_colsum_partials(_p(X), rows, cols, ldx or cols, _dt(X), _p(part), part.numel(), _stream()),
            "xp_colsum_partials")
    defer.add(part, 0, out, chunks, cols, cols, accumulate)
    return out


def layernorm_fwd(x: torch.Tensor, gamma: torch.Tensor, beta: torch.Tensor, rows: int, cols: int, ldx=None,
                  eps: float = 1e-5, x_side=None, y_side=None, side=None, ldy=None, y=None, mean=None, rstd=None):
    _chk(x, "x"); _chk(gamma, "gamma", torch.float32); _chk(beta, "beta", torch.float32)
    ldy = ldy or cols
    if y is None:
        y = torch.empty((rows, ldy), dtype=x.dtype, device=x.device)
    else:
        _chk(y, "y", x.dtype)
        if not y.is_contiguous() or y.numel() < (rows - 1) * ldy + cols:
            raise ValueError("layernorm_fwd: y is too small or not contiguous")
    for t, nm in ((mean, "mean"), (rstd, "rstd")):
        if t is not None:
            _chk(t, nm, torch.float32)
            if not t.is_contiguous() or t.numel() < rows:
                raise ValueError(f"layernorm_fwd: {nm} is too small or not contiguous")
    mean = torch.empty(rows, dtype=torch.float32, device=x.device) if mean is None else mean
    rstd = torch.empty(rows, dtype=torch.float32, device=x.device) if rstd is None else rstd
    if x_side is None and y_side is None:
        L.check(L.lib().xp_layernorm_fwd(_p(x), ldx or cols, _p(gamma), _p(beta), _p(y), ldy, _p(mean), _p(rstd),
                                         rows, cols, eps, _dt(x), _stream()), "xp_layernorm_fwd")
    else:
        S, M, stride = side
        for t, nm in ((x_side, "x_side"), (y_side, "y_side")):
            if t is not None:
                _chk(t, nm, torch.float32)
                if not t.is_contiguous() or t.numel() < ((rows - 1) // S * stride + min(M, S)) * cols:
                    raise ValueError(f"layernorm_fwd: {nm} is too small or not contiguous")
        L.check(L.lib().xp_layernorm_fwd_side(_p(x), ldx or cols, _p(gamma), _p(beta), _p(y), ldy, _p(mean), _p(rstd),
                                              rows, cols, eps, _dt(x), _p(x_side), _p(y_side), S, M, stride, _stream()),
                "xp_layernorm_fwd_side")
    return y, mean, rstd


def layernorm_bwd(dy, x, gamma, mean, rstd, rows, cols, *, ldx=None, lddy=None, dres=None, dx=None, lddx=None,
                  dgamma=None, dbeta=None, accumulate=False, defer: "DeferredReduce" = None, dx_colsum=False, dres_colsum=False,
                  name="ln", x_side=None, side=None, param_grads=True, lddres=None, dx_colsum_out=None, dres_colsum_out=None):
    _chk(dy, "dy"); _chk(x, "x", dy.dtype)
    S, M, stride = side if x_side is not None else (0, 0, 0)
    if x_side is not None:
        _chk(x_side, "x_side", torch.float32)
        if not x_side.is_contiguous() or x_side.numel() < ((rows - 1) // S * stride + min(M, S)) * cols:
            raise ValueError("layernorm_bwd: x_side is too small or not contiguous")
    if not param_grads and (defer is None or dx_colsum or dres_colsum):
        raise ValueError("layernorm_bwd: param_grads=False needs a DeferredReduce and no column sums")
    dx = torch.empty((rows, cols), dtype=dy.dtype, device=dy.device) if dx is None else dx
    if param_grads:
        dgamma = torch.empty(cols, dtype=torch.float32, device=dy.device) if dgamma is None else dgamma
        dbeta = torch.empty(cols, dtype=torch.float32, device=dy.device) if dbeta is None else dbeta
    nb = L.lib().xp_layernorm_bwd_workspace_bytes(rows, cols)
    if defer is not None:
        ws = defer.slot(nb, name)
        L.check(L.lib().xp_layernorm_bwd_partials_side(_p(dy), lddy or cols, _p(x), ldx or cols, _p(gamma), _p(mean), _p(rstd),
                                                       _p(dres), lddres or cols, _p(dx), lddx or cols, 2 if dres_colsum else int(dx_colsum),
                                                       rows, cols, _dt(dy), _p(x_side), S, M, stride, _p(ws), ws.numel(), _stream()),
                "xp_layernorm_bwd_partials_side")
        if not param_grads:
            return dx, None, None
        nrows = L.lib().xp_layernorm_bwd_partial_rows(rows)
        if dres_colsum and not (dx_colsum and dres is not None):
            raise ValueError("layernorm_bwd: dres_colsum needs dx_colsum and dres")
        pitch = (4 if dres_colsum else 3 if dx_colsum else 2) * cols
        defer.add(ws, 0, dgamma, nrows, cols, pitch, accumulate)
        defer.add(ws, cols, dbeta, nrows, cols, pitch, accumulate)
        if dx_colsum:
            dxs = torch.empty(cols, dtype=torch.float32, device=dy.device) if dx_colsum_out is None else dx_colsum_out
            defer.add(ws, 2 * cols, dxs, nrows, cols, pitch)
            if dres_colsum:
                drs = torch.empty(cols, dtype=torch.float32, device=dy.device) if dres_colsum_out is None else dres_colsum_out
                defer.add(ws, 3 * cols, drs, nrows, cols, pitch)
# ... 596 lines not shown
```

Before: 565.0 pairs/s.

## Skip zero rows in last-layer backward via listed M/K tile GEMMs

When the upstream gradient of the last encoder layer comes from a CLS-only row gather (scatter_rows with no index), it is tagged as supported on a single row per sample. The backward then runs listed GEMM variants that compute only the M tiles and K tiles containing nonzero rows. Outputs are zero-filled first and the weight-gradient GEMMs iterate only the listed k-tiles. This cuts wasted GEMM work on mostly-zero gradients in exchange for extra kernel variants, memsets, and host-side bookkeeping through a weakref claim registry.

```diff
diff --git a/include/xpretrain_hip.h b/include/xpretrain_hip.h
--- a/include/xpretrain_hip.h
+++ b/include/xpretrain_hip.h
@@ -49,6 +49,8 @@
   int32_t side_M;
   const float* resid_side; float* out_side; int64_t side_S;
   const void* a_frames; int32_t a_frames_u8; int32_t fr_H, fr_W, fr_P; float fr_mean[3], fr_std[3];
+  const int32_t* m_tiles; int32_t n_m_tiles; int32_t reserved1;
+  const int32_t* k_tiles; const int32_t* k_tile_begin; const int32_t* k_tile_begin_host;
 } XpGemmDesc;
 
 int xp_gemm(const XpGemmDesc* desc, void* stream);
@@ -314,6 +316,11 @@
 size_t xp_encoder_layer_fwd_workspace_bytes(const XpLayerDims* dims);
 int xp_encoder_layer_fwd(const XpLayerFwd* args, void* stream);
 
+typedef struct XpDx3Support {
+  const int32_t* m_tiles; int32_t n_m_tiles; int32_t reserved;
+  const int32_t* k_tiles[3]; const int32_t* k_tile_begin[3]; const int32_t* k_tile_begin_host[3];
+  int32_t split[3]; int32_t reserved1;
+} XpDx3Support;
 typedef struct XpLayerBwd {
   XpLayerDims dims;
   const void* x; const void* h1; const void* qkv; const void* attn_o; const void* x2; const void* h2; const void* pre;
@@ -329,6 +336,7 @@
 } XpLayerBwd;
 size_t xp_encoder_layer_bwd_workspace_bytes(const XpLayerDims* dims);
 int xp_encoder_layer_bwd(const XpLayerBwd* args, void* stream);
+int xp_encoder_layer_bwd_listed(const XpLayerBwd* args, const XpDx3Support* dx3_support, void* stream);
 typedef struct XpLayerPooledFwd {
   XpLayerDims dims;
   const void* x; const void* Wqkv; const void* Wo; const void* W1; const void* W2;
diff --git a/xpretrain_amd/csrc/gemm.hip b/xpretrain_amd/csrc/gemm.hip
--- a/xpretrain_amd/csrc/gemm.hip
+++ b/xpretrain_amd/csrc/gemm.hip
@@ -562,7 +562,31 @@
   if (split > 1) XP_REQUIRE(ep == XP_EPI_NONE && d->out_dtype == XP_F32 && d->c_grp == 0 && d->ldc == d->N,
                             "xp_gemm: split_k needs EPI_NONE, f32 output, dense C");
 
-  const GemmPlan plan = plan_gemm(d, split);
+  GemmPlan plan = plan_gemm(d, split);
+  const bool mlist = d->m_tiles || d->n_m_tiles, klist = d->k_tiles || d->k_tile_begin || d->k_tile_begin_host;
+  if (mlist || klist) {
+    XP_REQUIRE(plan.family == Family::G256, "xp_gemm: tile lists need a 256-wide-family plan (xp_debug_gemm_plan)");
+    XP_REQUIRE(d->a_grp == 0 && d->c_grp == 0 && !d->a_frames, "xp_gemm: tile lists take no row remap and no a_frames");
+    XP_REQUIRE(!(mlist && klist), "xp_gemm: m_tiles and k_tiles are for different operand layouts");
+    if (mlist) {
+      XP_REQUIRE(!d->a_kstrided && d->b_kstrided && split == 1, "xp_gemm: m_tiles is for the dX form (A k-contiguous, B k-strided, no split-K)");
+      XP_REQUIRE(d->m_tiles && d->n_m_tiles >= 1 && d->n_m_tiles <= plan.tiles_m && (uintptr_t)d->m_tiles % 4 == 0,
+                 "xp_gemm: m_tiles needs 1..%d entries, got %d", plan.tiles_m, d->n_m_tiles);
+      plan.grid = dim3(d->n_m_tiles * plan.tiles_n, 1, 1);
+    } else {
+      XP_REQUIRE(d->a_kstrided && d->b_kstrided && ep == XP_EPI_NONE, "xp_gemm: k_tiles is for the dW form (both operands k-strided, EPI_NONE)");
+      XP_REQUIRE(d->k_tiles && d->k_tile_begin && d->k_tile_begin_host && ((uintptr_t)d->k_tiles | (uintptr_t)d->k_tile_begin) % 4 == 0,
+                 "xp_gemm: k_tiles needs k_tile_begin and k_tile_begin_host");
+      const int32_t* kb = d->k_tile_begin_host;
+      XP_REQUIRE(kb[0] >= 0, "xp_gemm: k_tile_begin_host[0] is negative");
+      for (int z = 0; z < split; ++z) {
+        const int64_t k0 = (int64_t)z * plan.k_per_split, k1 = k0 + plan.k_per_split < d->K ? k0 + plan.k_per_split : d->K;
+        const int64_t n = (int64_t)kb[z + 1] - kb[z];
+        XP_REQUIRE(n >= 2 && n <= cdiv(k1 - k0, 64), "xp_gemm: slab %d lists %lld k-tiles, needs 2..%lld", z, (long long)n,
+                   (long long)cdiv(k1 - k0, 64));
+      }
+    }
+  }
   KParams kp;
   kp.A = d->A; kp.B = d->B; kp.C = d->C;
   kp.M = d->M; kp.N = d->N; kp.K = d->K; kp.lda = d->lda; kp.ldb = d->ldb; kp.ldc = d->ldc;
@@ -580,6 +604,9 @@
   kp.tiles_m = plan.tiles_m; kp.tiles_n = plan.tiles_n; kp.group_n = plan.group_n; kp.xcd_remap = plan.xcd_remap;
   kp.flat_split = plan.flat_split; kp.wide = plan.wide; kp.fast_epi = plan.fast_epi;
   kp.colsum = d->colsum_partials;
+  if (mlist || klist) {
+    kp.m_tiles = d->m_tiles; kp.n_m_tiles = d->n_m_tiles; kp.k_tiles = d->k_tiles; kp.k_tile_begin = d->k_tile_begin;
+  }
   kp.rside = d->resid_side; kp.oside = d->out_side; kp.side_S = (unsigned)d->side_S; kp.side_M = (unsigned)d->side_M;
   if (d->resid_side || d->out_side)
     XP_REQUIRE(d->resid_side && d->out_side && ep == XP_EPI_BIAS_RESID && d->out_dtype == d->in_dtype && d->c_grp == 0 &&
diff --git a/xpretrain_amd/csrc/gemm256.hip b/xpretrain_amd/csrc/gemm256.hip
--- a/xpretrain_amd/csrc/gemm256.hip
+++ b/xpretrain_amd/csrc/gemm256.hip
@@ -82,12 +82,15 @@
 template <bool AKS, bool BKS, typename... Act>
 __global__ __launch_bounds__(NTH, 2) void gemm256_kernel(KParams p) {
   constexpr int ACT = ActOf<Act...>::value;
+  constexpr bool LISTED = HasTag<TileListTag, Act...>::value;
+  constexpr bool MLIST = LISTED && !AKS, KLIST = LISTED && AKS;
   extern __shared__ __attribute__((aligned(16))) char smem[];
   const int tid = threadIdx.x, lane = tid & 63;
   const int wave = __builtin_amdgcn_readfirstlane(tid >> 6);
   const int wm = wave / WAVES_N, wn = wave % WAVES_N;
 
-  const int nwg = p.tiles_m * p.tiles_n;
+  const int rows_m = MLIST ? p.n_m_tiles : p.tiles_m;
+  const int nwg = rows_m * p.tiles_n;
   int bid, zs, nsplit;
   if (p.flat_split > 0) {
     const int l = xcd_remap(blockIdx.x, nwg * p.flat_split, 1);
@@ -96,12 +99,29 @@
     bid = xcd_remap(blockIdx.x, nwg, p.xcd_remap); zs = blockIdx.z; nsplit = gridDim.z;
   }
   int tm, tn;
-  tile_of(bid, p.tiles_m, p.tiles_n, p.group_n, tm, tn);
+  tile_of(bid, rows_m, p.tiles_n, p.group_n, tm, tn);
+  if constexpr (MLIST) {
+    tm = p.m_tiles[tm];
+    if ((unsigned)tm >= (unsigned)p.tiles_m) return;
+  }
   const int64_t m0 = (int64_t)tm * TM, n0 = (int64_t)tn * TN;
 
-  const int64_t kbeg = (int64_t)zs * p.k_per_split;
-  const int64_t kend = (kbeg + p.k_per_split < p.K) ? kbeg + p.k_per_split : p.K;
-  const int nk = (int)((kend - kbeg + KE - 1) / KE);
+  const int64_t kslab = (int64_t)zs * p.k_per_split;
+  const int64_t kend = (kslab + p.k_per_split < p.K) ? kslab + p.k_per_split : p.K;
+  const int64_t kbeg = KLIST ? 0 : kslab;
+  const int* klist = nullptr;
+  int nk;
+  if constexpr (KLIST) {
+    const int b0 = p.k_tile_begin[zs];
+    klist = p.k_tiles + b0;
+    nk = p.k_tile_begin[zs + 1] - b0;
+  } else {
+    nk = (int)((kend - kbeg + KE - 1) / KE);
+  }
+  auto phys = [&](int t) -> int {
+    if constexpr (KLIST) return t < nk ? __builtin_amdgcn_readfirstlane(klist[t]) : 0;
+    else return t;
+  };
 
   HalfStager<AKS, 64> ga;
   HalfStager<BKS, 32> gb;
@@ -122,8 +142,12 @@
 
   auto slot = [&](int kt, int w) -> char* { return smem + (((kt & 1) << 2) + w) * HALF_BYTES; };
 
-  gb.issue(slot(1, 3), 0, 0);
-  ga.issue(slot(0, 0), 0, 0); gb.issue(slot(0, 1), 1, 0); ga.issue(slot(0, 2), 1, 0); gb.issue(slot(0, 3), 0, 1);
+  int kc1 = phys(1), kc2 = phys(2);
+  auto next1 = [&](int t) -> int { if constexpr (KLIST) return kc1; else return t + 1; };
+  auto next2 = [&](int t) -> int { if constexpr (KLIST) return kc2; else return t + 2; };
+  const int kfirst = phys(0);
+  gb.issue(slot(1, 3), 0, kfirst);
+  ga.issue(slot(0, 0), 0, kfirst); gb.issue(slot(0, 1), 1, kfirst); ga.issue(slot(0, 2), 1, kfirst); gb.issue(slot(0, 3), 0, next1(0));
   wait_vmcnt<4>();
   __builtin_amdgcn_s_barrier();
   if (wm == 1) __builtin_amdgcn_s_barrier();
@@ -153,6 +177,7 @@
     _Pragma("unroll") for (int nt = 0; nt < 2; ++nt) DST[ks][nt] = frag<BKS>(TILE, wn * 2 + nt, ks, lane)
 
   XP_READ_B(fbn, slot(1, 3));
+  if constexpr (KLIST) asm volatile("s_waitcnt lgkmcnt(0)" ::: "memory");
 
   auto ktile = [&](int t, auto tail_c) {
     constexpr int TAIL = decltype(tail_c)::value;
@@ -164,17 +189,18 @@
     __builtin_amdgcn_sched_barrier(0);
     XP_READ_A(slot(t, 0));
     __builtin_amdgcn_sched_barrier(0);
-    if constexpr (TAIL <= 1) { ga.issue(slot(t + 1, 0), 0, t + 1); gb.issue(slot(t + 1, 1), 1, t + 1); }
+    if constexpr (TAIL <= 1) { ga.issue(slot(t + 1, 0), 0, next1(t)); gb.issue(slot(t + 1, 1), 1, next1(t)); }
     wait_vmcnt<(TAIL <= 1 ? 4 : 0)>();
     XP_PHASE_MMA(0);
     if constexpr (TAIL <= 1) { XP_READ_B(fbn, slot(t, 3)); }
     __builtin_amdgcn_sched_barrier(0);
     XP_READ_A(slot(t, 2));
     __builtin_amdgcn_sched_barrier(0);
-    if constexpr (TAIL <= 1) ga.issue(slot(t + 1, 2), 1, t + 1);
-    if constexpr (TAIL == 0) gb.issue(slot(t + 1, 3), 0, t + 2);
+    if constexpr (TAIL <= 1) ga.issue(slot(t + 1, 2), 1, next1(t));
+    if constexpr (TAIL == 0) gb.issue(slot(t + 1, 3), 0, next2(t));
     wait_vmcnt<(TAIL == 0 ? 4 : (TAIL == 1 ? 2 : 0))>();
     XP_PHASE_MMA(1);
+    if constexpr (KLIST && TAIL == 0) { kc1 = kc2; kc2 = phys(t + 3); }
   };
   for (int t = 0; t < nk - 2; ++t) ktile(t, std::integral_constant<int, 0>{});
   ktile(nk - 2, std::integral_constant<int, 1>{});
@@ -258,12 +284,14 @@
   if (tline) { asm volatile("s_waitcnt vmcnt(0)" ::: "memory"); tr[64 + bid * 4 + 2] = __builtin_amdgcn_s_memrealtime(); }
 }
 
-template <bool AKS, bool BKS>
-bool launch_one(int act, const KParams& kp, dim3 grid, hipStream_t st) {
-  auto kern = act == XP_ACT_GELU ? gemm256_kernel<AKS, BKS, GeluErfTag> : gemm256_kernel<AKS, BKS>;
+bool launch_kernel(void (*kern)(KParams), const KParams& kp, dim3 grid, hipStream_t st) {
   if (!xp_device_cus(reinterpret_cast<const void*>(kern), LDS_BYTES)) return false;
   kern<<<grid, NTH, LDS_BYTES, st>>>(kp);
   return true;
+}
+template <bool AKS, bool BKS, typename... List>
+bool launch_one(int act, const KParams& kp, dim3 grid, hipStream_t st) {
+  return launch_kernel(act == XP_ACT_GELU ? gemm256_kernel<AKS, BKS, GeluErfTag, List...> : gemm256_kernel<AKS, BKS, List...>, kp, grid, st);
 }
 
 template __global__ void gemm256_kernel<false, false>(KParams);
@@ -274,6 +302,9 @@
 template __global__ void gemm256_kernel<false, true, GeluErfTag>(KParams);
 template __global__ void gemm256_kernel<true, true, GeluErfTag>(KParams);
 template __global__ void gemm256_kernel<true, false, GeluErfTag>(KParams);
+template __global__ void gemm256_kernel<false, true, TileListTag>(KParams);
+template __global__ void gemm256_kernel<false, true, GeluErfTag, TileListTag>(KParams);
+template __global__ void gemm256_kernel<true, true, TileListTag>(KParams);
 
 }
 
@@ -297,6 +328,8 @@
 
 bool xp_gemm256_launch(const XpGemmDesc* d, const xpgemm::KParams& kp, dim3 grid, hipStream_t st) {
   const int act = xpgemm::epi_act(d->epilogue);
+  if (d->m_tiles) return launch_one<false, true, xpgemm::TileListTag>(act, kp, grid, st);
+  if (d->k_tiles) return launch_kernel(gemm256_kernel<true, true, xpgemm::TileListTag>, kp, grid, st);
   if (!d->a_kstrided && !d->b_kstrided)      return launch_one<false, false>(act, kp, grid, st);
   else if (!d->a_kstrided && d->b_kstrided)  return launch_one<false, true>(act, kp, grid, st);
   else if (d->a_kstrided && d->b_kstrided)   return launch_one<true, true>(act, kp, grid, st);
diff --git a/xpretrain_amd/csrc/gemm_common.h b/xpretrain_amd/csrc/gemm_common.h
--- a/xpretrain_amd/csrc/gemm_common.h
+++ b/xpretrain_amd/csrc/gemm_common.h
@@ -19,8 +19,9 @@
 }
 
 struct GeluErfTag {};
-template <typename... Tag> struct ActOf { static constexpr int value = XP_ACT_QUICK_GELU; };
-template <> struct ActOf<GeluErfTag> { static constexpr int value = XP_ACT_GELU; };
+struct TileListTag {};
+template <typename T, typename... Tag> struct HasTag { static constexpr bool value = (std::is_same<T, Tag>::value || ...); };
+template <typename... Tag> struct ActOf { static constexpr int value = HasTag<GeluErfTag, Tag...>::value ? XP_ACT_GELU : XP_ACT_QUICK_GELU; };
 
 struct KParams {
   const void* A; const void* B; void* C;
@@ -41,7 +42,13 @@
   const float* rside; float* oside; unsigned side_S, side_M;
   unsigned long long* dbg;
   int flat_split;
-  const void* im_src; int im_u8, im_H, im_W, im_P, im_gw, im_L; float im_mean[3], im_std[3];
+  union {
+    struct { const void* im_src; int im_u8, im_H, im_W, im_P, im_gw, im_L; float im_mean[3], im_std[3]; };
+    struct {
+      const int* m_tiles; int n_m_tiles;
+      const int* k_tiles; const int* k_tile_begin;
+    };
+  };
 };
 
 
diff --git a/xpretrain_amd/csrc/layer.hip b/xpretrain_amd/csrc/layer.hip
--- a/xpretrain_amd/csrc/layer.hip
+++ b/xpretrain_amd/csrc/layer.hip
@@ -40,8 +40,13 @@
   d.a_kstrided = d.b_kstrided = 1; d.lda = lddy; d.ldb = ldx; d.out_dtype = XP_F32;
   return d;
 }
-int run_wgrad(XpGemmDesc d, float* slabs, size_t slab_bytes, void* st, bool slack) {
+int run_wgrad(XpGemmDesc d, float* slabs, size_t slab_bytes, void* st, bool slack, const XpDx3Support* sup = nullptr, int w = 0) {
   const int split = slack ? xp_gemm_auto_split_slack(&d) : xp_gemm_auto_split(&d);
+  if (sup) {
+    XP_REQUIRE(sup->split[w] == (split > 1 ? split : 1), "encoder layer backward: dx3_support lists weight gradient %d for split %d, "
+               "the library plans %d", w, sup->split[w], split);
+    d.k_tiles = sup->k_tiles[w]; d.k_tile_begin = sup->k_tile_begin[w]; d.k_tile_begin_host = sup->k_tile_begin_host[w];
+  }
   if (split <= 1) return xp_gemm(&d, st);
   XP_REQUIRE(slab_bytes >= (size_t)split * d.M * d.N * sizeof(float), "encoder layer backward: split-K slab space too small");
   float* dw = (float*)d.C;
@@ -164,24 +169,35 @@
 
 template <class Args>
 int mlp_out_proj_bwd(const Args& a, int64_t n, const TailBwd& t, float* slabs, size_t slab_bytes, int64_t sS,
-                     int32_t sM, Defer& df, const WgradOrder& wg, void* st) {
+                     int32_t sM, Defer& df, const WgradOrder& wg, void* st, const XpDx3Support* sup = nullptr) {
   const int64_t D = a.dims.D, Dff = a.dims.Dff;
   const int dt = a.dims.dtype;
   int rc;
+  auto listed = [&](XpGemmDesc& g, void* fill, size_t bytes) -> int {
+    if (!sup) return XP_OK;
+    g.m_tiles = sup->m_tiles; g.n_m_tiles = sup->n_m_tiles;
+    if (fill && hipMemsetAsync(fill, 0, bytes, (hipStream_t)st) != hipSuccess) {
+      xp_set_error("%s: zero fill in front of a listed GEMM failed", wg.name);
+      return XP_ERR_LAUNCH;
+    }
+    return XP_OK;
+  };
   XpGemmDesc g = gemm_desc(a.dx3, a.W2, t.dpre, n, Dff, D, dt);
   g.b_kstrided = 1; g.ldb = Dff; g.epilogue = epi_act_bwd(a.dims); g.resid = a.pre; g.ldr = Dff;
   if (a.db1 && t.db1_fused_rows > 0) g.colsum_partials = t.cs_pre;
+  if ((rc = listed(g, g.colsum_partials, (size_t)t.cs_pre_rows * Dff * sizeof(float)))) return rc;
   if ((rc = xp_gemm(&g, st))) return rc;
   if (a.db1) {
     if (t.db1_fused_rows == 0 && (rc = xp_colsum_partials(t.dpre, n, Dff, Dff, dt, t.cs_pre, t.cs_pre_bytes, st))) return rc;
     df.add(t.cs_pre, a.db1, Dff, (int)t.cs_pre_rows, (int)Dff);
   }
-  if (a.dw2 && (rc = run_wgrad(wgrad_desc(a.dx3, a.act, a.dw2, n, D, Dff, dt), slabs, slab_bytes, wg.stream(), true))) return rc;
+  if (a.dw2 && (rc = run_wgrad(wgrad_desc(a.dx3, a.act, a.dw2, n, D, Dff, dt), slabs, slab_bytes, wg.stream(), true, sup, 0))) return rc;
   if ((rc = wg.mark(1))) return rc;
   g = gemm_desc(t.dpre, a.W1, t.dh2, n, D, Dff, dt);
   g.b_kstrided = 1; g.ldb = D;
-  if ((rc = xp_gemm(&g, st))) return rc;
-  if (a.dw1 && (rc = run_wgrad(wgrad_desc(t.dpre, a.h2, a.dw1, n, Dff, D, dt), slabs, slab_bytes, wg.stream(), true))) return rc;
+  if ((rc = listed(g, t.dh2, (size_t)n * D * t.esz))) return rc;
+  if ((rc = xp_gemm(&g, st))) return rc;
+  if (a.dw1 && (rc = run_wgrad(wgrad_desc(t.dpre, a.h2, a.dw1, n, Dff, D, dt), slabs, slab_bytes, wg.stream(), true, sup, 1))) return rc;
   if ((rc = xp_layernorm_bwd_partials_side(t.dh2, D, a.x2, D, a.ln2_w, a.mean2, a.rstd2, a.dx3, D, t.dx2, D, 2, n, D, dt,
                                            a.side_x2, sS, sM, sM, t.ln2_part, t.ln2_bytes, st))) return rc;
   df.add(t.ln2_part, a.dln2_w, 4 * D, (int)t.ln_rows, (int)D);
@@ -191,8 +207,9 @@
   if ((rc = wg.mark(2))) return rc;
   g = gemm_desc(t.dx2, a.Wo, t.dattn, n, D, D, dt);
   g.b_kstrided = 1; g.ldb = D;
-  if ((rc = xp_gemm(&g, st))) return rc;
-  if (a.dwo && (rc = run_wgrad(wgrad_desc(t.dx2, a.attn_o, a.dwo, n, D, D, dt), slabs, slab_bytes, wg.stream(), true))) return rc;
+  if ((rc = listed(g, t.dattn, (size_t)n * D * t.esz))) return rc;
+  if ((rc = xp_gemm(&g, st))) return rc;
+  if (a.dwo && (rc = run_wgrad(wgrad_desc(t.dx2, a.attn_o, a.dwo, n, D, D, dt), slabs, slab_bytes, wg.stream(), true, sup, 2))) return rc;
   return XP_OK;
 }
 
@@ -298,7 +315,14 @@
   return carve_bwd(*d, nullptr, 0).ws.bytes();
 }
 
-extern "C" int xp_encoder_layer_bwd(const XpLayerBwd* a, void* st) {
+static int encoder_layer_bwd(const XpLayerBwd* a, const XpDx3Support* sup, void* st);
+extern "C" int xp_encoder_layer_bwd(const XpLayerBwd* a, void* st) { return encoder_layer_bwd(a, nullptr, st); }
+extern "C" int xp_encoder_layer_bwd_listed(const XpLayerBwd* a, const XpDx3Support* sup, void* st) {
+  XP_REQUIRE(sup, "xp_encoder_layer_bwd_listed: null dx3_support");
+  return encoder_layer_bwd(a, sup, st);
+}
+
+static int encoder_layer_bwd(const XpLayerBwd* a, const XpDx3Support* sup, void* st) {
   XP_REQUIRE(a, "xp_encoder_layer_bwd: null argument");
   const XpLayerDims& d = a->dims;
   int rc = check_dims("xp_encoder_layer_bwd", d);
@@ -316,7 +340,13 @@
   Defer df;
   const WgradOrder wg{(d.attn_mode == XP_ATTN_PROXY && rows >= 4096) ? wgrad_side() : nullptr, (hipStream_t)st, "xp_encoder_layer_bwd"};
   if ((rc = wg.mark(0))) return rc;
-  if ((rc = mlp_out_proj_bwd(*a, rows, w.t, w.slabs, w.slab_bytes, a->side_S, a->side_M, df, wg, st))) return rc;
+  if (sup) {
+    XP_REQUIRE(w.t.db1_fused_rows > 0 && sup->m_tiles && sup->n_m_tiles >= 1, "xp_encoder_layer_bwd: dx3_support needs the 256-wide "
+               "GEMM plans of this shape (fused fc1 bias sums) and a non-empty m_tiles");
+    for (int i = 0; i < 3; ++i)
+      XP_REQUIRE(sup->k_tiles[i] && sup->k_tile_begin[i] && sup->k_tile_begin_host[i], "xp_encoder_layer_bwd: dx3_support list %d is null", i);
+  }
+  if ((rc = mlp_out_proj_bwd(*a, rows, w.t, w.slabs, w.slab_bytes, a->side_S, a->side_M, df, wg, st, sup))) return rc;
   if ((rc = xp_attn_bwd2(a->qkv, 3 * D, a->attn_o, w.t.dattn, D, a->stats, a->pad_mask, w.dqkv, d.q_scale, d.attn_mode, d.B, d.heads,
                          d.S, d.M, d.N, d.L, dt, w.attn, w.attn_bytes, (a->dbqkv && w.cs_qkv_fused) ? w.cs_qkv : nullptr, st))) return rc;
   if ((rc = wg.mark(3))) return rc;
diff --git a/xpretrain_amd/functional.py b/xpretrain_amd/functional.py
--- a/xpretrain_amd/functional.py
+++ b/xpretrain_amd/functional.py
@@ -143,6 +143,7 @@
 
 
 LAYER_CALLS = "op_by_op" not in L.DEBUG
+SPARSE_LAST_BWD = os.environ.get("XPRETRAIN_SPARSE_LAST_BWD", "1") != "0"
 _DT_CODE = {torch.bfloat16: L.XP_BF16, torch.float32: L.XP_F32}
 _NULLCTX = contextlib.nullcontext()
 _ES = {torch.bfloat16: 2, torch.float32: 4}
@@ -359,10 +360,10 @@
             setattr(a, n, t.data_ptr() + first)
 
 
-def _call_native(entry, a, ws_bytes, device, ws_tag):
+def _call_native(entry, a, ws_bytes, device, ws_tag, *extra):
     ws = H.workspace(ws_bytes, device, ws_tag)
     a.workspace, a.workspace_bytes = ws.data_ptr(), ws.numel()
-    L.check(getattr(L.lib(), entry)(C.byref(a), H._stream()), entry)
+    L.check(getattr(L.lib(), entry)(C.byref(a), *extra, H._stream()), entry)
 
 
 def _layer_fwd_args(plan, dims, x, params, pad_mask, arena, x3, keep_pre, side, side_out, side_x2, r0=0):
@@ -435,7 +436,7 @@
             pick(dwqkv, 2, need[7]), pick(dbqkv, 2, need[8]))
 
 
-def _layer_backward(ctx, build, entry, ws_tag, ops, x, *rest):
+def _layer_backward(ctx, build, entry, ws_tag, ops, x, *rest, extra=()):
     plan, dev, need = ctx.plan, x.device, ctx.needs_input_grad
     flat = None
     if GRAD_SINKS and ctx.sink_key is not None and all(need[1:17]):
@@ -447,7 +448,7 @@
     g = {name: t for name, t in zip(plan.gnames, flat.split_with_sizes(plan.gsizes)) if want[name]}
     dx = torch.empty_like(x)
     if ctx.native:
-        _call_native(entry, build(plan, x, *rest, dx, g), plan.bwd_ws, dev, ws_tag)
+        _call_native(entry, build(plan, x, *rest, dx, g), plan.bwd_ws, dev, ws_tag, *extra)
     else:
         ops(plan, x, *rest, dx, g)
     D, Dff = plan.dims.D, plan.dims.Dff
@@ -455,6 +456,81 @@
     return (dx, g.get("dln1_w"), g.get("dln1_b"), *_qkv_grads(gw("dwqkv", (3 * D, D)), g.get("dbqkv"), need, D),
             gw("dwo", (D, D)), g.get("dbo"), g.get("dln2_w"), g.get("dln2_b"),
             gw("dw1", (Dff, D)), g.get("db1"), gw("dw2", (D, Dff)), g.get("db2"))
+
+
+_ROW_CLAIMS = {}
+_SUPPORTS = {}
+sparse_last_bwd_calls = 0
+
+
+def claim_row_support(t, B, S, r0):
+    key = id(t)
+    _ROW_CLAIMS[key] = (weakref.ref(t, lambda _, key=key: _ROW_CLAIMS.pop(key, None)), t._version, t.data_ptr(), (int(B), int(S), int(r0)))
+
+
+def row_support_of(t):
+    c = _ROW_CLAIMS.get(id(t))
+    if c is None or c[0]() is not t or c[1] != t._version or c[2] != t.data_ptr():
+        return None
+    return c[3]
+
+
+def dx3_tile_lists(B, S, r0, slabs):
+    rows = B * S
+    active = sorted({(b * S + r0) // 64 for b in range(B)})
+    hot = {kt // 4 for kt in active}
+    m, lists = set(hot), []
+    for split, kps in slabs:
+        tiles, begin = [], [0]
+        for z in range(split):
+            k0, k1 = z * kps // 64, (min((z + 1) * kps, rows) + 63) // 64
+            mine = [kt for kt in active if k0 <= kt < k1]
+            spare = [kt for kt in range(k0, k1) if kt not in mine]
+            spare.sort(key=lambda kt: (kt // 4 not in hot, kt))
+            mine = sorted(mine + spare[:max(0, 2 - len(mine))])
+            if len(mine) < 2:
+                raise ValueError(f"dx3_tile_lists: slab {z} of {split} x {kps} rows has fewer than 2 k-tiles")
+            tiles += mine
+            begin.append(len(tiles))
+        m.update(kt // 4 for kt in tiles)
+        lists.append((tiles, begin))
+    return sorted(m), lists
+
+
+class _Dx3Support:
+
+    def __init__(self, dev, m_tiles, lists, splits):
+        put = lambda v: torch.tensor(v, dtype=torch.int32, device=dev)
+        self.keep = [put(m_tiles)]
+        s = self.struct = L.XpDx3Support()
+        s.m_tiles, s.n_m_tiles = self.keep[0].data_ptr(), len(m_tiles)
+        for w, ((tiles, begin), split) in enumerate(zip(lists, splits)):
+            host = (C.c_int32 * len(begin))(*begin)
+            self.keep += [put(tiles), put(begin), host]
+            s.k_tiles[w], s.k_tile_begin[w], s.k_tile_begin_host[w] = self.keep[-3].data_ptr(), self.keep[-2].data_ptr(), C.addressof(host)
+            s.split[w] = split
+
+
+def _dx3_support(plan, dev, claim):
+    d = plan.dims
+    if claim is None or (claim[0], claim[1]) != (d.B, d.S) or not 0 <= claim[2] < d.S:
+        return None
+    rows, D, Dff = d.rows, d.D, d.Dff
+    wg = ((D, Dff), (Dff, D), (D, D))
+    splits = tuple(_split_for(no, ni, rows, plan.dtype, (0, 0, 0), True) for no, ni in wg)
+    key = (dev, d.B, d.S, claim[2], D, Dff, plan.dtype, d.act, splits)
+    if key not in _SUPPORTS:
+        if torch.cuda.is_current_stream_capturing():
+            return None
+        plans = [H.gemm_plan(no, ni, rows, plan.dtype, a_kstrided=True, b_kstrided=True, split_k=sp) for (no, ni), sp in zip(wg, splits)]
+        plans += [H.gemm_plan(rows, n, k, plan.dtype, b_kstrided=True, **kw)
+                  for n, k, kw in ((Dff, D, dict(epilogue=L.EPI_ACT_BWD[d.act], colsum=True)), (D, Dff, {}), (D, D, {}))]
+        sup = None
+        if all(p["family"] == L.GEMM_FAMILY_256 for p in plans) and plans[3]["colsum_rows"] > 0:
+            m_tiles, lists = dx3_tile_lists(d.B, d.S, claim[2], [(p["split"], p["k_per_split"]) for p in plans[:3]])
+            sup = _Dx3Support(dev, m_tiles, lists, splits)
+        _SUPPORTS[key] = sup
+    return _SUPPORTS[key]
 
 
 def _layer_bwd_args(plan, x, params, arena, dx3, pad_mask, side, side_x2, dx, grads):
@@ -608,9 +684,17 @@
         if dx3 is None:
             return (None,) * 26
         x, arena, *params, pad_mask, side, side_x2 = ctx.saved_tensors
+        claim = row_support_of(dx3)
         dx3 = _check_dx3("EncoderLayerFn", dx3, x, x.shape)
-        return _layer_backward(ctx, _layer_bwd_args, "xp_encoder_layer_bwd", "layer_bwd", _layer_bwd_ops, x, params, arena, dx3,
-                               pad_mask, side, side_x2) + (None,) * 9
+        entry, extra = "xp_encoder_layer_bwd", ()
+        if SPARSE_LAST_BWD and ctx.native and ctx.plan.size is not None and claim is not None:
+            support = _dx3_support(ctx.plan, x.device, claim)
+            if support is not None:
+                global sparse_last_bwd_calls
+                sparse_last_bwd_calls += 1
+                entry, extra = "xp_encoder_layer_bwd_listed", (C.byref(support.struct),)
+        return _layer_backward(ctx, _layer_bwd_args, entry, "layer_bwd", _layer_bwd_ops, x, params, arena, dx3,
+                               pad_mask, side, side_x2, extra=extra) + (None,) * 9
 
 
 class _PooledLayerPlan:
@@ -875,7 +959,10 @@
     def backward(ctx, dout):
         (idx,) = ctx.saved_tensors
         B, S, D = ctx.meta
-        return H.scatter_rows(dout.contiguous(), idx, B, S, D), None, None, None
+        dx = H.scatter_rows(dout.contiguous(), idx, B, S, D)
+        if idx is None:
+            claim_row_support(dx, B, S, 0)
+        return dx, None, None, None
 
 
 class ProjectionFn(torch.autograd.Function):
diff --git a/xpretrain_amd/hip_ops.py b/xpretrain_amd/hip_ops.py
--- a/xpretrain_amd/hip_ops.py
+++ b/xpretrain_amd/hip_ops.py
@@ -51,7 +51,8 @@
          a_kstrided=False, b_kstrided=False, out_dtype=None, epilogue=L.EPI_NONE, bias=None, scale=1.0,
          scale_cols=0, resid=None, ldr=None, aux=None, ldaux=None, tab1=None, tab2=None, tab_L=0,
          a_remap=(0, 0, 0), c_remap=(0, 0, 0), split_k=1, out_rows=None, colsum_defer=None, colsum_name="gemm_colsum",
-         colsum_out=None, resid_side=None, out_side=None, side=None, frames=None, frame_patch=0, frame_norm=None, plan_only=False):
+         colsum_out=None, resid_side=None, out_side=None, side=None, frames=None, frame_patch=0, frame_norm=None, plan_only=False,
+         m_tiles=None, k_tiles=None, k_tile_begin=None):
     if frames is not None:
         _chk(frames, "frames"); _chk(B, "B", torch.bfloat16)
         if A is not None or frames.dim() != 4 or frames.shape[1] != 3 or not frames.is_contiguous() or \
@@ -99,6 +100,14 @@
         if not (resid_side.is_contiguous() and out_side.is_contiguous()) or resid_side.numel() < need or out_side.numel() < need:
             raise ValueError("gemm: resid_side / out_side are too small or not contiguous")
         d.resid_side, d.out_side, d.side_S, d.side_M = resid_side.data_ptr(), out_side.data_ptr(), S_, M_
+    lists = [None if v is None else torch.tensor(list(v), dtype=torch.int32, device=B.device) for v in (m_tiles, k_tiles, k_tile_begin)]
+    if m_tiles is not None:
+        d.m_tiles, d.n_m_tiles = lists[0].data_ptr(), lists[0].numel()
+    if k_tiles is not None or k_tile_begin is not None:
+        if k_tiles is None or k_tile_begin is None or len(k_tile_begin) != max(split_k, 1) + 1:
+            raise ValueError("gemm: k_tiles and k_tile_begin go together, k_tile_begin with split_k + 1 entries")
+        begin_host = (C.c_int32 * len(k_tile_begin))(*k_tile_begin)
+        d.k_tiles, d.k_tile_begin, d.k_tile_begin_host = lists[1].data_ptr(), lists[2].data_ptr(), C.addressof(begin_host)
     if plan_only:
         if colsum_defer is not None and L.lib().xp_gemm_colsum_rows(C.byref(d)) > 0:
             d.colsum_partials = 1
@@ -121,6 +130,20 @@
     info = L.XpGemmPlanInfo()
     L.check(L.lib().xp_debug_gemm_plan(C.byref(d), C.byref(info)), "xp_debug_gemm_plan")
     return {f: (tuple(getattr(info, f)) if f == "grid" else getattr(info, f)) for f, _ in info._fields_ if f != "reserved"}
+
+
+def gemm_plan(M: int, N: int, K: int, dtype: torch.dtype, *, a_kstrided=False, b_kstrided=False, split_k=1, epilogue=L.EPI_NONE,
+              colsum=False) -> dict:
+    d = L.XpGemmDesc()
+    d.M, d.N, d.K = M, N, K
+    d.lda, d.ldb, d.ldc, d.ldr, d.ldaux = (M if a_kstrided else K), (N if b_kstrided else K), N, N, N
+    d.a_kstrided, d.b_kstrided = int(a_kstrided), int(b_kstrided)
+    d.in_dtype, d.out_dtype = _DT[dtype], _DT[torch.float32 if split_k > 1 or (a_kstrided and b_kstrided) else dtype]
+    d.epilogue, d.split_k, d.scale = epilogue, split_k, 1.0
+    d.resid = int(epilogue in L.EPI_ACT_BWD)
+    if colsum and L.lib().xp_gemm_colsum_rows(C.byref(d)) > 0:
+        d.colsum_partials = 1
+    return gemm_plan_of(d)
 
 
 def gemm_auto_split(M: int, N: int, K: int, dtype: torch.dtype, *, a_kstrided=True, b_kstrided=True, lda=None,
```

Result: faster. 572.8 pairs/s, median of 6 (+1.4%).
